# geekieo/collaborative-deep-metric-learning

Measured on NVIDIA B200. Metric: train_triplets_per_sec, higher is better.
Workload: dtype fp16 operands / fp32 accumulate (tcgen05 kind::f16), fp32 master weights

## Files before the change

collaborative-deep-metric-learning_b200/csrc/gemm_launch.cuh:

```cuda
#pragma once
#include "../../include/cdml.h"
#include "ctx.cuh"
#include "gemm_sm100.cuh"
#include "gemm2_sm100.cuh"

#include <stdlib.h>

namespace cdml {

inline bool trace_on() {
  static int on = -1;
  if (on < 0) on = getenv("CDML_TRACE") != nullptr ? 1 : 0;
  return on == 1;
}
inline int trace_sync(const char* what, long M, long N, long K, int grid, cudaStream_t st) {
  if (!trace_on()) return 0;
  fprintf(stderr, "[cdml] %s M=%ld N=%ld K=%ld grid=%d ... ", what, M, N, K, grid);
  fflush(stderr);
  cudaError_t e = cudaStreamSynchronize(st);
  fprintf(stderr, "%s\n", cudaGetErrorString(e));
  fflush(stderr);
  return e == cudaSuccess ? 0 : -2;
}

constexpr int kBN = 256;
constexpr int kStages = 4;

inline int pick_splits(int num_sms, int tiles, int num_kb) {
  if (tiles >= 2 * num_sms || num_kb < 16) return 1;
  const int smax = max(1, min(64, num_kb / 8));
  int best = 1;
  double best_eff = -1.0;
  for (int s = 1; s <= smax; ++s) {
    const int per = (num_kb + s - 1) / s;
    const int seff = (num_kb + per - 1) / per;
    if (seff != s) continue;
    const long units = static_cast<long>(tiles) * s;
    const long waves = (units + num_sms - 1) / num_sms;
    double eff = static_cast<double>(units) / static_cast<double>(waves * num_sms);
    if (units < num_sms) eff *= 0.5;
    eff -= 0.002 * s;
    if (eff > best_eff) best_eff = eff, best = s;
  }
  return best;
}

inline bool two_cta_enabled() {
  static int on = -1;
  if (on < 0) {
    const char* e = getenv("CDML_2CTA");
    on = (e != nullptr && e[0] == '0') ? 0 : 1;
  }
  return on == 1;
}

template <int AMN, int BMN, class Epi>
static int launch_gemm2(cdml_ctx* ctx, const void* A, int64_t lda, const void* B, int64_t ldb, int64_t M, int64_t N,
                        int64_t K, int dtype16, int num_splits, const Epi& epi, cudaStream_t stream) {
  using L = Gemm2Smem;
  CUtensorMap ta, tb;
  int rc;
  if (AMN == 0) rc = make_tmap_2d(ctx, &ta, A, dtype16, K, M, lda, kBK, kBM);
  else rc = make_tmap_2d(ctx, &ta, A, dtype16, M, K, lda, 64, kBK);
  if (rc) return rc;
  if (BMN == 0) rc = make_tmap_2d(ctx, &tb, B, dtype16, K, N, ldb, kBK, kBN2 / 2);
  else rc = make_tmap_2d(ctx, &tb, B, dtype16, N, K, ldb, 64, kBK);
  if (rc) return rc;
  GemmShape s;
  s.M = static_cast<int>(M), s.N = static_cast<int>(N), s.K = static_cast<int>(K);
  s.m_tiles = (s.M + 2 * kBM - 1) / (2 * kBM);
  s.n_tiles = (s.N + kBN2 - 1) / kBN2;
  s.num_kb = (s.K + kBK - 1) / kBK;
  num_splits = max(1, min(num_splits, s.num_kb));
  s.kb_per_split = (s.num_kb + num_splits - 1) / num_splits;
  s.num_splits = (s.num_kb + s.kb_per_split - 1) / s.kb_per_split;
  s.idesc = make_idesc_f16(dtype16 == CDML_BF16 ? 1 : 0, AMN, BMN, 2 * kBM, kBN2);
  s.m_fastest = (s.num_splits > 1 && N >= M) ? 1 : 0;
  auto kern = gemm2_tcgen05_kernel<AMN, BMN, Epi>;
  static bool attr_set = false;
  if (!attr_set) {
    CDML_CHECK_CUDA(cudaFuncSetAttribute(kern, cudaFuncAttributeMaxDynamicSharedMemorySize, L::kTotal));
    attr_set = true;
  }
  const long units = static_cast<long>(s.m_tiles) * s.n_tiles * s.num_splits;
  const int clusters = static_cast<int>(units < ctx->num_sms / 2 ? units : ctx->num_sms / 2);
  cudaLaunchConfig_t cfg = {};
  cfg.gridDim = dim3(2 * clusters);
  cfg.blockDim = dim3(kGemmThreads);
  cfg.dynamicSmemBytes = L::kTotal;
  cfg.stream = stream;
  cudaLaunchAttribute attr[1];
  attr[0].id = cudaLaunchAttributeClusterDimension;
  attr[0].val.clusterDim.x = 2, attr[0].val.clusterDim.y = 1, attr[0].val.clusterDim.z = 1;
  cfg.attrs = attr;
  cfg.numAttrs = 1;
  CDML_CHECK_CUDA(cudaLaunchKernelEx(&cfg, kern, ta, tb, s, epi));
  if (trace_sync("gemm2_tcgen05", M, N, K, 2 * clusters, stream)) return -2;
  return s.num_splits;
}

template <int AMN, int BMN, class Epi>
static int launch_gemm(cdml_ctx* ctx, const void* A, int64_t lda, const void* B, int64_t ldb, int64_t M, int64_t N,
                       int64_t K, int dtype16, int num_splits, const Epi& epi, cudaStream_t stream) {
  {
    const int64_t kb_per = ((K + kBK - 1) / kBK + max(num_splits, 1) - 1) / max(num_splits, 1);
    if (two_cta_enabled() && M >= 2 * kBM && kb_per >= 8)
      return launch_gemm2<AMN, BMN>(ctx, A, lda, B, ldb, M, N, K, dtype16, num_splits, epi, stream);
  }
  using L = GemmSmem<kBN, kStages>;
  CUtensorMap ta, tb;
  int rc;
  if (AMN == 0) rc = make_tmap_2d(ctx, &ta, A, dtype16, K, M, lda, kBK, kBM);
  else rc = make_tmap_2d(ctx, &ta, A, dtype16, M, K, lda, 64, kBK);
  if (rc) return rc;
  if (BMN == 0) rc = make_tmap_2d(ctx, &tb, B, dtype16, K, N, ldb, kBK, kBN);
  else rc = make_tmap_2d(ctx, &tb, B, dtype16, N, K, ldb, 64, kBK);
  if (rc) return rc;

  GemmShape s;
  s.M = static_cast<int>(M), s.N = static_cast<int>(N), s.K = static_cast<int>(K);
  s.m_tiles = (s.M + kBM - 1) / kBM;
  s.n_tiles = (s.N + kBN - 1) / kBN;
  s.num_kb = (s.K + kBK - 1) / kBK;
  num_splits = max(1, min(num_splits, s.num_kb));
  s.kb_per_split = (s.num_kb + num_splits - 1) / num_splits;
  s.num_splits = (s.num_kb + s.kb_per_split - 1) / s.kb_per_split;
  s.idesc = make_idesc_f16(dtype16 == CDML_BF16 ? 1 : 0, AMN, BMN, kBM, kBN);
  s.m_fastest = (s.num_splits > 1 && N >= M) ? 1 : 0;

  auto kern = gemm_tcgen05_kernel<AMN, BMN, kBN, kStages, Epi>;
  static bool attr_set = false;
  if (!attr_set) {
    CDML_CHECK_CUDA(cudaFuncSetAttribute(kern, cudaFuncAttributeMaxDynamicSharedMemorySize, L::kTotal));
    attr_set = true;
  }
  const long units = static_cast<long>(s.m_tiles) * s.n_tiles * s.num_splits;
  const int grid = static_cast<int>(units < ctx->num_sms ? units : ctx->num_sms);
  kern<<<grid, kGemmThreads, L::kTotal, stream>>>(ta, tb, s, epi);
  CDML_CHECK_CUDA(cudaGetLastError());
  if (trace_sync("gemm_tcgen05", M, N, K, grid, stream)) return -2;
  return s.num_splits;
}

constexpr int kResBStages = 4;
inline bool resb_applicable(int64_t K) {
  static int off = -1;
  if (off < 0) off = getenv("CDML_NO_RESB") != nullptr ? 1 : 0;
  return off == 0 && K <= 4 * kBK;
}

template <class Epi, int kEpiWarps = 8>
static int launch_gemm_resb(cdml_ctx* ctx, const void* A, int64_t lda, const void* B, int64_t ldb, int64_t M, int64_t N,
                            int64_t K, int dtype16, const Epi& epi, cudaStream_t stream, int n_fastest = 0) {
  using L = ResBSmem<kBN, kResBStages, kEpiWarps, Epi::kRowConsts, Epi::kTmaStore ? 2 : 1>;
  static_assert(L::kTotal <= 232448, "resident-B kernel: shared memory over the 227 KB limit");
  CUtensorMap ta, tb;
  int rc = make_tmap_2d(ctx, &ta, A, dtype16, K, M, lda, kBK, kBM);
  if (rc) return rc;
  rc = make_tmap_2d(ctx, &tb, B, dtype16, K, N, ldb, kBK, kBN);
  if (rc) return rc;
  ResBShape s;
  s.M = static_cast<int>(M), s.N = static_cast<int>(N), s.K = static_cast<int>(K);
  s.m_tiles = (s.M + kBM - 1) / kBM;
  s.n_tiles = (s.N + kBN - 1) / kBN;
  s.num_kb = (s.K + kBK - 1) / kBK;
  int best = 1;
  double best_eff = -1.0;
  const int cmax = max(1, min(s.m_tiles / 8, 4 * ctx->num_sms));
  for (int c = 1; c <= cmax; ++c) {
    const int tpc = (s.m_tiles + c - 1) / c;
    const int ceff = (s.m_tiles + tpc - 1) / tpc;
    if (ceff != c) continue;
    const long units = static_cast<long>(s.n_tiles) * c;
    const long waves = (units + ctx->num_sms - 1) / ctx->num_sms;
    double eff = static_cast<double>(units) / static_cast<double>(waves * ctx->num_sms);
    eff -= 0.15 / tpc;
    if (eff > best_eff) best_eff = eff, best = c;
  }
  s.m_chunks = best;
  s.tiles_per_chunk = (s.m_tiles + best - 1) / best;
  s.n_fastest = n_fastest;
  s.idesc = make_idesc_f16(dtype16 == CDML_BF16 ? 1 : 0, 0, 0, kBM, kBN);
  auto kern = gemm_resb_tcgen05_kernel<kBN, kResBStages, Epi, kEpiWarps>;
  static bool attr_set = false;
  if (!attr_set) {
    CDML_CHECK_CUDA(cudaFuncSetAttribute(kern, cudaFuncAttributeMaxDynamicSharedMemorySize, L::kTotal));
    attr_set = true;
  }
  const long units = static_cast<long>(s.n_tiles) * s.m_chunks;
  const int grid = static_cast<int>(units < ctx->num_sms ? units : ctx->num_sms);
  kern<<<grid, 128 + 32 * kEpiWarps, L::kTotal, stream>>>(ta, tb, s, epi);
  CDML_CHECK_CUDA(cudaGetLastError());
  if (trace_sync("gemm_resb", M, N, K, grid, stream)) return -2;
  return 1;
}

}
```

collaborative-deep-metric-learning_b200/csrc/gemm_sm100.cuh:

```cuda
#pragma once
#include "common.cuh"

namespace cdml {

constexpr int kBM = 128;
constexpr int kBK = 64;
constexpr int kUK = 16;
constexpr uint32_t kEpiStageBytes = 16384;
constexpr int kGemmThreads = 384;

struct GemmShape {
  int M, N, K;
  int m_tiles, n_tiles;
  int num_kb;
  int kb_per_split;
  int num_splits;
  int m_fastest;
  uint32_t idesc;
};

template <int BN, int kStages>
struct GemmSmem {
  static constexpr uint32_t kABytes = kBM * kBK * 2;
  static constexpr uint32_t kBBytes = BN * kBK * 2;
  static constexpr uint32_t kEpiOff = kStages * (kABytes + kBBytes);
  static constexpr uint32_t kBarOff = kEpiOff + kEpiStageBytes;
  static constexpr uint32_t kNumBars = 2 * kStages + 4;
  static constexpr uint32_t kTotal = kBarOff + kNumBars * 8 + 16 + 1024;
};

__device__ __forceinline__ float leaky(float v, float alpha) { return v > 0.f ? v : alpha * v; }
__device__ __forceinline__ float chunk_bias(const float* bias, int nb, int N) {
  const int col = nb + static_cast<int>(threadIdx.x & 31);
  return (bias != nullptr && col < N) ? __ldg(bias + col) : 0.f;
}

__device__ __forceinline__ void store_chunk16(uint16_t* out, int64_t ld, int row_base, int nb, int M, int N, uint32_t stg,
                                              const uint32_t (&pk)[16]) {
  const int lane = threadIdx.x & 31;
  __syncwarp();
#pragma unroll
  for (int j = 0; j < 4; ++j)
    sts128(stg + lane * 64 + ((j ^ ((lane >> 1) & 3)) << 4), pk[4 * j], pk[4 * j + 1], pk[4 * j + 2], pk[4 * j + 3]);
  __syncwarp();
  const int cch = lane & 3;
  const int col = nb + 8 * cch;
  const bool vec = (ld & 7) == 0;
#pragma unroll
  for (int i = 0; i < 4; ++i) {
    const int r = 8 * i + (lane >> 2);
    const uint4 v = lds128(stg + r * 64 + ((cch ^ ((r >> 1) & 3)) << 4));
    const int grow = row_base + r;
    if (grow < M) {
      uint16_t* p = out + static_cast<int64_t>(grow) * ld + col;
      if (vec && col + 8 <= N) {
        *reinterpret_cast<uint4*>(p) = v;
      } else {
        const uint32_t w[4] = {v.x, v.y, v.z, v.w};
#pragma unroll
        for (int e = 0; e < 8; ++e)
          if (col + e < N) p[e] = static_cast<uint16_t>(w[e >> 1] >> ((e & 1) * 16));
      }
    }
  }
}

__device__ __forceinline__ void store_chunk32(float* out, int64_t ld, int row_base, int nb, int M, int N, uint32_t stg,
                                              const float (&f)[32]) {
  const int lane = threadIdx.x & 31;
  __syncwarp();
#pragma unroll
  for (int j = 0; j < 8; ++j)
    sts128(stg + lane * 128 + ((j ^ (lane & 7)) << 4), __float_as_uint(f[4 * j]), __float_as_uint(f[4 * j + 1]),
           __float_as_uint(f[4 * j + 2]), __float_as_uint(f[4 * j + 3]));
  __syncwarp();
  const int cch = lane & 7;
  const int col = nb + 4 * cch;
  const bool vec = (ld & 3) == 0;
#pragma unroll
  for (int i = 0; i < 8; ++i) {
    const int r = 4 * i + (lane >> 3);
    const uint4 v = lds128(stg + r * 128 + ((cch ^ (r & 7)) << 4));
    const int grow = row_base + r;
    if (grow < M) {
      float* p = out + static_cast<int64_t>(grow) * ld + col;
      if (vec && col + 4 <= N) {
        *reinterpret_cast<uint4*>(p) = v;
      } else {
        const uint32_t w[4] = {v.x, v.y, v.z, v.w};
#pragma unroll
        for (int e = 0; e < 4; ++e)
          if (col + e < N) p[e] = __uint_as_float(w[e]);
      }
    }
  }
}

constexpr uint32_t kColCacheOff = 128, kColTagOff = 640, kWarpSliceBytes = 2048;
__device__ __forceinline__ void col_cache_reset(uint32_t epi_smem) {
  for (int w = 0; w < 8; ++w)
    asm volatile("st.shared.b32 [%0], %1;" ::"r"(epi_smem + w * kWarpSliceBytes + kColTagOff), "r"(0u) : "memory");
}
template <class Fetch>
__device__ __forceinline__ void col_cache_fill(uint32_t stg, int n0, int c0, Fetch&& fetch) {
  uint32_t tag;
  asm volatile("ld.shared.b32 %0, [%1];" : "=r"(tag) : "r"(stg + kColTagOff) : "memory");
  if (tag == static_cast<uint32_t>(n0 + 1)) return;
  const int lane = threadIdx.x & 31;
  __syncwarp();
#pragma unroll
  for (int i = 0; i < 4; ++i) {
    const uint32_t v = fetch(n0 + (c0 + i) * 32 + lane);
    asm volatile("st.shared.b32 [%0], %1;" ::"r"(stg + kColCacheOff + 4 * (32 * i + lane)), "r"(v) : "memory");
  }
  if (lane == 0) asm volatile("st.shared.b32 [%0], %1;" ::"r"(stg + kColTagOff), "r"(n0 + 1) : "memory");
  __syncwarp();
}

template <int BN>
struct EpiStoreF32 {
  static constexpr bool kSplitColumns = true;
  struct State {};
  __device__ __forceinline__ void pre(State&, int, int, const GemmShape&, int, int, uint32_t) const {}
  static constexpr bool kPrefetchNext = false;
  static constexpr bool kRowConsts = false;
  static constexpr bool kEarlyRelease = false;
  static constexpr bool kTmaStore = false;
  __device__ __forceinline__ void cols(int, const GemmShape&, int, int, uint32_t) const {}
  __device__ __forceinline__ void block_begin(uint32_t) const {}
  __device__ __forceinline__ void block_end(uint32_t) const {}
  float* out;
  int64_t ld;
  int64_t split_stride;
  const float* bias;
  float alpha;
  __device__ __forceinline__ void run(uint32_t taddr, int row, int n0, int split, const GemmShape& s, int c0, int c1, uint32_t stg, State& st) const {
    float* orow = out + static_cast<int64_t>(split) * split_stride + static_cast<int64_t>(row) * ld;
    const bool row_ok = row < s.M;
#pragma unroll 1
    for (int c = c0; c < c1; ++c) {
      const int nb = n0 + c * 32;
      if (nb >= s.N) break;
      uint32_t v[32];
      tmem_ld_32x32(taddr + c * 32, v);
      const float b_lane = chunk_bias(bias, nb, s.N);
      tmem_ld_wait();
      float f[32];
#pragma unroll
      for (int j = 0; j < 32; ++j)
        f[j] = leaky(__uint_as_float(v[j]) + __shfl_sync(0xffffffffu, b_lane, j), alpha);
      if (row_ok) {
        if (nb + 32 <= s.N && (ld & 3) == 0) {
          float4* p = reinterpret_cast<float4*>(orow + nb);
#pragma unroll
          for (int j = 0; j < 8; ++j) p[j] = make_float4(f[4 * j], f[4 * j + 1], f[4 * j + 2], f[4 * j + 3]);
        } else {
#pragma unroll
          for (int j = 0; j < 32; ++j)
            if (nb + j < s.N) orow[nb + j] = f[j];
        }
      }
    }
  }
};

template <int BN, int kBf16>
struct EpiStore16 {
  static constexpr bool kSplitColumns = true;
  struct State {};
  __device__ __forceinline__ void pre(State&, int, int, const GemmShape&, int, int, uint32_t) const {}
  static constexpr bool kPrefetchNext = false;
  static constexpr bool kRowConsts = false;
  static constexpr bool kEarlyRelease = false;
  static constexpr bool kTmaStore = false;
  __device__ __forceinline__ void cols(int, const GemmShape&, int, int, uint32_t) const {}
  __device__ __forceinline__ void block_begin(uint32_t) const {}
  __device__ __forceinline__ void block_end(uint32_t) const {}
  uint16_t* out;
  int64_t ld;
  const float* bias;
  float alpha;
  uint32_t* mask_out;
  int64_t ld_mask;
  __device__ __forceinline__ void run(uint32_t taddr, int row, int n0, int , const GemmShape& s, int c0, int c1, uint32_t stg, State& st) const {
#pragma unroll 1
    for (int c = c0; c < c1; ++c) {
      const int nb = n0 + c * 32;
      if (nb >= s.N) break;
      uint32_t v[32];
      tmem_ld_32x32(taddr + c * 32, v);
      const float b_lane = chunk_bias(bias, nb, s.N);
      tmem_ld_wait();
      uint32_t pk[16];
      uint32_t bits = 0u;
#pragma unroll
      for (int j = 0; j < 16; ++j) {
        const float x0 = __uint_as_float(v[2 * j]) + __shfl_sync(0xffffffffu, b_lane, 2 * j);
        const float x1 = __uint_as_float(v[2 * j + 1]) + __shfl_sync(0xffffffffu, b_lane, 2 * j + 1);
        bits |= (x0 > 0.f ? 1u : 0u) << (2 * j);
        bits |= (x1 > 0.f ? 1u : 0u) << (2 * j + 1);
        pk[j] = pack2<kBf16>(leaky(x0, alpha), leaky(x1, alpha));
      }
      if (mask_out != nullptr && row < s.M) mask_out[static_cast<int64_t>(nb >> 5) * ld_mask + row] = bits;
      store_chunk16(out, ld, row - static_cast<int>(threadIdx.x & 31), nb, s.M, s.N, stg, pk);
    }
  }
};

template <int BN, int kBf16>
struct EpiL2Norm {
  static constexpr bool kSplitColumns = false;
  struct State {};
  __device__ __forceinline__ void pre(State&, int, int, const GemmShape&, int, int, uint32_t) const {}
  static constexpr bool kPrefetchNext = false;
  static constexpr bool kRowConsts = false;
  static constexpr bool kEarlyRelease = false;
  static constexpr bool kTmaStore = false;
  __device__ __forceinline__ void cols(int, const GemmShape&, int, int, uint32_t) const {}
  __device__ __forceinline__ void block_begin(uint32_t) const {}
  __device__ __forceinline__ void block_end(uint32_t) const {}
  float* out;
  int64_t ld;
  const float* bias;
  float alpha;
  float* rinv;
  uint16_t* out16;
  int64_t ld16;
  __device__ __forceinline__ void run(uint32_t taddr, int row, int n0, int , const GemmShape& s, int c0, int c1, uint32_t stg, State& st) const {
    const bool row_ok = row < s.M;
    float ss = 0.f;
#pragma unroll 1
    for (int c = c0; c < c1; ++c) {
      const int nb = n0 + c * 32;
      if (nb >= s.N) break;
      uint32_t v[32];
      tmem_ld_32x32(taddr + c * 32, v);
      const float b_lane = chunk_bias(bias, nb, s.N);
      tmem_ld_wait();
#pragma unroll
      for (int j = 0; j < 32; ++j) {
        const float x = leaky(__uint_as_float(v[j]) + __shfl_sync(0xffffffffu, b_lane, j), alpha);
        ss = fmaf(x, x, ss);
      }
    }
    const float r = rsqrtf(fmaxf(ss, 1e-12f));
    if (row_ok && rinv != nullptr) rinv[row] = r;
#pragma unroll 1
    for (int c = c0; c < c1; ++c) {
      const int nb = n0 + c * 32;
      if (nb >= s.N) break;
      uint32_t v[32];
      tmem_ld_32x32(taddr + c * 32, v);
      const float b_lane = chunk_bias(bias, nb, s.N);
      tmem_ld_wait();
      float f[32];
#pragma unroll
      for (int j = 0; j < 32; ++j)
        f[j] = leaky(__uint_as_float(v[j]) + __shfl_sync(0xffffffffu, b_lane, j), alpha) * r;
      store_chunk32(out, ld, row - static_cast<int>(threadIdx.x & 31), nb, s.M, s.N, stg, f);
      if (out16 != nullptr) {
        uint32_t pk[16];
#pragma unroll
        for (int j = 0; j < 16; ++j) pk[j] = pack2<kBf16>(f[2 * j], f[2 * j + 1]);
        store_chunk16(out16, ld16, row - static_cast<int>(threadIdx.x & 31), nb, s.M, s.N, stg, pk);
      }
    }
  }
};

template <int BN, int kBf16>
struct EpiMaskLeaky {
  static constexpr bool kSplitColumns = true;
  struct State {
    uint4 raw[4][4];
  };
  static constexpr bool kPrefetchNext = false;
  static constexpr bool kRowConsts = false;
  static constexpr bool kEarlyRelease = false;
  static constexpr bool kTmaStore = false;
  __device__ __forceinline__ void cols(int, const GemmShape&, int, int, uint32_t) const {}
  __device__ __forceinline__ void block_begin(uint32_t) const {}
  __device__ __forceinline__ void block_end(uint32_t) const {}
  uint16_t* out;
  int64_t ld;
  const uint16_t* mask;
  int64_t ld_mask;
  float alpha;
  __device__ __forceinline__ void fetch_mask(int row_base, int nb, int M, int N, bool active, uint4 (&raw)[4]) const {
    const int lane = threadIdx.x & 31;
    const int col = nb + 8 * (lane & 3);
#pragma unroll
    for (int i = 0; i < 4; ++i) {
      const int grow = row_base + 8 * i + (lane >> 2);
      raw[i] = make_uint4(0u, 0u, 0u, 0u);
      if (active && grow < M) {
        const uint16_t* p = mask + static_cast<int64_t>(grow) * ld_mask + col;
        if ((ld_mask & 7) == 0 && col + 8 <= N) {
          raw[i] = __ldg(reinterpret_cast<const uint4*>(p));
        } else {
          uint32_t w[4] = {0u, 0u, 0u, 0u};
#pragma unroll
          for (int e = 0; e < 8; ++e)
            if (col + e < N) w[e >> 1] |= static_cast<uint32_t>(p[e]) << ((e & 1) * 16);
          raw[i] = make_uint4(w[0], w[1], w[2], w[3]);
        }
      }
    }
  }
  __device__ __forceinline__ void transpose_mask(uint32_t stg, const uint4 (&raw)[4], uint32_t (&mk)[16]) const {
    const int lane = threadIdx.x & 31;
    const int cch = lane & 3;
    __syncwarp();
#pragma unroll
    for (int i = 0; i < 4; ++i) {
      const int r = 8 * i + (lane >> 2);
      sts128(stg + r * 64 + ((cch ^ ((r >> 1) & 3)) << 4), raw[i].x, raw[i].y, raw[i].z, raw[i].w);
    }
    __syncwarp();
#pragma unroll
    for (int j = 0; j < 4; ++j) {
      const uint4 t = lds128(stg + lane * 64 + ((j ^ ((lane >> 1) & 3)) << 4));
      mk[4 * j] = t.x, mk[4 * j + 1] = t.y, mk[4 * j + 2] = t.z, mk[4 * j + 3] = t.w;
    }
  }
  __device__ __forceinline__ void pre(State& st, int row, int n0, const GemmShape& s, int c0, int c1, uint32_t ) const {
    static_assert(BN == 256, "a warp owns 4 chunks of the tile");
    const int row_base = row - static_cast<int>(threadIdx.x & 31);
#pragma unroll
    for (int cc = 0; cc < 4; ++cc)
      fetch_mask(row_base, n0 + (c0 + cc) * 32, s.M, s.N, c0 + cc < c1 && n0 + (c0 + cc) * 32 < s.N, st.raw[cc]);
  }
  __device__ __forceinline__ void run(uint32_t taddr, int row, int n0, int , const GemmShape& s, int c0, int c1,
                                      uint32_t stg, State& st) const {
    const int row_base = row - static_cast<int>(threadIdx.x & 31);
#pragma unroll
    for (int cc = 0; cc < 4; ++cc) {
      const int c = c0 + cc;
      const int nb = n0 + c * 32;
      if (c < c1 && nb < s.N) {
        uint32_t v[32];
        tmem_ld_32x32(taddr + c * 32, v);
        uint32_t mk[16];
        transpose_mask(stg, st.raw[cc], mk);
        tmem_ld_wait();
        uint32_t pk[16];
#pragma unroll
        for (int j = 0; j < 16; ++j) {
          const float2 m = unpack2<kBf16>(mk[j]);
          const float x0 = __uint_as_float(v[2 * j]) * (m.x > 0.f ? 1.f : alpha);
          const float x1 = __uint_as_float(v[2 * j + 1]) * (m.y > 0.f ? 1.f : alpha);
          pk[j] = pack2<kBf16>(x0, x1);
        }
        store_chunk16(out, ld, row_base, nb, s.M, s.N, stg, pk);
      }
    }
  }
};

template <int BN, int kBf16>
struct EpiMaskBits {
  static constexpr bool kSplitColumns = true;
  struct State {
    uint32_t bits[4];
  };
  static constexpr bool kPrefetchNext = true;
  static constexpr bool kRowConsts = false;
  static constexpr bool kEarlyRelease = false;
  static constexpr bool kTmaStore = false;
  __device__ __forceinline__ void cols(int, const GemmShape&, int, int, uint32_t) const {}
  __device__ __forceinline__ void block_begin(uint32_t) const {}
  __device__ __forceinline__ void block_end(uint32_t) const {}
  uint16_t* out;
  int64_t ld;
  const uint32_t* mask;
  int64_t ld_mask;
  float alpha;
  __device__ __forceinline__ void pre(State& st, int row, int n0, const GemmShape& s, int c0, int c1, uint32_t ) const {
    static_assert(BN == 256, "a warp owns 4 chunks of the tile");
#pragma unroll
    for (int cc = 0; cc < 4; ++cc) {
      const int nb = n0 + (c0 + cc) * 32;
      st.bits[cc] = (c0 + cc < c1 && nb < s.N && row < s.M) ? __ldg(mask + static_cast<int64_t>(nb >> 5) * ld_mask + row) : 0u;
    }
  }
  __device__ __forceinline__ void run(uint32_t taddr, int row, int n0, int , const GemmShape& s, int c0, int c1,
                                      uint32_t stg, State& st) const {
    const int row_base = row - static_cast<int>(threadIdx.x & 31);
    auto ok = [&](int cc) { return c0 + cc < c1 && n0 + (c0 + cc) * 32 < s.N; };
    auto chunk = [&](const uint32_t (&v)[32], int cc) {
      const uint32_t b = st.bits[cc];
      uint32_t pk[16];
#pragma unroll
      for (int j = 0; j < 16; ++j) {
        const float x0 = __uint_as_float(v[2 * j]) * ((b >> (2 * j)) & 1u ? 1.f : alpha);
        const float x1 = __uint_as_float(v[2 * j + 1]) * ((b >> (2 * j + 1)) & 1u ? 1.f : alpha);
        pk[j] = pack2<kBf16>(x0, x1);
      }
      store_chunk16(out, ld, row_base, n0 + (c0 + cc) * 32, s.M, s.N, stg, pk);
    };
    uint32_t va[32], vb[32];
    if (ok(0)) tmem_ld_32x32(taddr + c0 * 32, va);
#pragma unroll
    for (int cc = 0; cc < 4; cc += 2) {
      tmem_ld_wait();
      if (ok(cc + 1)) tmem_ld_32x32(taddr + (c0 + cc + 1) * 32, vb);
      if (ok(cc)) chunk(va, cc);
      tmem_ld_wait();
      if (cc + 2 < 4 && ok(cc + 2)) tmem_ld_32x32(taddr + (c0 + cc + 2) * 32, va);
      if (ok(cc + 1)) chunk(vb, cc + 1);
    }
  }
};

template <int BN, int kBf16>
struct EpiMaskBitsTma {
  static constexpr bool kSplitColumns = true;
  struct State {
    uint32_t bits[4];
    uint32_t release_bar;
  };
  static constexpr bool kPrefetchNext = true;
  static constexpr bool kRowConsts = false;
  static constexpr bool kEarlyRelease = true;
  static constexpr bool kTmaStore = true;
  __device__ __forceinline__ void cols(int, const GemmShape&, int, int, uint32_t) const {}
  __device__ __forceinline__ void block_begin(uint32_t) const {}
  __device__ __forceinline__ void block_end(uint32_t) const {}
  CUtensorMap out_map;
  const uint32_t* mask;
  int64_t ld_mask;
  float alpha;
  __device__ __forceinline__ void pre(State& st, int row, int n0, const GemmShape& s, int c0, int c1, uint32_t ) const {
    static_assert(BN == 256, "a warp owns 4 chunks of the tile");
#pragma unroll
    for (int cc = 0; cc < 4; ++cc) {
      const int nb = n0 + (c0 + cc) * 32;
      st.bits[cc] = (c0 + cc < c1 && nb < s.N && row < s.M) ? __ldg(mask + static_cast<int64_t>(nb >> 5) * ld_mask + row) : 0u;
    }
    st.release_bar = 0u;
  }
  __device__ __forceinline__ void run(uint32_t taddr, int row, int n0, int , const GemmShape& s, int c0, int c1,
                                      uint32_t stg0, State& st) const {
    const int lane = threadIdx.x & 31;
    const int row_base = row - lane;
    auto ok = [&](int cc) { return c0 + cc < c1 && n0 + (c0 + cc) * 32 < s.N; };
    auto chunk = [&](const uint32_t (&v)[32], int cc) {
      const uint32_t b = st.bits[cc];
      uint32_t pk[16];
#pragma unroll
      for (int j = 0; j < 16; ++j) {
        const float x0 = __uint_as_float(v[2 * j]) * ((b >> (2 * j)) & 1u ? 1.f : alpha);
        const float x1 = __uint_as_float(v[2 * j + 1]) * ((b >> (2 * j + 1)) & 1u ? 1.f : alpha);
        pk[j] = pack2<kBf16>(x0, x1);
      }
      const uint32_t stg = stg0 + (cc & 1) * 2048u;
      if (lane == 0) bulk_wait_read1();
      __syncwarp();
#pragma unroll
      for (int j = 0; j < 4; ++j)
        sts128(stg + lane * 64 + ((j ^ ((lane >> 1) & 3)) << 4), pk[4 * j], pk[4 * j + 1], pk[4 * j + 2], pk[4 * j + 3]);
      fence_proxy_async();
      __syncwarp();
      if (lane == 0) {
        tma_store_2d(&out_map, stg, n0 + (c0 + cc) * 32, row_base);
        bulk_commit();
      }
    };
    uint32_t va[32], vb[32];
    if (ok(0)) tmem_ld_32x32(taddr + c0 * 32, va);
#pragma unroll
    for (int cc = 0; cc < 4; cc += 2) {
      tmem_ld_wait();
      if (ok(cc + 1)) tmem_ld_32x32(taddr + (c0 + cc + 1) * 32, vb);
      if (ok(cc)) chunk(va, cc);
      tmem_ld_wait();
      if (cc + 2 < 4 && ok(cc + 2)) tmem_ld_32x32(taddr + (c0 + cc + 2) * 32, va);
      if (cc + 2 >= 4 && st.release_bar != 0u) {
        tc_fence_before();
        __syncwarp();
        if (lane == 0) mbar_arrive(st.release_bar);
      }
      if (ok(cc + 1)) chunk(vb, cc + 1);
    }
  }
};

template <int BN, int kReadTmem>
struct EpiNull {
  static constexpr bool kSplitColumns = true;
  struct State {};
  __device__ __forceinline__ void pre(State&, int, int, const GemmShape&, int, int, uint32_t) const {}
  static constexpr bool kPrefetchNext = false;
  static constexpr bool kRowConsts = false;
  static constexpr bool kEarlyRelease = false;
  static constexpr bool kTmaStore = false;
  __device__ __forceinline__ void cols(int, const GemmShape&, int, int, uint32_t) const {}
  __device__ __forceinline__ void block_begin(uint32_t) const {}
  __device__ __forceinline__ void block_end(uint32_t) const {}
  float* out;
  __device__ __forceinline__ void run(uint32_t taddr, int row, int n0, int , const GemmShape& s, int c0, int c1, uint32_t stg, State& st) const {
    if (kReadTmem) {
      uint32_t acc = 0u;
#pragma unroll 1
      for (int c = c0; c < c1; ++c) {
        uint32_t v[32];
        tmem_ld_32x32(taddr + c * 32, v);
        tmem_ld_wait();
#pragma unroll
        for (int j = 0; j < 32; ++j) acc ^= v[j];
      }
      if (acc == 0x7fc12345u && row == s.M + 7) out[0] = 1.f;
    }
  }
};

template <int kAMajorMN, int kBMajorMN, int BN, int kStages, class Epi>
__global__ void __launch_bounds__(kGemmThreads, 1)
gemm_tcgen05_kernel(const __grid_constant__ CUtensorMap tma_a, const __grid_constant__ CUtensorMap tma_b,
                    const GemmShape s, const Epi epi) {
  using L = GemmSmem<BN, kStages>;
  extern __shared__ uint8_t smem_raw[];
  const uint32_t raw_u32 = smem_u32(smem_raw);
  const uint32_t base = (raw_u32 + 1023u) & ~1023u;
  const uint32_t bar0 = base + L::kBarOff;
  auto a_smem = [&](int st) { return base + st * L::kABytes; };
  auto b_smem = [&](int st) { return base + kStages * L::kABytes + st * L::kBBytes; };
  auto full_bar = [&](int st) { return bar0 + 8u * st; };
  auto empty_bar = [&](int st) { return bar0 + 8u * (kStages + st); };
  auto tfull_bar = [&](int i) { return bar0 + 8u * (2 * kStages + i); };
  auto tempty_bar = [&](int i) { return bar0 + 8u * (2 * kStages + 2 + i); };
  const uint32_t tmem_slot = bar0 + 8u * L::kNumBars;
  volatile uint32_t* tmem_slot_ptr = reinterpret_cast<volatile uint32_t*>(smem_raw + (tmem_slot - raw_u32));

  const int warp = threadIdx.x >> 5;
  const int lane = threadIdx.x & 31;
  constexpr uint32_t kTmemCols = (2 * BN <= 32) ? 32 : (2 * BN <= 64) ? 64 : (2 * BN <= 128) ? 128 : (2 * BN <= 256) ? 256 : 512;
  static_assert(2 * BN <= 512, "two accumulator stages must fit TMEM");

  if (warp == 0 && lane == 0) {
    tma_prefetch_desc(&tma_a);
    tma_prefetch_desc(&tma_b);
  }
  if (warp == 1 && lane == 0) {
    for (int i = 0; i < kStages; ++i) {
      mbar_init(full_bar(i), 1);
      mbar_init(empty_bar(i), 1);
    }
    for (int i = 0; i < 2; ++i) {
      mbar_init(tfull_bar(i), 1);
      mbar_init(tempty_bar(i), 8);
    }
    fence_mbar_init();
  }
  if (warp == 2) {
    tmem_alloc(tmem_slot, kTmemCols);
    tmem_relinquish();
  }
  if (threadIdx.x == 96) epi.block_begin(base + L::kEpiOff);
  tc_fence_before();
  __syncthreads();
  tc_fence_after();
  const uint32_t tmem_base = *tmem_slot_ptr;

  const int tiles = s.m_tiles * s.n_tiles;
  const int units = tiles * s.num_splits;

  if (warp == 0 && lane == 0) {
    int stage = 0;
    uint32_t phase = 0;
    for (int u = blockIdx.x; u < units; u += gridDim.x) {
      const int split = u / tiles, t = u - split * tiles;
      const int m0 = (s.m_fastest ? t % s.m_tiles : t / s.n_tiles) * kBM;
      const int n0 = (s.m_fastest ? t / s.m_tiles : t % s.n_tiles) * BN;
      const int kb0 = split * s.kb_per_split;
      const int kb1 = min(s.num_kb, kb0 + s.kb_per_split);
      for (int kb = kb0; kb < kb1; ++kb) {
        mbar_wait(empty_bar(stage), phase ^ 1, 100 + stage);
        mbar_arrive_expect_tx(full_bar(stage), L::kABytes + L::kBBytes);
        const int k0 = kb * kBK;
        if constexpr (kAMajorMN == 0) {
          tma_load_2d(a_smem(stage), &tma_a, full_bar(stage), k0, m0);
        } else {
#pragma unroll
          for (int i = 0; i < kBM / 64; ++i)
            tma_load_2d(a_smem(stage) + i * (kBK * 128), &tma_a, full_bar(stage), m0 + i * 64, k0);
        }
        if constexpr (kBMajorMN == 0) {
          tma_load_2d(b_smem(stage), &tma_b, full_bar(stage), k0, n0);
        } else {
#pragma unroll
          for (int i = 0; i < BN / 64; ++i)
            tma_load_2d(b_smem(stage) + i * (kBK * 128), &tma_b, full_bar(stage), n0 + i * 64, k0);
        }
        if (++stage == kStages) stage = 0, phase ^= 1;
      }
    }
  } else if (warp == 1 && lane == 0) {
    int stage = 0;
    uint32_t phase = 0;
    int it = 0;
    constexpr uint32_t kAStep = kAMajorMN ? (kUK * 128) : (kUK * 2);
    constexpr uint32_t kBStep = kBMajorMN ? (kUK * 128) : (kUK * 2);
    constexpr uint32_t kALbo = kAMajorMN ? (kBK * 128) : 16;
    constexpr uint32_t kBLbo = kBMajorMN ? (kBK * 128) : 16;
    for (int u = blockIdx.x; u < units; u += gridDim.x, ++it) {
      const int split = u / tiles;
      const int kb0 = split * s.kb_per_split;
      const int kb1 = min(s.num_kb, kb0 + s.kb_per_split);
      const int as = it & 1;
      const uint32_t ap = (it >> 1) & 1;
      mbar_wait(tempty_bar(as), ap ^ 1, 200 + as);
      tc_fence_after();
      const uint32_t tmem_d = tmem_base + as * BN;
      for (int kb = kb0; kb < kb1; ++kb) {
        mbar_wait(full_bar(stage), phase, 300 + stage);
        tc_fence_after();
#pragma unroll
        for (int k = 0; k < kBK / kUK; ++k) {
          const uint64_t ad = make_smem_desc(a_smem(stage) + k * kAStep, kALbo, 1024);
          const uint64_t bd = make_smem_desc(b_smem(stage) + k * kBStep, kBLbo, 1024);
          umma_f16(tmem_d, ad, bd, s.idesc, (kb > kb0 || k > 0) ? 1u : 0u);
        }
        tc_commit(empty_bar(stage));
        if (kb == kb1 - 1) tc_commit(tfull_bar(as));
        if (++stage == kStages) stage = 0, phase ^= 1;
      }
    }
  } else if (warp >= 4) {
    const int q = warp & 3;
    const int half = (warp - 4) >> 2;
    const uint32_t stg = base + L::kEpiOff + (warp - 4) * (Epi::kSplitColumns ? 2048u : 4096u);
    int it = 0;
    for (int u = blockIdx.x; u < units; u += gridDim.x, ++it) {
      const int split = u / tiles, t = u - split * tiles;
      const int m0 = (s.m_fastest ? t % s.m_tiles : t / s.n_tiles) * kBM;
      const int n0 = (s.m_fastest ? t / s.m_tiles : t % s.n_tiles) * BN;
      const int as = it & 1;
      const uint32_t ap = (it >> 1) & 1;
      const int ec0 = Epi::kSplitColumns ? half * (BN / 64) : 0, ec1 = Epi::kSplitColumns ? (half + 1) * (BN / 64) : BN / 32;
      typename Epi::State est;
      if (Epi::kSplitColumns || half == 0) {
        epi.cols(n0, s, ec0, ec1, stg);
        epi.pre(est, m0 + q * 32 + lane, n0, s, ec0, ec1, stg);
      }
      mbar_wait(tfull_bar(as), ap, 400 + as);
      tc_fence_after();
      const uint32_t taddr = tmem_base + (static_cast<uint32_t>(q * 32) << 16) + as * BN;
      if (Epi::kSplitColumns || half == 0) epi.run(taddr, m0 + q * 32 + lane, n0, split, s, ec0, ec1, stg, est);
      tc_fence_before();
      __syncwarp();
      if (lane == 0) mbar_arrive(tempty_bar(as));
    }
  }

  tc_fence_before();
  __syncthreads();
  if (threadIdx.x == 96) epi.block_end(base + L::kEpiOff);
  if (warp == 2) {
    tc_fence_after();
    tmem_dealloc(tmem_base, kTmemCols);
  }
}

struct ResBShape {
  int M, N, K;
  int m_tiles, n_tiles, num_kb;
  int m_chunks;
  int tiles_per_chunk;
  int n_fastest;
  uint32_t idesc;
};

template <int BN, int kAStages, int kEpiWarps = 8, bool kRowSlots = false, int kStageSlices = 1>
struct ResBSmem {
  static constexpr uint32_t kABytes = kBM * kBK * 2;
  static constexpr uint32_t kBPanel = BN * kBK * 2;
  static constexpr uint32_t kMaxKb = 4;
  static constexpr uint32_t kEpiOff = kMaxKb * kBPanel + kAStages * kABytes;
  static constexpr uint32_t kEpiBytes = kEpiWarps * 2048 * kStageSlices;
  static constexpr uint32_t kRowConstOff = kEpiOff + kEpiBytes;
  static constexpr uint32_t kRowConstSlot = kRowSlots ? kBM * 32 : 0;
  static constexpr uint32_t kBarOff = kRowConstOff + 2 * kRowConstSlot;
  static constexpr uint32_t kNumBars = 2 * kAStages + 2 + 4 + 2;
  static constexpr uint32_t kTotal = kBarOff + kNumBars * 8 + 16 + 1024;
};

template <int BN, int kAStages, class Epi, int kEpiWarps = 8>
__global__ void __launch_bounds__(128 + 32 * kEpiWarps, 1)
gemm_resb_tcgen05_kernel(const __grid_constant__ CUtensorMap tma_a, const __grid_constant__ CUtensorMap tma_b,
                         const ResBShape s, const __grid_constant__ Epi epi) {
  using L = ResBSmem<BN, kAStages, kEpiWarps, Epi::kRowConsts, Epi::kTmaStore ? 2 : 1>;
  static_assert(kEpiWarps == 8 || kEpiWarps == 16, "two or four epilogue warps per TMEM lane quarter");
  static_assert(kEpiWarps == 8 || Epi::kSplitColumns, "four warps per quarter split the tile's columns");
  extern __shared__ uint8_t smem_raw[];
  const uint32_t raw_u32 = smem_u32(smem_raw);
  const uint32_t base = (raw_u32 + 1023u) & ~1023u;
  const uint32_t bar0 = base + L::kBarOff;
  auto b_panel = [&](int kb) { return base + kb * L::kBPanel; };
  auto a_smem = [&](int st) { return base + L::kMaxKb * L::kBPanel + st * L::kABytes; };
  auto a_full = [&](int st) { return bar0 + 8u * st; };
  auto a_empty = [&](int st) { return bar0 + 8u * (kAStages + st); };
  const uint32_t b_full = bar0 + 8u * (2 * kAStages);
  const uint32_t b_empty = bar0 + 8u * (2 * kAStages + 1);
  auto tfull_bar = [&](int i) { return bar0 + 8u * (2 * kAStages + 2 + i); };
  auto tempty_bar = [&](int i) { return bar0 + 8u * (2 * kAStages + 4 + i); };
  auto cfull_bar = [&](int i) { return bar0 + 8u * (2 * kAStages + 6 + i); };
  auto cslot = [&](int i) { return base + L::kRowConstOff + i * L::kRowConstSlot; };
  const uint32_t tmem_slot = bar0 + 8u * L::kNumBars;
  volatile uint32_t* tmem_slot_ptr = reinterpret_cast<volatile uint32_t*>(smem_raw + (tmem_slot - raw_u32));
  const int warp = threadIdx.x >> 5;
  const int lane = threadIdx.x & 31;
  constexpr uint32_t kTmemCols = 512;
  static_assert(2 * BN <= 512, "two accumulator stages must fit TMEM");

  if (warp == 0 && lane == 0) {
    tma_prefetch_desc(&tma_a);
    tma_prefetch_desc(&tma_b);
  }
  if (warp == 1 && lane == 0) {
    for (int i = 0; i < kAStages; ++i) {
      mbar_init(a_full(i), 1);
      mbar_init(a_empty(i), 1);
    }
    mbar_init(b_full, 1);
    mbar_init(b_empty, 1);
    for (int i = 0; i < 2; ++i) {
      mbar_init(tfull_bar(i), 1);
      mbar_init(tempty_bar(i), kEpiWarps);
      mbar_init(cfull_bar(i), 1);
    }
    fence_mbar_init();
  }
  if (warp == 2) {
    tmem_alloc(tmem_slot, kTmemCols);
    tmem_relinquish();
  }
  if (threadIdx.x == 96) epi.block_begin(base + L::kEpiOff);
  tc_fence_before();
  __syncthreads();
  tc_fence_after();
  const uint32_t tmem_base = *tmem_slot_ptr;

  const int units = s.n_tiles * s.m_chunks;
  if (warp == 0 && lane == 0) {
    int stage = 0;
    uint32_t phase = 0, bphase = 0;
    for (int u = blockIdx.x; u < units; u += gridDim.x) {
      const int chunk = s.n_fastest ? u / s.n_tiles : u % s.m_chunks, nblk = s.n_fastest ? u % s.n_tiles : u / s.m_chunks;
      const int t0 = chunk * s.tiles_per_chunk, t1 = min(s.m_tiles, t0 + s.tiles_per_chunk);
      if (t0 >= t1) continue;
      mbar_wait(b_empty, bphase ^ 1, 500);
      mbar_arrive_expect_tx(b_full, s.num_kb * L::kBPanel);
      for (int kb = 0; kb < s.num_kb; ++kb) tma_load_2d(b_panel(kb), &tma_b, b_full, kb * kBK, nblk * BN);
      bphase ^= 1;
      for (int t = t0; t < t1; ++t) {
        for (int kb = 0; kb < s.num_kb; ++kb) {
          mbar_wait(a_empty(stage), phase ^ 1, 100 + stage);
          mbar_arrive_expect_tx(a_full(stage), L::kABytes);
          tma_load_2d(a_smem(stage), &tma_a, a_full(stage), kb * kBK, t * kBM);
          if (++stage == kAStages) stage = 0, phase ^= 1;
        }
      }
    }
  } else if (warp == 1 && lane == 0) {
    int stage = 0, it = 0;
    uint32_t phase = 0, bphase = 0;
    for (int u = blockIdx.x; u < units; u += gridDim.x) {
      const int chunk = s.n_fastest ? u / s.n_tiles : u % s.m_chunks, nblk = s.n_fastest ? u % s.n_tiles : u / s.m_chunks;
      const int t0 = chunk * s.tiles_per_chunk, t1 = min(s.m_tiles, t0 + s.tiles_per_chunk);
      if (t0 >= t1) continue;
      mbar_wait(b_full, bphase, 600);
      bphase ^= 1;
      tc_fence_after();
      for (int t = t0; t < t1; ++t, ++it) {
        const int as = it & 1;
        const uint32_t ap = (it >> 1) & 1;
        mbar_wait(tempty_bar(as), ap ^ 1, 200 + as);
        tc_fence_after();
        const uint32_t tmem_d = tmem_base + as * BN;
        for (int kb = 0; kb < s.num_kb; ++kb) {
          mbar_wait(a_full(stage), phase, 300 + stage);
          tc_fence_after();
#pragma unroll
          for (int k = 0; k < kBK / kUK; ++k) {
            const uint64_t ad = make_smem_desc(a_smem(stage) + k * (kUK * 2), 16, 1024);
            const uint64_t bd = make_smem_desc(b_panel(kb) + k * (kUK * 2), 16, 1024);
            umma_f16(tmem_d, ad, bd, s.idesc, (kb > 0 || k > 0) ? 1u : 0u);
          }
          tc_commit(a_empty(stage));
          if (kb == s.num_kb - 1) tc_commit(tfull_bar(as));
          if (++stage == kAStages) stage = 0, phase ^= 1;
        }
      }
      tc_commit(b_empty);
    }
  } else if (warp == 3) {
   if constexpr (Epi::kRowConsts) {
    int it = 0;
    GemmShape gs;
    gs.M = s.M, gs.N = s.N, gs.K = s.K;
    for (int u = blockIdx.x; u < units; u += gridDim.x) {
      const int chunk = s.n_fastest ? u / s.n_tiles : u % s.m_chunks;
      const int t0 = chunk * s.tiles_per_chunk, t1 = min(s.m_tiles, t0 + s.tiles_per_chunk);
      for (int t = t0; t < t1; ++t, ++it) {
        const int as = it & 1;
        const uint32_t ap = (it >> 1) & 1;
        mbar_wait(tempty_bar(as), ap ^ 1, 700 + as);
#pragma unroll
        for (int r = lane; r < kBM; r += 32) epi.row_consts(t * kBM + r, gs, cslot(as) + r * 32);
        __syncwarp();
        if (lane == 0) mbar_arrive(cfull_bar(as));
      }
    }
   }
  } else if (warp >= 4) {
    const int q = warp & 3;
    const int half = (warp - 4) >> 2;
    const uint32_t stg = base + L::kEpiOff + (warp - 4) * (Epi::kTmaStore ? 4096u : (Epi::kSplitColumns || kEpiWarps == 16) ? 2048u : 4096u);
    int it = 0;
    GemmShape gs;
    gs.M = s.M, gs.N = s.N, gs.K = s.K, gs.m_tiles = s.m_tiles, gs.n_tiles = s.n_tiles, gs.num_kb = s.num_kb;
    gs.kb_per_split = s.num_kb, gs.num_splits = 1, gs.m_fastest = 0, gs.idesc = s.idesc;
    struct TileIter {
      int u, t, t1, nblk;
      bool valid;
    };
    auto seek = [&](TileIter& ti) {
      ti.valid = false;
      for (; ti.u < units; ti.u += gridDim.x) {
        const int chunk = s.n_fastest ? ti.u / s.n_tiles : ti.u % s.m_chunks;
        const int t0 = chunk * s.tiles_per_chunk, t1 = min(s.m_tiles, t0 + s.tiles_per_chunk);
        if (t0 < t1) {
          ti.t = t0, ti.t1 = t1, ti.nblk = s.n_fastest ? ti.u % s.n_tiles : ti.u / s.m_chunks, ti.valid = true;
          return;
        }
      }
    };
    const bool active = Epi::kSplitColumns || half == 0;
    constexpr int kChunksPerWarp = (BN / 32) / (kEpiWarps / 4);
    const int ec0 = Epi::kSplitColumns ? half * kChunksPerWarp : 0, ec1 = Epi::kSplitColumns ? (half + 1) * kChunksPerWarp : BN / 32;
    TileIter cur;
    cur.u = blockIdx.x;
    seek(cur);
    typename Epi::State est;
    if (cur.valid && active) {
      epi.cols(cur.nblk * BN, gs, ec0, ec1, stg);
      if constexpr (!Epi::kRowConsts) epi.pre(est, cur.t * kBM + q * 32 + lane, cur.nblk * BN, gs, ec0, ec1, stg);
    }
    while (cur.valid) {
      TileIter nxt = cur;
      if (++nxt.t >= nxt.t1) {
        nxt.u += gridDim.x;
        seek(nxt);
      }
      const int as = it & 1;
      const uint32_t ap = (it >> 1) & 1;
      typename Epi::State est_next;
      if constexpr (Epi::kRowConsts) {
        mbar_wait(cfull_bar(as), ap, 800 + as);
        if (active) epi.load_state(est, cslot(as) + (q * 32 + lane) * 32);
        est_next = est;
      }
      mbar_wait(tfull_bar(as), ap, 400 + as);
      tc_fence_after();
      const uint32_t taddr = tmem_base + (static_cast<uint32_t>(q * 32) << 16) + as * BN;
      if (active) {
        if constexpr (!Epi::kRowConsts)
          if (Epi::kPrefetchNext && nxt.valid) epi.pre(est_next, nxt.t * kBM + q * 32 + lane, nxt.nblk * BN, gs, ec0, ec1, stg);
        if constexpr (Epi::kEarlyRelease) est.release_bar = tempty_bar(as);
        epi.run(taddr, cur.t * kBM + q * 32 + lane, cur.nblk * BN, 0, gs, ec0, ec1, stg, est);
      }
      if (!(Epi::kEarlyRelease && active)) {
        tc_fence_before();
        __syncwarp();
        if (lane == 0) mbar_arrive(tempty_bar(as));
      }
      if (active && nxt.valid) {
        epi.cols(nxt.nblk * BN, gs, ec0, ec1, stg);
        if constexpr (!Epi::kRowConsts)
          if (!Epi::kPrefetchNext) epi.pre(est_next, nxt.t * kBM + q * 32 + lane, nxt.nblk * BN, gs, ec0, ec1, stg);
      }
      est = est_next;
      cur = nxt;
      ++it;
    }
    if constexpr (Epi::kTmaStore) {
      if (lane == 0) bulk_wait_all();
    }
  }

  tc_fence_before();
  __syncthreads();
  if (threadIdx.x == 96) epi.block_end(base + L::kEpiOff);
  if (warp == 2) {
    tc_fence_after();
    tmem_dealloc(tmem_base, kTmemCols);
  }
}

}
```

collaborative-deep-metric-learning_b200/csrc/knn.cu:

```cuda
#include <math.h>
#include <string.h>

#include <algorithm>

#include <vector>

#include "gemm_launch.cuh"

namespace cdml {

constexpr int kCandCap = 2048;
constexpr int kKeepCap = 2048;
constexpr int kMaxGroups = 4096;
constexpr int kRefineThreads = 256;

__device__ __forceinline__ uint32_t f2key(float f) {
  const uint32_t u = __float_as_uint(f);
  return (u & 0x80000000u) ? ~u : (u | 0x80000000u);
}
__device__ __forceinline__ float key2f(uint32_t k) {
  return __uint_as_float((k & 0x80000000u) ? (k & 0x7FFFFFFFu) : ~k);
}
__device__ __forceinline__ float neg_inf() { return __int_as_float(0xff800000); }
__device__ __forceinline__ float pos_inf() { return __int_as_float(0x7f800000); }

__device__ __forceinline__ float4 ld4_or(const float* p, int col, int N, float fill) {
  if (col + 4 <= N) return __ldg(reinterpret_cast<const float4*>(p + col));
  float4 r;
  r.x = col < N ? __ldg(p + col) : fill;
  r.y = col + 1 < N ? __ldg(p + col + 1) : fill;
  r.z = col + 2 < N ? __ldg(p + col + 2) : fill;
  r.w = col + 3 < N ? __ldg(p + col + 3) : fill;
  return r;
}

template <int BN>
struct EpiKnnGroupMax {
  static constexpr bool kSplitColumns = true;
  static constexpr bool kPrefetchNext = false;
  static constexpr bool kRowConsts = false;
  static constexpr bool kEarlyRelease = false;
  static constexpr bool kTmaStore = false;
  struct State {};
  __device__ __forceinline__ void pre(State&, int, int, const GemmShape&, int, int, uint32_t) const {}
  __device__ __forceinline__ void block_begin(uint32_t epi_smem) const { col_cache_reset(epi_smem); }
  __device__ __forceinline__ void block_end(uint32_t) const {}
  const float* h;
  float* gmax;
  int64_t ldg;
  int wide;
  __device__ __forceinline__ void cols(int n0, const GemmShape& s, int c0, int , uint32_t stg) const {
    static_assert(BN == 256, "a warp owns 4 chunks (128 columns) of the tile");
    col_cache_fill(stg, n0, c0, [&](int col) { return __float_as_uint(col < s.N ? __ldg(h + col) : pos_inf()); });
  }
  __device__ __forceinline__ void run(uint32_t taddr, int row, int n0, int , const GemmShape& s, int c0,
                                      int , uint32_t stg, State& ) const {
    float g[4];
    uint32_t va[32], vb[32];
    auto group = [&](const uint32_t (&v)[32], int cc) {
      const uint32_t hbase = stg + kColCacheOff + 128 * cc;
      float b0 = neg_inf(), b1 = neg_inf();
#pragma unroll
      for (int j = 0; j < 8; ++j) {
        const uint4 t = lds128(hbase + 16 * j);
        const float2 lo = sub2(__uint_as_float(v[4 * j]), __uint_as_float(v[4 * j + 1]), __uint_as_float(t.x), __uint_as_float(t.y));
        const float2 hi = sub2(__uint_as_float(v[4 * j + 2]), __uint_as_float(v[4 * j + 3]), __uint_as_float(t.z), __uint_as_float(t.w));
        b0 = fmax3(b0, lo.x, lo.y);
        b1 = fmax3(b1, hi.x, hi.y);
      }
      return fmaxf(b0, b1);
    };
    auto ok = [&](int cc) { return n0 + (c0 + cc) * 32 < s.N; };
    tmem_ld_32x32(taddr + c0 * 32, va);
#pragma unroll
    for (int cc = 0; cc < 4; cc += 2) {
      tmem_ld_wait();
      if (ok(cc + 1)) tmem_ld_32x32(taddr + (c0 + cc + 1) * 32, vb);
      g[cc] = ok(cc) ? group(va, cc) : neg_inf();
      tmem_ld_wait();
      if (cc + 2 < 4 && ok(cc + 2)) tmem_ld_32x32(taddr + (c0 + cc + 2) * 32, va);
      g[cc + 1] = ok(cc + 1) ? group(vb, cc + 1) : neg_inf();
    }
    if (row < s.M) {
      if (wide) gmax[static_cast<int64_t>(row) * ldg + n0 / 128 + c0 / 4] = fmaxf(fmaxf(g[0], g[1]), fmaxf(g[2], g[3]));
      else *reinterpret_cast<float4*>(gmax + static_cast<int64_t>(row) * ldg + n0 / 32 + c0) = make_float4(g[0], g[1], g[2], g[3]);
    }
  }
};

constexpr uint32_t kKnnWarpStage = kWarpSliceBytes;
constexpr uint32_t kKnnThrOff = kColCacheOff, kKnnCurOff = 644;
constexpr int kKnnLogsPerCta = 8;

template <int BN>
struct EpiKnnCollect {
  static constexpr bool kSplitColumns = true;
  const float* h;
  const float* thr;
  uint4* log;
  int32_t* log_count;
  int32_t* log_overflow;
  unsigned int warp_cap;
  struct State {
    float hr;
    uint32_t release_bar;
  };
  static constexpr bool kPrefetchNext = true;
  static constexpr bool kRowConsts = false;
  static constexpr bool kEarlyRelease = true;
  static constexpr bool kTmaStore = false;
  __device__ __forceinline__ void block_begin(uint32_t epi_smem) const {
    col_cache_reset(epi_smem);
    for (int w = 0; w < kKnnLogsPerCta; ++w)
      asm volatile("st.shared.b32 [%0], %1;" ::"r"(epi_smem + w * kKnnWarpStage + kKnnCurOff), "r"(0u) : "memory");
  }
  __device__ __forceinline__ void block_end(uint32_t epi_smem) const {
    for (int w = 0; w < kKnnLogsPerCta; ++w) {
      unsigned int n;
      asm volatile("ld.shared.b32 %0, [%1];" : "=r"(n) : "r"(epi_smem + w * kKnnWarpStage + kKnnCurOff) : "memory");
      log_count[blockIdx.x * kKnnLogsPerCta + w] = static_cast<int32_t>(n < warp_cap ? n : warp_cap);
      if (n > warp_cap) atomicOr(log_overflow, 1);
    }
  }
  __device__ __forceinline__ void pre(State& st, int row, int, const GemmShape& s, int, int, uint32_t) const {
    st.hr = row < s.M ? __ldg(h + row) : pos_inf();
    st.release_bar = 0u;
  }
  __device__ __forceinline__ void cols(int n0, const GemmShape& s, int c0, int , uint32_t stg) const {
    static_assert(BN == 256, "a warp owns 4 chunks (128 columns) of the tile");
    col_cache_fill(stg, n0, c0, [&](int col) { return __float_as_uint(col < s.N ? __ldg(thr + col) : pos_inf()); });
  }
  __device__ __forceinline__ void run(uint32_t taddr, int row, int n0, int , const GemmShape& s, int c0,
                                      int c1, uint32_t stg, State& st) const {
    const float hr = st.hr;
    const int lane = threadIdx.x & 31;
    const int warp_slot = (threadIdx.x >> 5) - 4;
    uint4* my_log = log + (static_cast<size_t>(blockIdx.x) * kKnnLogsPerCta + warp_slot) * warp_cap;
    unsigned int cursor;
    asm volatile("ld.shared.b32 %0, [%1];" : "=r"(cursor) : "r"(stg + kKnnCurOff) : "memory");
    uint32_t va[32], vb[32];
    tmem_ld_32x32(taddr + c0 * 32, va);
    auto chunk = [&](const uint32_t (&v)[32], int cc) {
      const int nb = n0 + (c0 + cc) * 32;
      const uint32_t tbase = stg + kKnnThrOff + 128 * cc;
      float m0 = neg_inf(), m1 = neg_inf();
#pragma unroll
      for (int j = 0; j < 8; ++j) {
        const uint4 t = lds128(tbase + 16 * j);
        const float2 lo = sub2(__uint_as_float(v[4 * j]), __uint_as_float(v[4 * j + 1]), __uint_as_float(t.x), __uint_as_float(t.y));
        const float2 hi = sub2(__uint_as_float(v[4 * j + 2]), __uint_as_float(v[4 * j + 3]), __uint_as_float(t.z), __uint_as_float(t.w));
        m0 = fmax3(m0, lo.x, lo.y);
        m1 = fmax3(m1, hi.x, hi.y);
      }
      unsigned int hits = __ballot_sync(0xffffffffu, fmaxf(m0, m1) > hr);
      if (hits != 0u) {
        float thr_lane;
        asm volatile("ld.shared.f32 %0, [%1];" : "=f"(thr_lane) : "r"(tbase + 4 * lane) : "memory");
        do {
          const int src = __ffs(hits) - 1;
          hits &= hits - 1u;
          __syncwarp();
          if (lane == src) {
#pragma unroll
            for (int j = 0; j < 8; ++j) sts128(stg + 16 * j, v[4 * j], v[4 * j + 1], v[4 * j + 2], v[4 * j + 3]);
          }
          __syncwarp();
          float val;
          asm volatile("ld.shared.f32 %0, [%1];" : "=f"(val) : "r"(stg + 4 * lane) : "memory");
          const float hr_src = __shfl_sync(0xffffffffu, hr, src);
          const bool pass = val - thr_lane > hr_src;
          const unsigned int pm = __ballot_sync(0xffffffffu, pass);
          const unsigned int pos = cursor + static_cast<unsigned int>(__popc(pm & ((1u << lane) - 1u)));
          if (pass && pos < warp_cap)
            my_log[pos] = make_uint4(static_cast<uint32_t>(nb + lane), static_cast<uint32_t>(row - lane + src),
                                     __float_as_uint(val - hr_src), 0u);
          cursor += static_cast<unsigned int>(__popc(pm));
        } while (hits != 0u);
      }
    };
#pragma unroll
    for (int cc = 0; cc < 4; cc += 2) {
      const bool ok0 = c0 + cc < c1 && n0 + (c0 + cc) * 32 < s.N;
      const bool ok1 = c0 + cc + 1 < c1 && n0 + (c0 + cc + 1) * 32 < s.N;
      const bool ok2 = cc + 2 < 4 && c0 + cc + 2 < c1 && n0 + (c0 + cc + 2) * 32 < s.N;
      tmem_ld_wait();
      if (ok1) tmem_ld_32x32(taddr + (c0 + cc + 1) * 32, vb);
      if (ok0) chunk(va, cc);
      tmem_ld_wait();
      if (ok2) tmem_ld_32x32(taddr + (c0 + cc + 2) * 32, va);
      if (cc + 2 >= 4 && st.release_bar != 0u) {
        tc_fence_before();
        __syncwarp();
        if (lane == 0) mbar_arrive(st.release_bar);
      }
      if (ok1) chunk(vb, cc + 1);
    }
    __syncwarp();
    if (lane == 0) asm volatile("st.shared.b32 [%0], %1;" ::"r"(stg + kKnnCurOff), "r"(cursor) : "memory");
  }
};

__global__ void __launch_bounds__(256)
knn_bin_kernel(const uint4* __restrict__ log, const int32_t* __restrict__ log_count, unsigned int log_cap,
               int32_t* __restrict__ cand_idx, float* __restrict__ cand_val, int32_t* __restrict__ cnt, int cap) {
  const int n = log_count[blockIdx.y];
  const uint4* my = log + static_cast<size_t>(blockIdx.y) * log_cap;
  for (int i = blockIdx.x * blockDim.x + threadIdx.x; i < n; i += gridDim.x * blockDim.x) {
    const uint4 e = my[i];
    const int pos = atomicAdd(cnt + e.x, 1);
    if (pos < cap) {
      cand_idx[static_cast<int64_t>(e.x) * cap + pos] = static_cast<int32_t>(e.y);
      cand_val[static_cast<int64_t>(e.x) * cap + pos] = __uint_as_float(e.z);
    }
  }
}

__global__ void __launch_bounds__(256)
row_sumsq32_kernel(const float* __restrict__ X, int64_t n, int d, int64_t ld, float* __restrict__ ss, float half_scale,
                   float* __restrict__ half_out) {
  const int warp = threadIdx.x >> 5, lane = threadIdx.x & 31;
  for (int64_t r = static_cast<int64_t>(blockIdx.x) * 8 + warp; r < n; r += static_cast<int64_t>(gridDim.x) * 8) {
    const float* x = X + r * ld;
    float a = 0.f;
    for (int j = lane; j < d; j += 32) a = fmaf(x[j], x[j], a);
#pragma unroll
    for (int o = 16; o > 0; o >>= 1) a += __shfl_xor_sync(0xffffffffu, a, o);
    if (lane == 0) {
      ss[r] = a;
      if (half_out != nullptr) half_out[r] = a * half_scale;
    }
  }
}

__global__ void max_reduce_kernel(const float* __restrict__ x, int64_t n, float* __restrict__ out) {
  __shared__ float sh[32];
  float m = 0.f;
  for (int64_t i = threadIdx.x; i < n; i += blockDim.x) m = fmaxf(m, x[i]);
#pragma unroll
  for (int o = 16; o > 0; o >>= 1) m = fmaxf(m, __shfl_xor_sync(0xffffffffu, m, o));
  if ((threadIdx.x & 31) == 0) sh[threadIdx.x >> 5] = m;
  __syncthreads();
  if (threadIdx.x < 32) {
    m = threadIdx.x < (blockDim.x >> 5) ? sh[threadIdx.x] : 0.f;
#pragma unroll
    for (int o = 16; o > 0; o >>= 1) m = fmaxf(m, __shfl_xor_sync(0xffffffffu, m, o));
    if (threadIdx.x == 0) *out = m;
  }
}

__global__ void fill_f32_kernel(float* p, int64_t n, float v) {
  for (int64_t i = static_cast<int64_t>(blockIdx.x) * blockDim.x + threadIdx.x; i < n;
       i += static_cast<int64_t>(gridDim.x) * blockDim.x)
    p[i] = v;
}

__device__ __forceinline__ int block_sum(int v, int* sh) {
  v = __reduce_add_sync(0xffffffffu, v);
  __syncthreads();
  if ((threadIdx.x & 31) == 0) sh[threadIdx.x >> 5] = v;
  __syncthreads();
  int t = 0;
  for (int w = 0; w < (blockDim.x >> 5); ++w) t += sh[w];
  return t;
}

constexpr int kSelectBits = 20;
template <int kPer, bool kDual>
__global__ void __launch_bounds__(kRefineThreads)
knn_kth_kernel(const float* __restrict__ gmax, int64_t ldg, int G, int k, int k2, const float* __restrict__ qss,
               float slack_scale, float slack_abs, float* __restrict__ thr, float* __restrict__ thr2, float sign2) {
  __shared__ int sh[kRefineThreads / 32];
  const int q = blockIdx.x;
  const float* g = gmax + static_cast<int64_t>(q) * ldg;
  uint32_t keys[kPer];
#pragma unroll
  for (int i = 0; i < kPer; ++i) {
    const int j = threadIdx.x + i * kRefineThreads;
    keys[i] = j < G ? f2key(g[j]) : 0u;
  }
  uint32_t T = 0, T2 = 0;
  for (int bit = 31; bit >= 32 - kSelectBits; --bit) {
    const uint32_t cand = T | (1u << bit), cand2 = T2 | (1u << bit);
    int c = 0;
#pragma unroll
    for (int i = 0; i < kPer; ++i) c += (keys[i] >= cand ? 1 : 0) + (kDual && keys[i] >= cand2 ? 65536 : 0);
    c = block_sum(c, sh);
    if ((c & 0xffff) >= k) T = cand;
    if (kDual && (c >> 16) >= k2) T2 = cand2;
  }
  if (threadIdx.x == 0) {
    const float slack = slack_scale * sqrtf(qss[q]) + slack_abs;
    thr[q] = T > f2key(neg_inf()) ? key2f(T) - slack : neg_inf();
    if (kDual) thr2[q] = sign2 * (T2 > f2key(neg_inf()) ? key2f(T2) - slack : neg_inf());
  }
}

template <bool kDual>
__global__ void __launch_bounds__(256)
knn_kth_warp_kernel(const float* __restrict__ gmax, int64_t ldg, int G, int k, int k2, const float* __restrict__ qss,
                    int64_t nq, float slack_scale, float slack_abs, float* __restrict__ thr, float* __restrict__ thr2,
                    float sign2) {
  const int lane = threadIdx.x & 31;
  const int64_t q = static_cast<int64_t>(blockIdx.x) * 8 + (threadIdx.x >> 5);
  if (q >= nq) return;
  const float* g = gmax + q * ldg;
  uint32_t keys[32];
#pragma unroll
  for (int i = 0; i < 32; ++i) {
    const int j = lane + 32 * i;
    keys[i] = j < G ? f2key(g[j]) : 0u;
  }
  uint32_t T = 0, T2 = 0;
  for (int bit = 31; bit >= 32 - kSelectBits; --bit) {
    const uint32_t cand = T | (1u << bit), cand2 = T2 | (1u << bit);
    int c = 0;
#pragma unroll
    for (int i = 0; i < 32; ++i) c += (keys[i] >= cand ? 1 : 0) + (kDual && keys[i] >= cand2 ? 65536 : 0);
    c = __reduce_add_sync(0xffffffffu, c);
    if ((c & 0xffff) >= k) T = cand;
    if (kDual && (c >> 16) >= k2) T2 = cand2;
  }
  if (lane == 0) {
    const float slack = slack_scale * sqrtf(qss[q]) + slack_abs;
    thr[q] = T > f2key(neg_inf()) ? key2f(T) - slack : neg_inf();
    if (kDual) thr2[q] = sign2 * (T2 > f2key(neg_inf()) ? key2f(T2) - slack : neg_inf());
  }
}

__global__ void __launch_bounds__(256)
knn_nominee_kth_kernel(const float* __restrict__ cand_val, const int32_t* __restrict__ cnt, int cap, int k, int k2,
                       int64_t nq, float* __restrict__ pair) {
  const int lane = threadIdx.x & 31;
  const int64_t q = static_cast<int64_t>(blockIdx.x) * 8 + (threadIdx.x >> 5);
  if (q >= nq) return;
  const int n = cnt[q];
  float a = neg_inf(), b = neg_inf();
  if (n <= cap && n >= min(k, k2)) {
    const float* v = cand_val + q * cap;
    uint32_t keys[8];
    const bool in_regs = n <= 256;
#pragma unroll
    for (int i = 0; i < 8; ++i) keys[i] = (in_regs && lane + 32 * i < n) ? f2key(v[lane + 32 * i]) : 0u;
    uint32_t T = 0, T2 = 0;
    for (int bit = 31; bit >= 32 - kSelectBits; --bit) {
      const uint32_t cand = T | (1u << bit), cand2 = T2 | (1u << bit);
      int c = 0;
      if (in_regs) {
#pragma unroll
        for (int i = 0; i < 8; ++i) c += (keys[i] >= cand ? 1 : 0) + (keys[i] >= cand2 ? 65536 : 0);
      } else {
        for (int i = lane; i < n; i += 32) {
          const uint32_t key = f2key(v[i]);
          c += (key >= cand ? 1 : 0) + (key >= cand2 ? 65536 : 0);
        }
      }
      c = __reduce_add_sync(0xffffffffu, c);
      if ((c & 0xffff) >= k) T = cand;
      if ((c >> 16) >= k2) T2 = cand2;
    }
    if (n >= k && T > f2key(neg_inf())) a = key2f(T);
    if (n >= k2 && T2 > f2key(neg_inf())) b = key2f(T2);
  }
  if (lane == 0) pair[q] = a, pair[nq + q] = -b;
}

__global__ void knn_thr_combine_kernel(const float* __restrict__ full, const float* __restrict__ part,
                                       const float* __restrict__ qss, int64_t n, float slack_scale, float slack_abs,
                                       float* __restrict__ thr, float part_sign) {
  const int64_t i = static_cast<int64_t>(blockIdx.x) * blockDim.x + threadIdx.x;
  if (i >= n) return;
  const float b = fmaxf(full[i], part_sign * part[i]);
  thr[i] = b > neg_inf() ? b - (slack_scale * sqrtf(qss[i]) + slack_abs) : neg_inf();
}

__global__ void __launch_bounds__(kRefineThreads)
knn_refine_kernel(const float* __restrict__ Q, int64_t ldq, int d, const float* __restrict__ qss,
                  const float* __restrict__ X, int64_t ldx, const float* __restrict__ xss,
                  const int32_t* __restrict__ cand_idx, const float* __restrict__ cand_val,
                  const int32_t* __restrict__ cnt, int cap, int k, int metric, float slack_scale, float slack_abs,
                  int64_t id_offset, float* __restrict__ D, int64_t* __restrict__ I, int64_t out_ld,
                  int32_t* __restrict__ overflow, int n_all, const float* __restrict__ prune_pair, int64_t prune_ld,
                  const int32_t* __restrict__ handled) {
  __shared__ unsigned long long kept[kKeepCap];
  __shared__ int sh[kRefineThreads / 32];
  __shared__ uint32_t shu[2 * (kRefineThreads / 32)];
  __shared__ int n_keep;
  const int q = blockIdx.x;
  const int tid = threadIdx.x;
  if (handled != nullptr && handled[q] != 0) return;
  const int n = n_all > 0 ? 0 : cnt[q];
  if (n > cap) {
    if (tid == 0) overflow[q] = 1;
    return;
  }
  constexpr int kPer = kCandCap / kRefineThreads;
  uint32_t keys[kPer];
  int32_t idxs[kPer];
  uint32_t kmax = 0u, kmin = 0xffffffffu;
#pragma unroll
  for (int t = 0; t < kPer; ++t) {
    const int i = tid + t * kRefineThreads;
    keys[t] = 0u, idxs[t] = 0;
    if (i < n) {
      keys[t] = f2key(cand_val[static_cast<int64_t>(q) * cap + i]);
      idxs[t] = cand_idx[static_cast<int64_t>(q) * cap + i];
      kmax = max(kmax, keys[t]), kmin = min(kmin, keys[t]);
    }
  }
  if (tid == 0) n_keep = 0;
  uint32_t T = 0;
  if (n > k) {
    kmax = __reduce_max_sync(0xffffffffu, kmax), kmin = __reduce_min_sync(0xffffffffu, kmin);
    if ((tid & 31) == 0) shu[tid >> 5] = kmax, shu[kRefineThreads / 32 + (tid >> 5)] = kmin;
    __syncthreads();
#pragma unroll
    for (int w = 0; w < kRefineThreads / 32; ++w) kmax = max(kmax, shu[w]), kmin = min(kmin, shu[kRefineThreads / 32 + w]);
    const uint32_t diff = kmax ^ kmin;
    const int top = diff == 0u ? -1 : 31 - __clz(diff);
    T = top >= 31 ? 0u : (kmax >> (top + 1)) << (top + 1);
    for (int bit = top; bit >= 32 - kSelectBits; --bit) {
      const uint32_t cand = T | (1u << bit);
      int c = 0;
#pragma unroll
      for (int t = 0; t < kPer; ++t) c += keys[t] >= cand ? 1 : 0;
      if (block_sum(c, sh) >= k) T = cand;
    }
  } else {
    __syncthreads();
  }
  const float slack = slack_scale * sqrtf(qss[q]) + slack_abs;
  uint32_t keep_key = n > k ? f2key(key2f(T) - slack) : 0u;
  if (prune_pair != nullptr) {
    const float tg = fmaxf(prune_pair[q], -prune_pair[prune_ld + q]);
    if (tg > neg_inf()) keep_key = max(keep_key, f2key(tg - slack));
  }
#pragma unroll
  for (int t = 0; t < kPer; ++t) {
    if (tid + t * kRefineThreads < n && keys[t] >= keep_key) {
      const int pos = atomicAdd(&n_keep, 1);
      if (pos < kKeepCap) kept[pos] = static_cast<unsigned long long>(static_cast<uint32_t>(idxs[t]));
    }
  }
  if (n_all > 0) {
    for (int i = tid; i < n_all; i += kRefineThreads) kept[i] = static_cast<unsigned long long>(i);
    if (tid == 0) n_keep = n_all;
  }
  __syncthreads();
  const int nk = n_keep;
  if (nk > kKeepCap) {
    if (tid == 0) overflow[q] = 1;
    return;
  }
  const int warp = tid >> 5, lane = tid & 31;
  const float* qv = Q + static_cast<int64_t>(q) * ldq;
  const float qn = qss[q];
  const bool vec = (d & 3) == 0 && (ldx & 3) == 0 && (ldq & 3) == 0 &&
                   ((reinterpret_cast<uintptr_t>(X) | reinterpret_cast<uintptr_t>(Q)) & 15) == 0;
  for (int i0 = warp * 4; i0 < nk; i0 += (kRefineThreads / 32) * 4) {
    uint32_t id[4];
    float dot[4] = {0.f, 0.f, 0.f, 0.f};
#pragma unroll
    for (int c = 0; c < 4; ++c) id[c] = static_cast<uint32_t>(kept[min(i0 + c, nk - 1)]);
    if (vec) {
      for (int j = lane * 4; j < d; j += 128) {
        const float4 qq = __ldg(reinterpret_cast<const float4*>(qv + j));
        float4 xx[4];
#pragma unroll
        for (int c = 0; c < 4; ++c) xx[c] = __ldg(reinterpret_cast<const float4*>(X + static_cast<int64_t>(id[c]) * ldx + j));
#pragma unroll
        for (int c = 0; c < 4; ++c)
          dot[c] = fmaf(qq.x, xx[c].x, fmaf(qq.y, xx[c].y, fmaf(qq.z, xx[c].z, fmaf(qq.w, xx[c].w, dot[c]))));
      }
    } else {
      for (int j = lane; j < d; j += 32) {
        const float qj = qv[j];
#pragma unroll
        for (int c = 0; c < 4; ++c) dot[c] = fmaf(qj, X[static_cast<int64_t>(id[c]) * ldx + j], dot[c]);
      }
    }
#pragma unroll
    for (int c = 0; c < 4; ++c) {
#pragma unroll
      for (int o = 16; o > 0; o >>= 1) dot[c] += __shfl_xor_sync(0xffffffffu, dot[c], o);
    }
    __syncwarp();
    if (lane < 4 && i0 + lane < nk) {
      const float dsel = lane == 0 ? dot[0] : lane == 1 ? dot[1] : lane == 2 ? dot[2] : dot[3];
      const uint32_t isel = lane == 0 ? id[0] : lane == 1 ? id[1] : lane == 2 ? id[2] : id[3];
      const float key = metric == 0 ? fmaxf(qn + xss[isel] - 2.f * dsel, 0.f) : -dsel;
      kept[i0 + lane] = (static_cast<unsigned long long>(f2key(key)) << 32) | isel;
    }
  }
  __syncthreads();
  const auto emit = [&](int i, unsigned long long e) {
    const float key = key2f(static_cast<uint32_t>(e >> 32));
    D[static_cast<int64_t>(q) * out_ld + i] = metric == 0 ? key : -key;
    I[static_cast<int64_t>(q) * out_ld + i] = static_cast<int64_t>(static_cast<uint32_t>(e)) + id_offset;
  };
  if (nk <= 2 * kRefineThreads) {
    for (int i = tid; i < nk; i += kRefineThreads) {
      const unsigned long long e = kept[i];
      int rank = 0;
      for (int j = 0; j < nk; ++j) rank += kept[j] < e ? 1 : 0;
      if (rank < k) emit(rank, e);
    }
  } else {
    int P = 2;
    while (P < nk) P <<= 1;
    for (int i = nk + tid; i < P; i += kRefineThreads) kept[i] = ~0ull;
    __syncthreads();
    for (int size = 2; size <= P; size <<= 1) {
      for (int stride = size >> 1; stride > 0; stride >>= 1) {
        for (int t = tid; t < (P >> 1); t += kRefineThreads) {
          const int lo = ((t / stride) * (stride << 1)) + (t % stride);
          const int hi = lo + stride;
          const bool up = (lo & size) == 0;
          const unsigned long long a = kept[lo], b = kept[hi];
          if ((a > b) == up) kept[lo] = b, kept[hi] = a;
        }
        __syncthreads();
      }
    }
    for (int i = tid; i < k && i < nk; i += kRefineThreads) emit(i, kept[i]);
  }
  for (int i = nk + tid; i < k; i += kRefineThreads) {
    D[static_cast<int64_t>(q) * out_ld + i] = metric == 0 ? pos_inf() : neg_inf();
    I[static_cast<int64_t>(q) * out_ld + i] = -1;
  }
}

constexpr int kWarpNom = 256;
constexpr int kWarpKeep = 96;
__global__ void __launch_bounds__(256)
knn_refine_warp_kernel(const float* __restrict__ Q, int64_t ldq, int d, const float* __restrict__ qss,
                       const float* __restrict__ X, int64_t ldx, const float* __restrict__ xss,
                       const int32_t* __restrict__ cand_idx, const float* __restrict__ cand_val,
                       const int32_t* __restrict__ cnt, int cap, int k, int metric, float slack_scale, float slack_abs,
                       int64_t id_offset, float* __restrict__ D, int64_t* __restrict__ I, int64_t out_ld,
                       const float* __restrict__ prune_pair, int64_t prune_ld, int64_t nq, int32_t* __restrict__ handled) {
  __shared__ unsigned long long kept_all[8][kWarpKeep];
  const int warp = threadIdx.x >> 5, lane = threadIdx.x & 31;
  const int64_t q = static_cast<int64_t>(blockIdx.x) * 8 + warp;
  if (q >= nq) return;
  unsigned long long* kept = kept_all[warp];
  const int n = cnt[q];
  const float tg = fmaxf(prune_pair[q], -prune_pair[prune_ld + q]);
  if (n > kWarpNom || n > cap || !(tg > neg_inf())) {
    if (lane == 0) handled[q] = 0;
    return;
  }
  const float slack = slack_scale * sqrtf(qss[q]) + slack_abs;
  const uint32_t keep_key = f2key(tg - slack);
  int nk = 0;
#pragma unroll
  for (int t = 0; t < kWarpNom / 32; ++t) {
    const int i = lane + 32 * t;
    const bool pass = i < n && f2key(cand_val[q * cap + i]) >= keep_key;
    const unsigned int m = __ballot_sync(0xffffffffu, pass);
    const int pos = nk + __popc(m & ((1u << lane) - 1u));
    if (pass && pos < kWarpKeep) kept[pos] = static_cast<unsigned long long>(static_cast<uint32_t>(cand_idx[q * cap + i]));
    nk += __popc(m);
  }
  if (nk > kWarpKeep) {
    if (lane == 0) handled[q] = 0;
    return;
  }
  __syncwarp();
  const float* qv = Q + q * ldq;
  const float qn = qss[q];
  const bool vec = (d & 3) == 0 && (ldx & 3) == 0 && (ldq & 3) == 0 &&
                   ((reinterpret_cast<uintptr_t>(X) | reinterpret_cast<uintptr_t>(Q)) & 15) == 0;
  for (int i0 = 0; i0 < nk; i0 += 4) {
    uint32_t id[4];
    float dot[4] = {0.f, 0.f, 0.f, 0.f};
#pragma unroll
    for (int c = 0; c < 4; ++c) id[c] = static_cast<uint32_t>(kept[min(i0 + c, nk - 1)]);
    if (vec) {
      for (int j = lane * 4; j < d; j += 128) {
        const float4 qq = __ldg(reinterpret_cast<const float4*>(qv + j));
        float4 xx[4];
#pragma unroll
        for (int c = 0; c < 4; ++c) xx[c] = __ldg(reinterpret_cast<const float4*>(X + static_cast<int64_t>(id[c]) * ldx + j));
#pragma unroll
        for (int c = 0; c < 4; ++c)
          dot[c] = fmaf(qq.x, xx[c].x, fmaf(qq.y, xx[c].y, fmaf(qq.z, xx[c].z, fmaf(qq.w, xx[c].w, dot[c]))));
      }
    } else {
      for (int j = lane; j < d; j += 32) {
        const float qj = qv[j];
#pragma unroll
        for (int c = 0; c < 4; ++c) dot[c] = fmaf(qj, X[static_cast<int64_t>(id[c]) * ldx + j], dot[c]);
      }
    }
#pragma unroll
    for (int c = 0; c < 4; ++c) {
#pragma unroll
      for (int o = 16; o > 0; o >>= 1) dot[c] += __shfl_xor_sync(0xffffffffu, dot[c], o);
    }
    __syncwarp();
    if (lane < 4 && i0 + lane < nk) {
      const float dsel = lane == 0 ? dot[0] : lane == 1 ? dot[1] : lane == 2 ? dot[2] : dot[3];
      const uint32_t isel = lane == 0 ? id[0] : lane == 1 ? id[1] : lane == 2 ? id[2] : id[3];
      const float key = metric == 0 ? fmaxf(qn + xss[isel] - 2.f * dsel, 0.f) : -dsel;
      kept[i0 + lane] = (static_cast<unsigned long long>(f2key(key)) << 32) | isel;
    }
    __syncwarp();
  }
  for (int i = lane; i < nk; i += 32) {
    const unsigned long long e = kept[i];
    int rank = 0;
    for (int j = 0; j < nk; ++j) rank += kept[j] < e ? 1 : 0;
    if (rank < k) {
      const float key = key2f(static_cast<uint32_t>(e >> 32));
      D[q * out_ld + rank] = metric == 0 ? key : -key;
      I[q * out_ld + rank] = static_cast<int64_t>(static_cast<uint32_t>(e)) + id_offset;
    }
  }
  for (int i = nk + lane; i < k; i += 32) {
    D[q * out_ld + i] = metric == 0 ? pos_inf() : neg_inf();
    I[q * out_ld + i] = -1;
  }
  if (lane == 0) handled[q] = 1;
}

constexpr int kFbQueries = 8;
constexpr int kFbThreads = 256;
constexpr int kFbRound = (kFbThreads / 32) * 32;

__global__ void __launch_bounds__(kFbThreads)
knn_exact_batch_kernel(const int32_t* __restrict__ qlist, int nlist, const float* __restrict__ Q, int64_t ldq, int d,
                       const float* __restrict__ X, int64_t N, int64_t ldx, const float* __restrict__ xss, int metric,
                       int k, int kcap, int64_t id_offset, float* __restrict__ D, int64_t* __restrict__ I, int compact_out) {
  extern __shared__ unsigned long long fb_smem[];
  unsigned long long* buf = fb_smem;
  float* qs = reinterpret_cast<float*>(buf + kFbQueries * 2 * kcap);
  __shared__ uint32_t thr_key[kFbQueries];
  __shared__ int cnt[kFbQueries];
  __shared__ float qnorm[kFbQueries];
  const int tid = threadIdx.x, warp = tid >> 5, lane = tid & 31;
  const int q0 = blockIdx.x * kFbQueries;
  const int nqs = min(kFbQueries, nlist - q0);
  const int cap = 2 * kcap;
  for (int i = tid; i < kFbQueries * d; i += kFbThreads) {
    const int j = i / d;
    qs[i] = j < nqs ? Q[static_cast<int64_t>(qlist[q0 + j]) * ldq + (i - j * d)] : 0.f;
  }
  if (tid < kFbQueries) thr_key[tid] = 0xffffffffu, cnt[tid] = 0;
  __syncthreads();
  if (warp < kFbQueries) {
    float a = 0.f;
    for (int c = lane; c < d; c += 32) a = fmaf(qs[warp * d + c], qs[warp * d + c], a);
#pragma unroll
    for (int o = 16; o > 0; o >>= 1) a += __shfl_xor_sync(0xffffffffu, a, o);
    if (lane == 0) qnorm[warp] = a;
  }
  __syncthreads();
  auto compact = [&](int j) {
    const int n = min(cnt[j], cap);
    unsigned long long* b = buf + static_cast<size_t>(j) * cap;
    int P = 2;
    while (P < n) P <<= 1;
    for (int i = n + tid; i < P; i += kFbThreads) b[i] = ~0ull;
    __syncthreads();
    for (int size = 2; size <= P; size <<= 1)
      for (int stride = size >> 1; stride > 0; stride >>= 1) {
        for (int t = tid; t < (P >> 1); t += kFbThreads) {
          const int lo = ((t / stride) * (stride << 1)) + (t % stride), hi = lo + stride;
          const bool up = (lo & size) == 0;
          const unsigned long long x = b[lo], y = b[hi];
          if ((x > y) == up) b[lo] = y, b[hi] = x;
        }
        __syncthreads();
      }
    if (tid == 0) {
      const int keep = min(n, k);
      cnt[j] = keep;
      if (keep == k) thr_key[j] = static_cast<uint32_t>(b[k - 1] >> 32);
    }
    __syncthreads();
  };
  const int64_t row_lo = N * blockIdx.y / gridDim.y, row_hi = N * (blockIdx.y + 1) / gridDim.y;
  float qreg[kFbQueries][8];
#pragma unroll
  for (int j = 0; j < kFbQueries; ++j)
#pragma unroll
    for (int p = 0; p < 8; ++p) qreg[j][p] = (d <= 256 && lane + 32 * p < d) ? qs[j * d + lane + 32 * p] : 0.f;
  for (int64_t r0 = row_lo; r0 < row_hi; r0 += kFbRound) {
    auto offer = [&](int64_t r, const float (&dot)[kFbQueries]) {
      if (lane < nqs) {
        float dsel = dot[0];
#pragma unroll
        for (int j = 1; j < kFbQueries; ++j) dsel = lane == j ? dot[j] : dsel;
        const float key = metric == 0 ? fmaxf(qnorm[lane] + xss[r] - 2.f * dsel, 0.f) : -dsel;
        const uint32_t kk = f2key(key);
        if (kk <= thr_key[lane]) {
          const int pos = atomicAdd(&cnt[lane], 1);
          if (pos < cap) buf[static_cast<size_t>(lane) * cap + pos] = (static_cast<unsigned long long>(kk) << 32) | static_cast<uint32_t>(r);
        }
      }
    };
    if (d <= 256) {
      for (int rr = 0; rr < 32; rr += 4) {
        const int64_t rb = r0 + warp * 32 + rr;
        if (rb >= row_hi) break;
        float x[4][8];
#pragma unroll
        for (int a = 0; a < 4; ++a) {
          const float* xv = X + min(rb + a, row_hi - 1) * ldx;
#pragma unroll
          for (int p = 0; p < 8; ++p) x[a][p] = lane + 32 * p < d ? __ldg(xv + lane + 32 * p) : 0.f;
        }
#pragma unroll
        for (int a = 0; a < 4; ++a) {
          float dot[kFbQueries];
#pragma unroll
          for (int j = 0; j < kFbQueries; ++j) {
            float t = 0.f;
#pragma unroll
            for (int p = 0; p < 8; ++p) t = fmaf(x[a][p], qreg[j][p], t);
#pragma unroll
            for (int o = 16; o > 0; o >>= 1) t += __shfl_xor_sync(0xffffffffu, t, o);
            dot[j] = t;
          }
          if (rb + a < row_hi) offer(rb + a, dot);
        }
      }
    } else {
      for (int rr = 0; rr < 32; ++rr) {
        const int64_t r = r0 + warp * 32 + rr;
        if (r >= row_hi) break;
        const float* xv = X + r * ldx;
        float dot[kFbQueries];
#pragma unroll
        for (int j = 0; j < kFbQueries; ++j) dot[j] = 0.f;
        for (int c = lane; c < d; c += 32) {
          const float x = __ldg(xv + c);
#pragma unroll
          for (int j = 0; j < kFbQueries; ++j) dot[j] = fmaf(x, qs[j * d + c], dot[j]);
        }
#pragma unroll
        for (int j = 0; j < kFbQueries; ++j) {
#pragma unroll
          for (int o = 16; o > 0; o >>= 1) dot[j] += __shfl_xor_sync(0xffffffffu, dot[j], o);
        }
        offer(r, dot);
      }
    }
    __syncthreads();
    unsigned int need = 0u;
    for (int j = 0; j < nqs; ++j) need |= (cnt[j] + kFbRound > cap ? 1u : 0u) << j;
    __syncthreads();
    for (int j = 0; j < nqs; ++j)
      if ((need >> j) & 1u) compact(j);
  }
  for (int j = 0; j < nqs; ++j) {
    compact(j);
    const int64_t q = compact_out ? static_cast<int64_t>(blockIdx.y) * nlist + q0 + j : qlist[q0 + j];
    const int have = cnt[j];
    for (int i = tid; i < k; i += kFbThreads) {
      if (i < have) {
        const unsigned long long e = buf[static_cast<size_t>(j) * cap + i];
        const float key = key2f(static_cast<uint32_t>(e >> 32));
        D[q * k + i] = metric == 0 ? key : -key;
        I[q * k + i] = static_cast<int64_t>(static_cast<uint32_t>(e)) + id_offset;
      } else {
        D[q * k + i] = metric == 0 ? pos_inf() : neg_inf();
        I[q * k + i] = -1;
      }
    }
    __syncthreads();
  }
}

__global__ void knn_scatter_rows_kernel(const int32_t* __restrict__ qlist, int nlist, int k, const float* __restrict__ Dm,
                                        const int64_t* __restrict__ Im, float* __restrict__ D, int64_t* __restrict__ I) {
  const int64_t i = static_cast<int64_t>(blockIdx.x) * blockDim.x + threadIdx.x;
  if (i >= static_cast<int64_t>(nlist) * k) return;
  const int64_t q = qlist[i / k];
  D[q * k + i % k] = Dm[i], I[q * k + i % k] = Im[i];
}

__global__ void __launch_bounds__(256)
knn_merge_kernel(const float* __restrict__ Dg, const int64_t* __restrict__ Ig, int G, int64_t nq, int k, int metric,
                 float* __restrict__ D, int64_t* __restrict__ I) {
  extern __shared__ unsigned long long mk[];
  const int64_t q = blockIdx.x;
  const int tid = threadIdx.x;
  const int n = G * k;
  int P = 2;
  while (P < n) P <<= 1;
  unsigned long long* key = mk;
  int* src = reinterpret_cast<int*>(mk + P);
  for (int i = tid; i < P; i += 256) {
    if (i < n) {
      const int g = i / k, j = i % k;
      const int64_t off = (static_cast<int64_t>(g) * nq + q) * k + j;
      const int64_t id = Ig[off];
      const float dv = Dg[off];
      key[i] = id < 0 ? ~0ull : ((static_cast<unsigned long long>(f2key(metric == 0 ? dv : -dv)) << 32) |
                                 static_cast<uint32_t>(id));
    } else {
      key[i] = ~0ull;
    }
    src[i] = i;
  }
  __syncthreads();
  for (int size = 2; size <= P; size <<= 1) {
    for (int stride = size >> 1; stride > 0; stride >>= 1) {
      for (int t = tid; t < (P >> 1); t += 256) {
        const int lo = ((t / stride) * (stride << 1)) + (t % stride);
        const int hi = lo + stride;
        const bool up = (lo & size) == 0;
        const unsigned long long a = key[lo], b = key[hi];
        if ((a > b) == up) {
          key[lo] = b, key[hi] = a;
          const int s = src[lo];
          src[lo] = src[hi], src[hi] = s;
        }
      }
      __syncthreads();
    }
  }
  for (int i = tid; i < k; i += 256) {
    const int s = src[i];
    if (key[i] != ~0ull && s < n) {
      const int g = s / k, j = s % k;
      const int64_t off = (static_cast<int64_t>(g) * nq + q) * k + j;
      D[q * k + i] = Dg[off];
      I[q * k + i] = Ig[off];
    } else {
      D[q * k + i] = metric == 0 ? pos_inf() : neg_inf();
      I[q * k + i] = -1;
    }
  }
}

__global__ void knn_any_overflow_kernel(const int32_t* __restrict__ overflow, int64_t n, const int32_t* __restrict__ log_overflow,
                                        int32_t* __restrict__ flag) {
  int any = (threadIdx.x == 0 && *log_overflow != 0) ? 1 : 0;
  for (int64_t i = threadIdx.x; i < n; i += blockDim.x) any |= overflow[i] != 0 ? 1 : 0;
  if (__syncthreads_or(any) && threadIdx.x == 0) *flag = 1;
}

__global__ void knn_pack_kernel(const float* __restrict__ D, const int64_t* __restrict__ I, int64_t n, int metric,
                                unsigned long long* __restrict__ rec) {
  const int64_t i = static_cast<int64_t>(blockIdx.x) * blockDim.x + threadIdx.x;
  if (i >= n) return;
  const int64_t id = I[i];
  const float dv = D[i];
  rec[i] = id < 0 ? ~0ull : ((static_cast<unsigned long long>(f2key(metric == 0 ? dv : -dv)) << 32) | static_cast<uint32_t>(id));
}

__global__ void knn_unpack_kernel(const unsigned long long* __restrict__ rec, int64_t n, int metric, float* __restrict__ D,
                                  int64_t* __restrict__ I) {
  const int64_t i = static_cast<int64_t>(blockIdx.x) * blockDim.x + threadIdx.x;
  if (i >= n) return;
  const unsigned long long e = rec[i];
  if (e == ~0ull) {
    D[i] = metric == 0 ? pos_inf() : neg_inf();
    I[i] = -1;
  } else {
    const float key = key2f(static_cast<uint32_t>(e >> 32));
    D[i] = metric == 0 ? key : -key;
    I[i] = static_cast<int64_t>(static_cast<uint32_t>(e));
  }
}

__global__ void __launch_bounds__(256)
knn_merge_packed_kernel(const unsigned long long* __restrict__ rec, int G, int64_t nq, int k, int metric, int warps,
                        float* __restrict__ D, int64_t* __restrict__ I, unsigned long long* __restrict__ rec_out) {
  extern __shared__ unsigned long long ms[];
  const int warp = threadIdx.x >> 5, lane = threadIdx.x & 31;
  if (warp >= warps) return;
  const int64_t q = static_cast<int64_t>(blockIdx.x) * warps + warp;
  if (q >= nq) return;
  unsigned long long* mine = ms + static_cast<size_t>(warp) * G * k;
  for (int g = 0; g < G; ++g)
    for (int j = lane; j < k; j += 32) mine[g * k + j] = rec[(static_cast<int64_t>(g) * nq + q) * k + j];
  __syncwarp();
  int pos = 0;
  unsigned long long head = lane < G ? mine[lane * k] : ~0ull;
  for (int i = 0; i < k; ++i) {
    const uint32_t hi = static_cast<uint32_t>(head >> 32);
    const uint32_t mhi = __reduce_min_sync(0xffffffffu, hi);
    const uint32_t lo = hi == mhi ? static_cast<uint32_t>(head) : 0xffffffffu;
    const uint32_t mlo = __reduce_min_sync(0xffffffffu, lo);
    const bool win = hi == mhi && static_cast<uint32_t>(head) == mlo && head != ~0ull;
    const unsigned int who = __ballot_sync(0xffffffffu, win);
    if (who == 0u) {
      if (lane == 0) {
        if (rec_out != nullptr) {
          rec_out[q * k + i] = ~0ull;
        } else {
          D[q * k + i] = metric == 0 ? pos_inf() : neg_inf();
          I[q * k + i] = -1;
        }
      }
      continue;
    }
    if (lane == __ffs(who) - 1) {
      if (rec_out != nullptr) {
        rec_out[q * k + i] = head;
      } else {
        const float key = key2f(mhi);
        D[q * k + i] = metric == 0 ? key : -key;
        I[q * k + i] = static_cast<int64_t>(mlo);
      }
      ++pos;
      head = pos < k ? mine[lane * k + pos] : ~0ull;
    }
  }
}

template <typename T>
static int dev_alloc(T** p, size_t n) {
  CDML_CHECK_CUDA(cudaMalloc(reinterpret_cast<void**>(p), n * sizeof(T)));
  return 0;
}

}

using namespace cdml;

struct cdml_index {
  cdml_ctx* ctx;
  int64_t N;
  int d, dpad, metric;
  float* x32;
  float* xss;
  float* h;
  uint16_t* x16;
  int64_t Ns;
  uint16_t* xs16;
  float* hs;
  float xmaxnorm;
  int64_t qc;
  uint16_t* q16;
  float *qss, *gmax, *thr, *cand_val;
  int32_t *cand_idx, *cnt, *overflow, *handled;
  uint4* log;
  int32_t* log_count;
  unsigned int log_cap;
  int32_t *h_cnt, *h_ovf, *h_logovf;
  float* h_qss;
  int64_t h_cap;
  int64_t ldg;
  int64_t stats[2];
  float* Dtmp;
  int64_t* Itmp;
  int64_t tmp_cap;
};

static void index_free(cdml_index* ix) {
  if (ix == nullptr) return;
  cudaFree(ix->x32), cudaFree(ix->xss), cudaFree(ix->h), cudaFree(ix->x16), cudaFree(ix->xs16), cudaFree(ix->hs);
  cudaFree(ix->q16), cudaFree(ix->qss), cudaFree(ix->gmax), cudaFree(ix->thr), cudaFree(ix->cand_val);
  cudaFree(ix->cand_idx), cudaFree(ix->cnt), cudaFree(ix->overflow), cudaFree(ix->handled);
  cudaFree(ix->log), cudaFree(ix->log_count);
  cudaFree(ix->Dtmp), cudaFree(ix->Itmp);
  cudaFreeHost(ix->h_cnt), cudaFreeHost(ix->h_ovf), cudaFreeHost(ix->h_qss), cudaFreeHost(ix->h_logovf);
  delete ix;
}

extern "C" {

int cdml_knn_index_build(cdml_ctx* ctx, const float* X, int64_t N, int d, int64_t ldx, int metric, void* stream,
                         cdml_index** out) {
  CDML_REQUIRE(ctx && X && out, "cdml_knn_index_build: NULL argument");
  CDML_REQUIRE(N > 0 && N < (1ll << 31) && d > 0 && ldx >= d && (metric == 0 || metric == 1),
               "cdml_knn_index_build: bad geometry N=%lld d=%d", (long long)N, d);
  cudaStream_t st = static_cast<cudaStream_t>(stream);
  cdml_index* ix = new cdml_index();
  memset(ix, 0, sizeof(*ix));
  ix->ctx = ctx, ix->N = N, ix->d = d, ix->dpad = (d + 7) / 8 * 8, ix->metric = metric;
  *out = nullptr;
  int rc = 0;
  rc |= dev_alloc(&ix->x32, static_cast<size_t>(N) * d);
  rc |= dev_alloc(&ix->xss, N + 1);
  rc |= dev_alloc(&ix->h, N);
  rc |= dev_alloc(&ix->x16, static_cast<size_t>(N) * ix->dpad);
  if (rc) { index_free(ix); return -2; }
  cudaError_t e = cudaMemcpy2DAsync(ix->x32, sizeof(float) * d, X, sizeof(float) * ldx, sizeof(float) * d, N,
                                    cudaMemcpyDeviceToDevice, st);
  if (e != cudaSuccess) { index_free(ix); set_error("index build copy failed: %s", cudaGetErrorString(e)); return -2; }
  const int grid = static_cast<int>(std::min<int64_t>((N + 7) / 8, ctx->num_sms * 8));
  row_sumsq32_kernel<<<grid, 256, 0, st>>>(ix->x32, N, d, d, ix->xss, metric == 0 ? 0.5f : 0.f, ix->h);
  max_reduce_kernel<<<1, 1024, 0, st>>>(ix->xss, N, ix->xss + N);
  rc = cdml_rows_normalize_cast(ctx, ix->x32, N, d, d, 0, 0.f, ix->x16, ix->dpad, CDML_F16, nullptr, 0, nullptr, stream);
  if (rc) { index_free(ix); return rc; }
  float maxss = 0.f;
  e = cudaMemcpyAsync(&maxss, ix->xss + N, sizeof(float), cudaMemcpyDeviceToHost, st);
  if (e == cudaSuccess) e = cudaStreamSynchronize(st);
  if (e != cudaSuccess) { index_free(ix); set_error("index build failed: %s", cudaGetErrorString(e)); return -2; }
  ix->xmaxnorm = sqrtf(maxss);
  if (N > kCandCap) {
    int64_t ns = std::max<int64_t>(N / 8, 4096);
    ns = std::min<int64_t>(std::min<int64_t>(ns, N), static_cast<int64_t>(kMaxGroups) * 32);
    ns = ns / 32 * 32;
    ix->Ns = ns;
    std::vector<int32_t> rows(ns);
    for (int64_t i = 0; i < ns; ++i) rows[i] = static_cast<int32_t>(i * N / ns);
    int32_t* drows = nullptr;
    rc |= dev_alloc(&drows, ns);
    rc |= dev_alloc(&ix->xs16, static_cast<size_t>(ns) * ix->dpad);
    rc |= dev_alloc(&ix->hs, ns);
    if (rc) { cudaFree(drows); index_free(ix); return -2; }
    cudaMemcpyAsync(drows, rows.data(), sizeof(int32_t) * ns, cudaMemcpyHostToDevice, st);
    rc = cdml_gather_rows(ctx, ix->x16, N, ix->dpad * 2, ix->dpad * 2, drows, 0, ns, ix->xs16, ix->dpad * 2, stream);
    if (!rc) rc = cdml_gather_rows(ctx, ix->h, N, 4, 4, drows, 0, ns, ix->hs, 4, stream);
    cudaStreamSynchronize(st);
    cudaFree(drows);
    if (rc) { index_free(ix); return rc; }
  }
  *out = ix;
  return 0;
}

int cdml_knn_index_destroy(cdml_index* index) {
  index_free(index);
  return 0;
}

int cdml_knn_last_stats(cdml_index* index, int64_t* stats) {
  CDML_REQUIRE(index && stats, "cdml_knn_last_stats: NULL argument");
  stats[0] = index->stats[0], stats[1] = index->stats[1];
  return 0;
}

static int ensure_workspace(cdml_index* ix, int64_t qc) {
  if (ix->qc >= qc) return 0;
  cudaFree(ix->q16), cudaFree(ix->qss), cudaFree(ix->gmax), cudaFree(ix->thr), cudaFree(ix->cand_val);
  cudaFree(ix->cand_idx), cudaFree(ix->cnt), cudaFree(ix->overflow), cudaFree(ix->log), cudaFree(ix->log_count);
  cudaFree(ix->handled);
  ix->handled = nullptr;
  ix->log = nullptr, ix->log_count = nullptr;
  ix->q16 = nullptr, ix->qss = ix->gmax = ix->thr = ix->cand_val = nullptr, ix->cand_idx = ix->cnt = ix->overflow = nullptr;
  ix->qc = 0;
  ix->ldg = ix->Ns > 0 ? ((ix->Ns / 32 + 7) / 8 * 8) : 8;
  int rc = 0;
  rc |= dev_alloc(&ix->q16, static_cast<size_t>(qc) * ix->dpad);
  rc |= dev_alloc(&ix->qss, qc);
  rc |= dev_alloc(&ix->gmax, static_cast<size_t>(qc) * ix->ldg);
  rc |= dev_alloc(&ix->thr, qc);
  rc |= dev_alloc(&ix->cand_val, static_cast<size_t>(qc) * kCandCap);
  rc |= dev_alloc(&ix->cand_idx, static_cast<size_t>(qc) * kCandCap);
  rc |= dev_alloc(&ix->cnt, qc);
  rc |= dev_alloc(&ix->overflow, qc);
  rc |= dev_alloc(&ix->handled, qc);
  const int sms = ix->ctx->num_sms;
  ix->log_cap = static_cast<unsigned int>(std::max<int64_t>(qc * 2048 / (sms * kKnnLogsPerCta), 16384));
  rc |= dev_alloc(&ix->log, static_cast<size_t>(sms) * kKnnLogsPerCta * ix->log_cap);
  rc |= dev_alloc(&ix->log_count, sms * kKnnLogsPerCta + 1);
  if (rc) return -2;
  ix->qc = qc;
  return 0;
}

static int knn_run(cdml_ctx* ctx, cdml_index* ix, const float* Q, int64_t nq, int64_t ldq, int k, float* D, int64_t* I,
                   int64_t id_offset, void* stream, const float* ext_full, const float* ext_part, int k_part,
                   float* out_full, float* out_part, int phase = 0, float part_sign = 1.f, float* nom_pair = nullptr,
                   const float* prune_pair = nullptr, int32_t* defer_flag = nullptr) {
  const bool bounds_only = out_full != nullptr;
  CDML_REQUIRE((phase == 0 && !(bounds_only && part_sign < 0.f)) || nq <= 65536,
               "cdml_knn_shard_*: one chunk of at most 65536 queries per call (got %lld)", (long long)nq);
  CDML_REQUIRE(ctx && ix && Q && (bounds_only || phase == 1 || (D && I)), "cdml_knn_search: NULL argument");
  CDML_REQUIRE(nq >= 0 && ldq >= ix->d && k >= 1 && k <= 1024, "cdml_knn_search: bad arguments (k=%d, supported 1..1024)", k);
  CDML_REQUIRE(k <= kKeepCap / 2, "cdml_knn_search: k=%d exceeds the re-rank capacity %d", k, kKeepCap / 2);
  if (nq == 0) return 0;
  cudaStream_t st = static_cast<cudaStream_t>(stream);
  const int64_t chunk = std::min<int64_t>(nq, (phase != 0 || (bounds_only && part_sign < 0.f)) ? 65536 : 32768);
  int rc = ensure_workspace(ix, chunk);
  if (rc) { set_error("cdml_knn_search: workspace allocation failed"); return rc; }
  if (phase != 2) ix->stats[0] = ix->stats[1] = 0;
  const int d = ix->d;
  const float rel = 1.5f * 0.0009765625f + 1.2e-7f * d;
  const float slack_scale = 2.f * rel * ix->xmaxnorm;
  const float slack_abs = 2.f * 1e-6f * (1.f + ix->xmaxnorm);
  if (ix->h_cap < nq) {
    cudaFreeHost(ix->h_cnt), cudaFreeHost(ix->h_ovf), cudaFreeHost(ix->h_qss), cudaFreeHost(ix->h_logovf);
    ix->h_cnt = ix->h_ovf = ix->h_logovf = nullptr, ix->h_qss = nullptr, ix->h_cap = 0;
    CDML_CHECK_CUDA(cudaMallocHost(reinterpret_cast<void**>(&ix->h_cnt), sizeof(int32_t) * nq));
    CDML_CHECK_CUDA(cudaMallocHost(reinterpret_cast<void**>(&ix->h_ovf), sizeof(int32_t) * nq));
    CDML_CHECK_CUDA(cudaMallocHost(reinterpret_cast<void**>(&ix->h_qss), sizeof(float) * nq));
    CDML_CHECK_CUDA(cudaMallocHost(reinterpret_cast<void**>(&ix->h_logovf), sizeof(int32_t) * (nq / chunk + 2)));
    ix->h_cap = nq;
  }
  for (int64_t q0 = 0; q0 < nq; q0 += chunk) {
    const int64_t qc = std::min<int64_t>(chunk, nq - q0);
    const float* Qc = Q + q0 * ldq;
    const bool tiny = ix->N <= kKeepCap;
    if (phase != 2) {
    rc = cdml_rows_normalize_cast(ctx, Qc, qc, d, ldq, 0, 0.f, ix->q16, ix->dpad, CDML_F16, nullptr, 0, nullptr, stream);
    if (rc) return rc;
    const int grid = static_cast<int>(std::min<int64_t>((qc + 7) / 8, ctx->num_sms * 8));
    row_sumsq32_kernel<<<grid, 256, 0, st>>>(Qc, qc, d, ldq, ix->qss, 0.f, nullptr);
    CDML_CHECK_CUDA(cudaMemsetAsync(ix->cnt, 0, sizeof(int32_t) * qc, st));
    CDML_CHECK_CUDA(cudaMemsetAsync(ix->overflow, 0, sizeof(int32_t) * qc, st));
    CDML_CHECK_CUDA(cudaMemsetAsync(ix->log_count, 0, sizeof(int32_t) * (ctx->num_sms * kKnnLogsPerCta + 1), st));
    if (bounds_only && (tiny || !(ix->Ns > 0 && ix->Ns / 32 >= k))) {
      fill_f32_kernel<<<64, 256, 0, st>>>(out_full + q0, qc, -INFINITY);
      fill_f32_kernel<<<64, 256, 0, st>>>(out_part + q0, qc, -INFINITY * part_sign);
      continue;
    }
    }
    if (!tiny) {
     if (phase != 2) {
      if (ext_full != nullptr) {
        knn_thr_combine_kernel<<<static_cast<int>((qc + 255) / 256), 256, 0, st>>>(ext_full + q0, ext_part + q0, ix->qss, qc,
                                                                                slack_scale, slack_abs, ix->thr, part_sign);
      } else if (ix->Ns > 0 && ix->Ns / 32 >= k) {
        const int wide = (ix->Ns / 128 >= 2 * static_cast<int64_t>(k)) ? 1 : 0;
        const int groups = wide ? static_cast<int>((ix->Ns + 255) / 256 * 2) : static_cast<int>(ix->Ns / 32);
        EpiKnnGroupMax<kBN> ea{ix->hs, ix->gmax, ix->ldg, wide};
        if (resb_applicable(ix->dpad) && qc >= 8 * kBM)
          rc = launch_gemm_resb(ctx, ix->q16, ix->dpad, ix->xs16, ix->dpad, qc, ix->Ns, ix->dpad, CDML_F16, ea, st);
        else
          rc = launch_gemm<0, 0>(ctx, ix->q16, ix->dpad, ix->xs16, ix->dpad, qc, ix->Ns, ix->dpad, CDML_F16, 1, ea, st);
        if (rc < 0) return rc;
        auto kth = [&](int kk, int kk2, float sc, float ab, float* out, float* out2) {
          const int grid = static_cast<int>(qc);
          if (groups <= 1024) {
            const int wgrid = static_cast<int>((qc + 7) / 8);
            if (out2) knn_kth_warp_kernel<true><<<wgrid, 256, 0, st>>>(ix->gmax, ix->ldg, groups, kk, kk2, ix->qss, qc, sc, ab, out, out2, part_sign);
            else knn_kth_warp_kernel<false><<<wgrid, 256, 0, st>>>(ix->gmax, ix->ldg, groups, kk, kk2, ix->qss, qc, sc, ab, out, out2, part_sign);
          } else if (groups <= 4 * kRefineThreads) {
            if (out2) knn_kth_kernel<4, true><<<grid, kRefineThreads, 0, st>>>(ix->gmax, ix->ldg, groups, kk, kk2, ix->qss, sc, ab, out, out2, part_sign);
            else knn_kth_kernel<4, false><<<grid, kRefineThreads, 0, st>>>(ix->gmax, ix->ldg, groups, kk, kk2, ix->qss, sc, ab, out, out2, part_sign);
          } else {
            constexpr int kP = kMaxGroups / kRefineThreads;
            if (out2) knn_kth_kernel<kP, true><<<grid, kRefineThreads, 0, st>>>(ix->gmax, ix->ldg, groups, kk, kk2, ix->qss, sc, ab, out, out2, part_sign);
            else knn_kth_kernel<kP, false><<<grid, kRefineThreads, 0, st>>>(ix->gmax, ix->ldg, groups, kk, kk2, ix->qss, sc, ab, out, out2, part_sign);
          }
        };
        if (bounds_only) {
          kth(k, std::max(1, std::min(k_part, k)), 0.f, 0.f, out_full + q0, out_part + q0);
          CDML_CHECK_CUDA(cudaGetLastError());
          continue;
        }
        kth(k, k, slack_scale, slack_abs, ix->thr, nullptr);
      } else {
        fill_f32_kernel<<<64, 256, 0, st>>>(ix->thr, qc, -INFINITY);
      }
      EpiKnnCollect<kBN> eb{ix->h, ix->thr, ix->log, ix->log_count, ix->log_count + ctx->num_sms * kKnnLogsPerCta, ix->log_cap};
      if (resb_applicable(ix->dpad) && ix->N >= 8 * kBM)
        rc = launch_gemm_resb(ctx, ix->x16, ix->dpad, ix->q16, ix->dpad, ix->N, qc, ix->dpad, CDML_F16, eb, st, 1);
      else
        rc = launch_gemm<0, 0>(ctx, ix->x16, ix->dpad, ix->q16, ix->dpad, ix->N, qc, ix->dpad, CDML_F16, 1, eb, st);
      if (rc < 0) return rc;
      knn_bin_kernel<<<dim3(4, ctx->num_sms * kKnnLogsPerCta), 256, 0, st>>>(ix->log, ix->log_count, ix->log_cap, ix->cand_idx, ix->cand_val,
                                                            ix->cnt, kCandCap);
     }
      if (phase == 1) {
        knn_nominee_kth_kernel<<<static_cast<int>((qc + 7) / 8), 256, 0, st>>>(ix->cand_val, ix->cnt, kCandCap, k,
                                                                              std::max(1, std::min(k_part, k)), qc, nom_pair);
        CDML_CHECK_CUDA(cudaGetLastError());
        continue;
      }
      if (prune_pair != nullptr)
        knn_refine_warp_kernel<<<static_cast<int>((qc + 7) / 8), 256, 0, st>>>(
            Qc, ldq, d, ix->qss, ix->x32, d, ix->xss, ix->cand_idx, ix->cand_val, ix->cnt, kCandCap, k, ix->metric,
            slack_scale, slack_abs, id_offset, D + q0 * k, I + q0 * k, k, prune_pair, qc, qc, ix->handled);
      knn_refine_kernel<<<static_cast<int>(qc), kRefineThreads, 0, st>>>(
          Qc, ldq, d, ix->qss, ix->x32, d, ix->xss, ix->cand_idx, ix->cand_val, ix->cnt, kCandCap, k, ix->metric,
          slack_scale, slack_abs, id_offset, D + q0 * k, I + q0 * k, k, ix->overflow, 0, prune_pair, qc,
          prune_pair != nullptr ? ix->handled : nullptr);
    } else {
      if (phase == 1) {
        fill_f32_kernel<<<64, 256, 0, st>>>(nom_pair, qc, -INFINITY);
        fill_f32_kernel<<<64, 256, 0, st>>>(nom_pair + qc, qc, INFINITY);
        CDML_CHECK_CUDA(cudaGetLastError());
        continue;
      }
      knn_refine_kernel<<<static_cast<int>(qc), kRefineThreads, 0, st>>>(
          Qc, ldq, d, ix->qss, ix->x32, d, ix->xss, ix->cand_idx, ix->cand_val, ix->cnt, kCandCap, k, ix->metric,
          slack_scale, slack_abs, id_offset, D + q0 * k, I + q0 * k, k, ix->overflow, static_cast<int>(ix->N), nullptr, 0, nullptr);
      ix->stats[0] += ix->N * qc;
    }
    CDML_CHECK_CUDA(cudaGetLastError());
    CDML_CHECK_CUDA(cudaMemcpyAsync(ix->h_cnt + q0, ix->cnt, sizeof(int32_t) * qc, cudaMemcpyDeviceToHost, st));
    CDML_CHECK_CUDA(cudaMemcpyAsync(ix->h_ovf + q0, ix->overflow, sizeof(int32_t) * qc, cudaMemcpyDeviceToHost, st));
    CDML_CHECK_CUDA(cudaMemcpyAsync(ix->h_qss + q0, ix->qss, sizeof(float) * qc, cudaMemcpyDeviceToHost, st));
    CDML_CHECK_CUDA(cudaMemcpyAsync(ix->h_logovf + q0 / chunk, ix->log_count + ctx->num_sms * kKnnLogsPerCta, sizeof(int32_t),
                                    cudaMemcpyDeviceToHost, st));
  }
  if (bounds_only || phase == 1) return 0;
  if (defer_flag != nullptr) {
    knn_any_overflow_kernel<<<1, 1024, 0, st>>>(ix->overflow, nq, ix->log_count + ctx->num_sms * kKnnLogsPerCta, defer_flag);
    CDML_CHECK_CUDA(cudaGetLastError());
    return 0;
  }
  CDML_CHECK_CUDA(cudaStreamSynchronize(st));
  std::vector<int32_t> redo;
  for (int64_t i = 0; i < nq; ++i) {
    ix->stats[0] += ix->N <= kKeepCap ? 0 : ix->h_cnt[i];
    if (ix->h_ovf[i] || ix->h_logovf[i / chunk]) redo.push_back(static_cast<int32_t>(i));
  }
  ix->stats[1] = static_cast<int64_t>(redo.size());
  if (!redo.empty()) {
    int kcap = 64;
    while (kcap < k) kcap <<= 1;
    kcap = std::max(kcap, kFbRound);
    const size_t smem = static_cast<size_t>(kFbQueries) * 2 * kcap * sizeof(unsigned long long) + static_cast<size_t>(kFbQueries) * d * sizeof(float);
    CDML_REQUIRE(smem <= 200 * 1024, "cdml_knn_search: exact fallback needs %zu bytes of shared memory (k=%d, d=%d)", smem, k, d);
    CDML_CHECK_CUDA(cudaFuncSetAttribute(knn_exact_batch_kernel, cudaFuncAttributeMaxDynamicSharedMemorySize, static_cast<int>(smem)));
    int32_t* dlist = nullptr;
    if (dev_alloc(&dlist, redo.size())) return -2;
    CDML_CHECK_CUDA(cudaMemcpyAsync(dlist, redo.data(), sizeof(int32_t) * redo.size(), cudaMemcpyHostToDevice, st));
    const int nlist = static_cast<int>(redo.size());
    const int blocks = (nlist + kFbQueries - 1) / kFbQueries;
    int splits = std::max(1, std::min(16, (2 * ctx->num_sms + blocks - 1) / blocks));
    if (ix->N < 64 * 1024) splits = 1;
    float* Dp = nullptr;
    int64_t* Ip = nullptr;
    if (splits > 1 && (dev_alloc(&Dp, static_cast<size_t>(splits + 1) * nlist * k) || dev_alloc(&Ip, static_cast<size_t>(splits + 1) * nlist * k))) {
      cudaFree(dlist), cudaFree(Dp);
      return -2;
    }
    knn_exact_batch_kernel<<<dim3(blocks, splits), kFbThreads, smem, st>>>(dlist, nlist, Q, ldq, d, ix->x32, ix->N, d, ix->xss,
                                                                          ix->metric, k, kcap, id_offset, splits > 1 ? Dp : D,
                                                                          splits > 1 ? Ip : I, splits > 1 ? 1 : 0);
    CDML_CHECK_CUDA(cudaGetLastError());
    if (splits > 1) {
      float* Dm = Dp + static_cast<size_t>(splits) * nlist * k;
      int64_t* Im = Ip + static_cast<size_t>(splits) * nlist * k;
      int rcm = cdml_knn_merge(ctx, Dp, Ip, splits, nlist, k, ix->metric, Dm, Im, stream);
      if (rcm) { cudaFree(dlist), cudaFree(Dp), cudaFree(Ip); return rcm; }
      const int64_t tot = static_cast<int64_t>(nlist) * k;
      knn_scatter_rows_kernel<<<static_cast<int>((tot + 255) / 256), 256, 0, st>>>(dlist, nlist, k, Dm, Im, D, I);
      CDML_CHECK_CUDA(cudaGetLastError());
    }
    CDML_CHECK_CUDA(cudaStreamSynchronize(st));
    cudaFree(dlist), cudaFree(Dp), cudaFree(Ip);
  }
  return 0;
}

int cdml_knn_search(cdml_ctx* ctx, cdml_index* ix, const float* Q, int64_t nq, int64_t ldq, int k, float* D,
                    int64_t* I, int64_t id_offset, void* stream) {
  return knn_run(ctx, ix, Q, nq, ldq, k, D, I, id_offset, stream, nullptr, nullptr, k, nullptr, nullptr);
}

int cdml_knn_bounds(cdml_ctx* ctx, cdml_index* ix, const float* Q, int64_t nq, int64_t ldq, int k_full, int k_part,
                    float* bound_full, float* bound_part, void* stream) {
  CDML_REQUIRE(bound_full && bound_part && k_part >= 1, "cdml_knn_bounds: NULL / bad argument");
  return knn_run(ctx, ix, Q, nq, ldq, k_full, nullptr, nullptr, 0, stream, nullptr, nullptr, k_part, bound_full, bound_part);
}

int cdml_knn_search_bounded(cdml_ctx* ctx, cdml_index* ix, const float* Q, int64_t nq, int64_t ldq, int k,
                            const float* bound_full, const float* bound_part, float* D, int64_t* I, int64_t id_offset,
                            void* stream) {
  CDML_REQUIRE(bound_full && bound_part, "cdml_knn_search_bounded: NULL bounds");
  return knn_run(ctx, ix, Q, nq, ldq, k, D, I, id_offset, stream, bound_full, bound_part, k, nullptr, nullptr);
}

int cdml_knn_shard_bounds(cdml_ctx* ctx, cdml_index* ix, const float* Q, int64_t nq, int64_t ldq, int k, int k_part,
                          float* pair, void* stream) {
  CDML_REQUIRE(pair && k_part >= 1, "cdml_knn_shard_bounds: NULL / bad argument");
  return knn_run(ctx, ix, Q, nq, ldq, k, nullptr, nullptr, 0, stream, nullptr, nullptr, k_part, pair, pair + nq, 0, -1.f);
}

int cdml_knn_shard_collect(cdml_ctx* ctx, cdml_index* ix, const float* Q, int64_t nq, int64_t ldq, int k, int k_part,
                           const float* pair, float* nom_pair, void* stream) {
  CDML_REQUIRE(pair && nom_pair && k_part >= 1, "cdml_knn_shard_collect: NULL / bad argument");
  return knn_run(ctx, ix, Q, nq, ldq, k, nullptr, nullptr, 0, stream, pair, pair + nq, k_part, nullptr, nullptr, 1, -1.f,
                 nom_pair);
}

int cdml_knn_shard_refine(cdml_ctx* ctx, cdml_index* ix, const float* Q, int64_t nq, int64_t ldq, int k,
                          const float* nom_pair, unsigned long long* rec, int64_t id_offset, int32_t* overflow_flag,
                          void* stream) {
  CDML_REQUIRE(ix && rec, "cdml_knn_shard_refine: NULL argument");
  CDML_REQUIRE(id_offset >= 0 && id_offset + ix->N <= (1ll << 32) - 1, "cdml_knn_shard_refine: global ids must fit 32 bits");
  if (ix->tmp_cap < nq * k) {
    cudaFree(ix->Dtmp), cudaFree(ix->Itmp);
    ix->Dtmp = nullptr, ix->Itmp = nullptr, ix->tmp_cap = 0;
    if (dev_alloc(&ix->Dtmp, static_cast<size_t>(nq) * k) || dev_alloc(&ix->Itmp, static_cast<size_t>(nq) * k)) return -2;
    ix->tmp_cap = nq * k;
  }
  int rc = knn_run(ctx, ix, Q, nq, ldq, k, ix->Dtmp, ix->Itmp, id_offset, stream, nullptr, nullptr, k, nullptr, nullptr, 2, -1.f,
                   nullptr, nom_pair, overflow_flag);
  if (rc) return rc;
  const int64_t n = nq * k;
  knn_pack_kernel<<<static_cast<unsigned>((n + 255) / 256), 256, 0, static_cast<cudaStream_t>(stream)>>>(ix->Dtmp, ix->Itmp, n, ix->metric, rec);
  CDML_CHECK_CUDA(cudaGetLastError());
  return 0;
}

int cdml_knn_unpack_records(cdml_ctx* ctx, const unsigned long long* rec, int64_t n, int metric, float* D, int64_t* I,
                            void* stream) {
  CDML_REQUIRE(ctx && rec && D && I && n >= 0, "cdml_knn_unpack_records: bad argument");
  if (n == 0) return 0;
  knn_unpack_kernel<<<static_cast<unsigned>((n + 255) / 256), 256, 0, static_cast<cudaStream_t>(stream)>>>(rec, n, metric, D, I);
  CDML_CHECK_CUDA(cudaGetLastError());
  return 0;
}

int cdml_knn_merge_packed(cdml_ctx* ctx, const unsigned long long* rec, int G, int64_t nq, int k, int metric, float* D,
                          int64_t* I, unsigned long long* rec_out, void* stream) {
  CDML_REQUIRE(ctx && rec && ((D && I) || rec_out) && G >= 1 && G <= 32 && k >= 1 && nq >= 0,
               "cdml_knn_merge_packed: bad argument (1 <= G <= 32)");
  if (nq == 0) return 0;
  const size_t per = static_cast<size_t>(G) * k * sizeof(unsigned long long);
  CDML_REQUIRE(per <= 200 * 1024, "cdml_knn_merge_packed: G*k=%d too large for one warp's staging", G * k);
  const int warps = static_cast<int>(std::max<size_t>(1, std::min<size_t>(8, (96 * 1024) / per)));
  const size_t smem = per * warps;
  if (smem > 48 * 1024)
    CDML_CHECK_CUDA(cudaFuncSetAttribute(knn_merge_packed_kernel, cudaFuncAttributeMaxDynamicSharedMemorySize, static_cast<int>(smem)));
  knn_merge_packed_kernel<<<static_cast<unsigned>((nq + warps - 1) / warps), 256, smem, static_cast<cudaStream_t>(stream)>>>(
      rec, G, nq, k, metric, warps, D, I, rec_out);
  CDML_CHECK_CUDA(cudaGetLastError());
  return 0;
}

int cdml_knn_merge(cdml_ctx* ctx, const float* Dg, const int64_t* Ig, int G, int64_t nq, int k, int metric, float* D,
                   int64_t* I, void* stream) {
  CDML_REQUIRE(ctx && Dg && Ig && D && I && G >= 1 && k >= 1 && nq >= 0, "cdml_knn_merge: bad argument");
  if (nq == 0) return 0;
  int P = 2;
  while (P < G * k) P <<= 1;
  const size_t smem = static_cast<size_t>(P) * (sizeof(unsigned long long) + sizeof(int));
  CDML_REQUIRE(smem <= 200 * 1024, "cdml_knn_merge: G*k=%d too large for one block", G * k);
  if (smem > 48 * 1024)
    CDML_CHECK_CUDA(cudaFuncSetAttribute(knn_merge_kernel, cudaFuncAttributeMaxDynamicSharedMemorySize, static_cast<int>(smem)));
  knn_merge_kernel<<<static_cast<unsigned>(nq), 256, smem, static_cast<cudaStream_t>(stream)>>>(Dg, Ig, G, nq, k, metric, D, I);
  CDML_CHECK_CUDA(cudaGetLastError());
  return 0;
}

}
```

collaborative-deep-metric-learning_b200/csrc/mine.cu:

```cuda
#include <algorithm>

#include "gemm_launch.cuh"

namespace cdml {

constexpr unsigned long long kNoCand = ~0ull;
constexpr int kMassHits = 4;

static int epi_warps() {
  static int w = -1;
  if (w < 0) {
    const char* e = getenv("CDML_MINE_EPI_WARPS");
    w = (e != nullptr && e[0] == '1') ? 16 : 8;
  }
  return w;
}

template <int BN, int kVariant = 0>
struct EpiMine {
  static constexpr bool kSplitColumns = true;
  static constexpr bool kPrefetchNext = (kVariant & 1) == 0;
  static constexpr bool kRowConsts = (kVariant & 4) != 0;
  struct State {
    float dpi, bound_d;
    int ga, gp;
    uint32_t bound_row;
    uint32_t release_bar;
  };
  static constexpr bool kEarlyRelease = true;
  static constexpr bool kTmaStore = false;
  const float* dp;
  const int32_t* guid;
  unsigned long long* best;
  int cand;
  unsigned long long* stats;
  __device__ __forceinline__ void row_consts(int row, const GemmShape& s, uint32_t dst) const {
    const bool row_ok = row < s.M;
    const uint32_t inf = 0x7f800000u;
    const uint32_t dpi = row_ok ? __float_as_uint(__ldg(dp + row)) : inf;
    const uint32_t ga = row_ok ? static_cast<uint32_t>(__ldg(guid + 3 * row)) : 0u;
    const uint32_t gp = row_ok ? static_cast<uint32_t>(__ldg(guid + 3 * row + 1)) : 0u;
    const unsigned long long key = row_ok ? *(reinterpret_cast<volatile unsigned long long*>(best) + row) : ~0ull;
    sts128(dst, dpi, ga, gp, static_cast<uint32_t>(key >> 32));
    asm volatile("st.shared.b32 [%0], %1;" ::"r"(dst + 16), "r"(static_cast<uint32_t>(key)) : "memory");
  }
  __device__ __forceinline__ void load_state(State& st, uint32_t src) const {
    const uint4 v = lds128(src);
    st.dpi = __uint_as_float(v.x), st.ga = static_cast<int>(v.y), st.gp = static_cast<int>(v.z), st.bound_d = __uint_as_float(v.w);
    asm volatile("ld.shared.b32 %0, [%1];" : "=r"(st.bound_row) : "r"(src + 16) : "memory");
    st.release_bar = 0u;
  }
  __device__ __forceinline__ void pre(State& st, int row, int , const GemmShape& s, int, int, uint32_t) const {
    const bool row_ok = row < s.M;
    const float inf = __int_as_float(0x7f800000);
    st.dpi = row_ok ? __ldg(dp + row) : inf;
    st.ga = row_ok ? __ldg(guid + 3 * row) : 0;
    st.gp = row_ok ? __ldg(guid + 3 * row + 1) : 0;
    const unsigned long long key = row_ok ? best[row] : ~0ull;
    st.bound_d = __uint_as_float(static_cast<uint32_t>(key >> 32));
    st.bound_row = static_cast<uint32_t>(key);
    st.release_bar = 0u;
  }
  __device__ __forceinline__ void cols(int n0, const GemmShape& s, int c0, int , uint32_t stg) const {
    static_assert(BN == 256, "a warp owns 4 chunks (128 columns) of the tile");
    col_cache_fill(stg, n0, c0, [&](int col) { return static_cast<uint32_t>(col < s.N ? __ldg(guid + 3 * col + cand) : -1); });
  }
  __device__ __forceinline__ void block_begin(uint32_t epi_smem) const { col_cache_reset(epi_smem); }
  __device__ __forceinline__ void block_end(uint32_t) const {}
  __device__ __forceinline__ void run(uint32_t taddr, int row, int n0, int , const GemmShape& s, int c0,
                                      int c1, uint32_t stg, State& st) const {
    const int lane = threadIdx.x & 31;
    const bool row_ok = row < s.M;
    const float inf = __int_as_float(0x7f800000);
    const float dpi = st.dpi;
    const float s_hi = row_ok ? 1.f - 0.5f * dpi : -inf;
    const int ga = st.ga, gp = st.gp;
    float bound_d = st.bound_d;
    if (!(bound_d == bound_d)) bound_d = inf;
    float s_lo = 1.f - 0.5f * bound_d;
    uint32_t brow = st.bound_row;
    float bd = inf;
    int br = -1;
    uint32_t va[32], vb[32];
    auto chunk = [&](const uint32_t (&v)[32], int cc) {
      const int nb = n0 + (c0 + cc) * 32;
      uint32_t u0 = 0xffffffffu, u1 = 0xffffffffu;
#pragma unroll
      for (int j = 0; j < 8; ++j) {
        const float2 lo = sub2(s_hi, s_hi, __uint_as_float(v[4 * j]), __uint_as_float(v[4 * j + 1]));
        const float2 hi = sub2(s_hi, s_hi, __uint_as_float(v[4 * j + 2]), __uint_as_float(v[4 * j + 3]));
        u0 = umin3(u0, __float_as_uint(lo.x), __float_as_uint(lo.y));
        u1 = umin3(u1, __float_as_uint(hi.x), __float_as_uint(hi.y));
      }
      const uint32_t mu = min(u0, u1), thr = __float_as_uint(s_hi - s_lo);
      unsigned int hits = __ballot_sync(0xffffffffu, mu < thr || (mu == thr && static_cast<uint32_t>(3 * nb + cand) < brow));
      if (hits != 0u && __popc(hits) >= kMassHits) {
        if (lane == 0) atomicAdd(stats, static_cast<unsigned long long>(__popc(hits)));
        if ((hits >> lane) & 1u) {
          uint32_t kbest = 0xffffffffu;
          int cbest = -1;
#pragma unroll
          for (int j = 0; j < 32; ++j) {
            int g;
            asm volatile("ld.shared.b32 %0, [%1];" : "=r"(g) : "r"(stg + kColCacheOff + 128 * cc + 4 * j) : "memory");
            const float sc = __uint_as_float(v[j]);
            const float d = fmaxf(fmaf(-2.f, sc, 2.f), 0.f);
            const bool pass = sc < s_hi && sc >= s_lo && d > dpi && d < bd && g != ga && g != gp && g >= 0;
            if (pass && __float_as_uint(d) < kbest) kbest = __float_as_uint(d), cbest = j;
          }
          if (cbest >= 0) {
            bd = __uint_as_float(kbest), br = 3 * (nb + cbest) + cand;
            const float s_new = 1.f - 0.5f * bd;
            if (s_new > s_lo || (s_new == s_lo && static_cast<uint32_t>(br) < brow)) brow = static_cast<uint32_t>(br);
            s_lo = fmaxf(s_lo, s_new);
          }
        }
        __syncwarp();
      } else if (hits != 0u) {
        if (lane == 0) atomicAdd(stats, static_cast<unsigned long long>(__popc(hits)));
        int g_lane;
        asm volatile("ld.shared.b32 %0, [%1];" : "=r"(g_lane) : "r"(stg + kColCacheOff + 128 * cc + 4 * lane) : "memory");
        do {
          const int src = __ffs(hits) - 1;
          hits &= hits - 1u;
          __syncwarp();
          if (lane == src) {
#pragma unroll
            for (int j = 0; j < 8; ++j) sts128(stg + 16 * j, v[4 * j], v[4 * j + 1], v[4 * j + 2], v[4 * j + 3]);
          }
          __syncwarp();
          float sc;
          asm volatile("ld.shared.f32 %0, [%1];" : "=f"(sc) : "r"(stg + 4 * lane) : "memory");
          const float hi_s = __shfl_sync(0xffffffffu, s_hi, src), lo_s = __shfl_sync(0xffffffffu, s_lo, src);
          const float dp_s = __shfl_sync(0xffffffffu, dpi, src), bd_s = __shfl_sync(0xffffffffu, bd, src);
          const int ga_s = __shfl_sync(0xffffffffu, ga, src), gp_s = __shfl_sync(0xffffffffu, gp, src);
          const float d = fmaxf(fmaf(-2.f, sc, 2.f), 0.f);
          const bool pass = sc < hi_s && sc >= lo_s && d > dp_s && d < bd_s && g_lane != ga_s && g_lane != gp_s && g_lane >= 0;
          const uint32_t kmin = __reduce_min_sync(0xffffffffu, pass ? __float_as_uint(d) : 0xffffffffu);
          if (kmin != 0xffffffffu) {
            const int col = __ffs(__ballot_sync(0xffffffffu, pass && __float_as_uint(d) == kmin)) - 1;
            if (lane == src) {
              bd = __uint_as_float(kmin), br = 3 * (nb + col) + cand;
              const float s_new = 1.f - 0.5f * bd;
              if (s_new > s_lo || (s_new == s_lo && static_cast<uint32_t>(br) < brow)) brow = static_cast<uint32_t>(br);
              s_lo = fmaxf(s_lo, s_new);
            }
          }
        } while (hits != 0u);
      }
    };
    auto ok = [&](int cc) { return c0 + cc < c1 && n0 + (c0 + cc) * 32 < s.N; };
    if constexpr ((kVariant & 2) == 0) {
      tmem_ld_32x32(taddr + c0 * 32, va);
#pragma unroll
      for (int cc = 0; cc < 4; cc += 2) {
        tmem_ld_wait();
        if (ok(cc + 1)) tmem_ld_32x32(taddr + (c0 + cc + 1) * 32, vb);
        if (ok(cc)) chunk(va, cc);
        tmem_ld_wait();
        if (cc + 2 < 4 && ok(cc + 2)) tmem_ld_32x32(taddr + (c0 + cc + 2) * 32, va);
        if (cc + 2 >= 4 && st.release_bar != 0u) {
          tc_fence_before();
          __syncwarp();
          if (lane == 0) mbar_arrive(st.release_bar);
        }
        if (ok(cc + 1)) chunk(vb, cc + 1);
      }
    } else {
#pragma unroll
      for (int cc = 0; cc < 4; ++cc) {
        if (ok(cc)) {
          tmem_ld_32x32(taddr + (c0 + cc) * 32, va);
          tmem_ld_wait();
          chunk(va, cc);
        }
      }
      if (st.release_bar != 0u) {
        tc_fence_before();
        __syncwarp();
        if (lane == 0) mbar_arrive(st.release_bar);
      }
    }
    if (br >= 0)
      atomicMin(best + row, (static_cast<unsigned long long>(__float_as_uint(bd)) << 32) | static_cast<uint32_t>(br));
  }
};

__global__ void mine_prepare_kernel(const float* __restrict__ E, int64_t ld, int D, const int64_t* __restrict__ guid64,
                                    int64_t B, float* __restrict__ dp, int32_t* __restrict__ guid32,
                                    unsigned long long* __restrict__ best, unsigned long long* __restrict__ stats) {
  const int warp = threadIdx.x >> 5, lane = threadIdx.x & 31;
  if (blockIdx.x == 0 && threadIdx.x < 2) stats[threadIdx.x] = 0ull;
  for (int64_t i = static_cast<int64_t>(blockIdx.x) * 8 + warp; i < B; i += static_cast<int64_t>(gridDim.x) * 8) {
    const float* a = E + 3 * i * ld;
    const float* p = a + ld;
    float s = 0.f;
    for (int j = lane; j < D; j += 32) {
      const float t = a[j] - p[j];
      s = fmaf(t, t, s);
    }
#pragma unroll
    for (int o = 16; o > 0; o >>= 1) s += __shfl_xor_sync(0xffffffffu, s, o);
    if (lane == 0) dp[i] = s, best[i] = kNoCand;
    if (lane < 3) guid32[3 * i + lane] = static_cast<int32_t>(guid64[3 * i + lane]);
  }
}

__global__ void mine_finalize_kernel(const float* __restrict__ E, int64_t ld, int D,
                                     const unsigned long long* __restrict__ best, int64_t B,
                                     int32_t* __restrict__ neg_row, float* __restrict__ d_an,
                                     unsigned long long* __restrict__ stats) {
  const int warp = threadIdx.x >> 5, lane = threadIdx.x & 31;
  unsigned int mined = 0;
  for (int64_t i = static_cast<int64_t>(blockIdx.x) * 8 + warp; i < B; i += static_cast<int64_t>(gridDim.x) * 8) {
    const unsigned long long kb = best[i];
    const int r = kb != kNoCand ? static_cast<int>(static_cast<uint32_t>(kb)) : static_cast<int>(3 * i + 2);
    mined += kb != kNoCand ? 1u : 0u;
    if (lane == 0) neg_row[i] = r;
    if (d_an != nullptr) {
      const float* a = E + 3 * i * ld;
      const float* n = E + static_cast<int64_t>(r) * ld;
      float s = 0.f;
      for (int j = lane; j < D; j += 32) {
        const float t = a[j] - n[j];
        s = fmaf(t, t, s);
      }
#pragma unroll
      for (int o = 16; o > 0; o >>= 1) s += __shfl_xor_sync(0xffffffffu, s, o);
      if (lane == 0) d_an[i] = s;
    }
  }
  if (lane == 0 && mined != 0u) atomicAdd(stats + 1, static_cast<unsigned long long>(mined));
}

}

using namespace cdml;

extern "C" int cdml_mine_semihard(cdml_ctx* ctx, const void* E16, int64_t ld16, int dtype16, const float* E32,
                                  int64_t ld32, const int64_t* guid, int64_t B, int D, float margin, int32_t* neg_row,
                                  float* d_an, void* stream) {
  CDML_REQUIRE(ctx && E16 && E32 && guid && neg_row, "cdml_mine_semihard: NULL argument");
  CDML_REQUIRE(B > 0 && 3 * B < (1ll << 31) && D > 0 && D % 8 == 0 && ld16 >= D && ld32 >= D,
               "cdml_mine_semihard: bad geometry B=%lld D=%d", (long long)B, D);
  cudaStream_t st = static_cast<cudaStream_t>(stream);
  const size_t bytes = static_cast<size_t>(B) * (8 + 4 + 12) + 64;
  uint8_t* ws = static_cast<uint8_t*>(ctx_scratch(ctx, bytes));
  if (ws == nullptr) return -2;
  if (ctx->mine_stats == nullptr) CDML_CHECK_CUDA(cudaMalloc(&ctx->mine_stats, 2 * sizeof(unsigned long long)));
  unsigned long long* stats = ctx->mine_stats;
  unsigned long long* best = reinterpret_cast<unsigned long long*>(ws);
  float* dp = reinterpret_cast<float*>(best + B);
  int32_t* guid32 = reinterpret_cast<int32_t*>(dp + B);
  const int grid = static_cast<int>(std::min<int64_t>((B + 7) / 8, ctx->num_sms * 8));
  mine_prepare_kernel<<<grid, 256, 0, st>>>(E32, ld32, D, guid, B, dp, guid32, best, stats);
  int rc = 0;
  const uint16_t* e16 = static_cast<const uint16_t*>(E16);
  for (int cand = 1; cand <= 2 && rc >= 0; ++cand) {
    EpiMine<kBN, 1> epi{dp, guid32, best, cand, stats};
    static int rowc = -1;
    if (rowc < 0) rowc = getenv("CDML_MINE_ROWCONSTS") != nullptr ? 1 : 0;
    if (resb_applicable(D) && B >= 8 * kBM && rowc) {
      EpiMine<kBN, 5> epi5{dp, guid32, best, cand, stats};
      rc = launch_gemm_resb(ctx, e16, 3 * ld16, e16 + cand * ld16, 3 * ld16, B, B, D, dtype16, epi5, st);
    } else if (resb_applicable(D) && B >= 8 * kBM && epi_warps() == 16)
      rc = launch_gemm_resb<EpiMine<kBN, 1>, 16>(ctx, e16, 3 * ld16, e16 + cand * ld16, 3 * ld16, B, B, D, dtype16, epi, st);
    else if (resb_applicable(D) && B >= 8 * kBM)
      rc = launch_gemm_resb(ctx, e16, 3 * ld16, e16 + cand * ld16, 3 * ld16, B, B, D, dtype16, epi, st);
    else
      rc = launch_gemm<0, 0>(ctx, e16, 3 * ld16, e16 + cand * ld16, 3 * ld16, B, B, D, dtype16, 1, epi, st);
  }
  if (rc >= 0) {
    mine_finalize_kernel<<<grid, 256, 0, st>>>(E32, ld32, D, best, B, neg_row, d_an, stats);
    rc = cudaGetLastError() == cudaSuccess ? 0 : -2;
  }
  return rc < 0 ? rc : 0;
}

extern "C" int cdml_mine_last_stats(cdml_ctx* ctx, int64_t* out2, void* stream) {
  CDML_REQUIRE(ctx && out2, "cdml_mine_last_stats: NULL argument");
  out2[0] = out2[1] = 0;
  if (ctx->mine_stats == nullptr) return 0;
  cudaStream_t st = static_cast<cudaStream_t>(stream);
  unsigned long long h[2];
  CDML_CHECK_CUDA(cudaMemcpyAsync(h, ctx->mine_stats, sizeof(h), cudaMemcpyDeviceToHost, st));
  CDML_CHECK_CUDA(cudaStreamSynchronize(st));
  out2[0] = static_cast<int64_t>(h[0]), out2[1] = static_cast<int64_t>(h[1]);
  return 0;
}
```

collaborative-deep-metric-learning_b200/ops.py:

```python
import ctypes

import torch

from . import _lib
from ._lib import BF16, EPI_L2NORM, EPI_MASK_BITS, EPI_MASK_LEAKY, EPI_STORE_16, EPI_STORE_F32, F16, check, ptr, stream_ptr

TORCH16 = {F16: torch.float16, BF16: torch.bfloat16}

_LAUNCHES = 0


def _count(n):
  global _LAUNCHES
  _LAUNCHES += n


def launch_count():
  return _LAUNCHES


def _ctx(t):
  return _lib.context(t.device.index if t.device.index is not None else torch.cuda.current_device())


def dtype16_of(t):
  if t.dtype == torch.float16:
    return F16
  if t.dtype == torch.bfloat16:
    return BF16
  raise TypeError("expected a float16/bfloat16 tensor, got %s" % t.dtype)


def _row_major_2d(t, name):
  if t.dim() != 2 or t.stride(1) != 1:
    raise ValueError("%s must be a 2-D tensor with unit inner stride" % name)
  return t.stride(0)


def poll_errors(device_tensor):
  flags = ctypes.c_int32(0)
  check(_lib.load().cdml_ctx_poll_errors(_ctx(device_tensor), stream_ptr(), ctypes.byref(flags)))
  return flags.value


def gather_rows(table, idx, out=None):
  pitch = _row_major_2d(table, "table") * table.element_size()
  flat = idx.reshape(-1)
  if flat.dtype not in (torch.int32, torch.int64):
    raise TypeError("idx must be int32 or int64")
  flat = flat.contiguous()
  row_bytes = table.shape[1] * table.element_size()
  if out is None:
    out = torch.empty((flat.numel(), table.shape[1]), dtype=table.dtype, device=table.device)
  if flat.numel() == 0:
    return out
  out_pitch = _row_major_2d(out, "out") * out.element_size()
  _count(1)
  check(_lib.load().cdml_gather_rows(_ctx(table), ptr(table), table.shape[0], row_bytes, pitch, ptr(flat),
                                     int(flat.dtype == torch.int64), flat.numel(), ptr(out), out_pitch, stream_ptr()))
  return out


def rows_normalize_cast(x, dtype16=F16, normalize=1, eps=1e-12, ld_out=None, want_fp32=False, want_sumsq=False,
                        out16=None):
  ld_in = _row_major_2d(x, "x")
  n, F = x.shape
  if ld_out is None:
    ld_out = (F + 7) // 8 * 8
  if out16 is None:
    out16 = torch.empty((n, ld_out), dtype=TORCH16[dtype16], device=x.device)
  out32 = torch.empty((n, F), dtype=torch.float32, device=x.device) if want_fp32 else None
  sumsq = torch.empty((n,), dtype=torch.float32, device=x.device) if want_sumsq else None
  _count(1)
  check(_lib.load().cdml_rows_normalize_cast(_ctx(x), ptr(x), n, F, ld_in, normalize, eps, ptr(out16), out16.stride(0),
                                             dtype16, ptr(out32), F, ptr(sumsq), stream_ptr()))
  return out16, out32, sumsq


def gemm16(A, B, M, N, K, a_mn_major, b_mn_major, epilogue, out, bias=None, alpha=1.0, aux0=None, aux1=None,
           num_splits=1, split_stride=0, ld_out=None):
  lda, ldb = _row_major_2d(A, "A"), _row_major_2d(B, "B")
  used = ctypes.c_int(0)
  if ld_out is None:
    ld_out = out.stride(-2) if out.dim() >= 2 else N
  ld_aux1 = aux1.stride(0) if aux1 is not None else (aux0.stride(0) if (epilogue == EPI_STORE_16 and aux0 is not None) else 0)
  _count(1)
  check(_lib.load().cdml_gemm16(_ctx(A), ptr(A), int(a_mn_major), lda, ptr(B), int(b_mn_major), ldb, M, N, K,
                                dtype16_of(A), epilogue, ptr(out), ld_out, ptr(bias), float(alpha), ptr(aux0),
                                ptr(aux1), ld_aux1, num_splits, split_stride,
                                ctypes.byref(used), stream_ptr()))
  return used.value


def sign_mask_buffer(rows, cols, device):
  return torch.empty(((cols + 31) // 32, rows), dtype=torch.int32, device=device)


def auto_splits(ref, M, N, K):
  return _lib.load().cdml_gemm16_auto_splits(_ctx(ref), M, N, K)


def sum_partials(parts, num_parts, stride, n, out, scale=1.0):
  _count(1)
  check(_lib.load().cdml_sum_partials(_ctx(parts), ptr(parts), num_parts, stride, n, float(scale), ptr(out), stream_ptr()))
  return out


def colsum16(X, R, N, out, workspace=None):
  need = _lib.load().cdml_colsum_workspace_floats(R, N)
  if workspace is None or workspace.numel() < need:
    workspace = torch.empty((need,), dtype=torch.float32, device=X.device)
  _count(2)
  check(_lib.load().cdml_colsum16(_ctx(X), ptr(X), R, N, X.stride(0), dtype16_of(X), ptr(workspace), ptr(out), stream_ptr()))
  return out


def colsum_workspace_floats(R, N):
  return _lib.load().cdml_colsum_workspace_floats(R, N)


def triplet_hinge(E, B, margin, neg_row=None, grad_scale=1.0, rinv=None, leaky_alpha=0.2, want_dE=False, dz16=None,
                  workspace=None, out=None):
  D = E.shape[1]
  dev = E.device
  out = out or {}
  pos = out.get("pos_dist") if "pos_dist" in out else torch.empty((B,), dtype=torch.float32, device=dev)
  neg = out.get("neg_dist") if "neg_dist" in out else torch.empty((B,), dtype=torch.float32, device=dev)
  hin = out.get("hinge_dist") if "hinge_dist" in out else torch.empty((B,), dtype=torch.float32, device=dev)
  stats = out.get("stats") if "stats" in out else torch.empty((4,), dtype=torch.float32, device=dev)
  dE = None
  if want_dE:
    dE = out.get("dE") if "dE" in out else torch.empty_like(E)
  if dz16 is not None and dE is None and workspace is None:
    workspace = torch.empty((3 * B * E.stride(0),), dtype=torch.float32, device=dev)
  mined_grad = neg_row is not None and (dE is not None or dz16 is not None)
  _count(2 + (2 if mined_grad else 0) + (1 if dz16 is not None else 0))
  check(_lib.load().cdml_triplet_hinge(_ctx(E), ptr(E), B, D, E.stride(0), ptr(neg_row), float(margin), float(grad_scale),
                                       ptr(rinv), float(leaky_alpha), ptr(pos), ptr(neg), ptr(hin), ptr(stats), ptr(dE),
                                       ptr(dz16), dz16.stride(0) if dz16 is not None else 0,
                                       dtype16_of(dz16) if dz16 is not None else F16, ptr(workspace), stream_ptr()))
  return {"pos_dist": pos, "neg_dist": neg, "hinge_dist": hin, "stats": stats, "dE": dE, "dz16": dz16}


def adam_prepare(step_counter, scalars, base_lr, decay_steps=1e6, decay_rate=0.96, staircase=True, beta1=0.9,
                 beta2=0.999):
  _count(1)
  check(_lib.load().cdml_adam_prepare(_ctx(scalars), ptr(step_counter), float(base_lr), float(decay_steps),
                                      float(decay_rate), int(staircase), float(beta1), float(beta2), ptr(scalars),
                                      stream_ptr()))


def adam_apply(w, m, v, g, scalars, beta1=0.9, beta2=0.999, eps=1e-8, grad_scale=1.0, w16=None):
  _count(1)
  check(_lib.load().cdml_adam_apply(_ctx(w), ptr(w), ptr(m), ptr(v), ptr(g), w.numel(), ptr(scalars), float(beta1),
                                    float(beta2), float(eps), float(grad_scale), ptr(w16),
                                    dtype16_of(w16) if w16 is not None else F16, stream_ptr()))


OPT_ADAM, OPT_MOMENTUM, OPT_LARS, OPT_SGD = 0, 1, 2, 3


def opt_workspace_floats():
  return int(_lib.load().cdml_opt_workspace_floats())


def opt_sumsq(g, w, out2, workspace, grad_scale=1.0, wd_reg=0.0):
  _count(2)
  check(_lib.load().cdml_opt_sumsq(_ctx(w), ptr(g), ptr(w), w.numel(), float(grad_scale), float(wd_reg), ptr(workspace),
                                   ptr(out2), stream_ptr()))
  return out2


def opt_apply(kind, w, m, v, g, scalars, norms=None, beta1=0.9, beta2=0.999, eps=1e-8, grad_scale=1.0, wd_reg=0.0,
              clip_norm=0.0, momentum=0.9, lars_weight_decay=1e-4, lars_eeta=1e-3, w16=None):
  _count(1)
  check(_lib.load().cdml_opt_apply(_ctx(w), int(kind), ptr(w), ptr(m), ptr(v), ptr(g), w.numel(), ptr(scalars), ptr(norms),
                                   float(beta1), float(beta2), float(eps), float(grad_scale), float(wd_reg), float(clip_norm),
                                   float(momentum), float(lars_weight_decay), float(lars_eeta), ptr(w16),
                                   dtype16_of(w16) if w16 is not None else F16, stream_ptr()))


EW_MUL, EW_ADD, EW_MUL_ADD_BOTH, EW_MASK, EW_MUL_ADD, EW_FMA, EW_MUL_ADD_MASK, EW_MUL_MASK = 0, 1, 2, 3, 4, 5, 6, 7


def ew16(op, a, b, out, c=None, alpha=0.2):
  rows, cols = out.shape
  _count(1)
  check(_lib.load().cdml_ew16(_ctx(out), int(op), ptr(a), a.stride(0), ptr(b), b.stride(0), ptr(c),
                              c.stride(0) if c is not None else 0, ptr(out), out.stride(0), rows, cols, float(alpha),
                              dtype16_of(out), stream_ptr()))
  return out


def rows_l2norm16(y16, e, rinv=None, e16=None, eps=1e-12):
  n, D = y16.shape
  _count(1)
  check(_lib.load().cdml_rows_l2norm16(_ctx(y16), ptr(y16), n, D, y16.stride(0), float(eps), dtype16_of(y16), ptr(e),
                                       e.stride(0), ptr(rinv), ptr(e16), e16.stride(0) if e16 is not None else 0,
                                       stream_ptr()))
  return e


def cast16(x, out16):
  _count(1)
  check(_lib.load().cdml_cast16(_ctx(x), ptr(x), x.numel(), ptr(out16), dtype16_of(out16), stream_ptr()))
  return out16


def fill_column16(X16, col, value):
  if X16.dim() != 2 or X16.stride(1) != 1 or not (0 <= col < X16.stride(0)):
    raise ValueError("fill_column16: column %d outside the row pitch" % col)
  _count(1)
  check(_lib.load().cdml_fill_column16(_ctx(X16), ptr(X16), X16.shape[0], X16.stride(0), int(col), float(value),
                                       dtype16_of(X16), stream_ptr()))


def sample_triplets(pairs, start, B, num_guid, seed, out=None):
  if pairs.dtype != torch.int64 or pairs.dim() != 2 or pairs.shape[1] != 2 or not pairs.is_contiguous():
    raise TypeError("pairs must be a contiguous int64 [n,2] tensor")
  if out is None:
    out = torch.empty((B, 3), dtype=torch.int64, device=pairs.device)
  if B == 0:
    return out
  _count(1)
  check(_lib.load().cdml_sample_triplets(_ctx(pairs), ptr(pairs), pairs.shape[0], int(start), int(B), int(num_guid),
                                         int(seed) & 0xFFFFFFFFFFFFFFFF, ptr(out), stream_ptr()))
  return out


def desim(eI, fI, fD=None, fD_threshold=1.4, f_end=31, out=None, row_offset=0):
  if eI.dtype != torch.int64 or fI.dtype != torch.int64 or (fD is not None and fD.dtype != torch.float32):
    raise TypeError("desim: eI / fI must be int64, fD float32")
  n, ke = eI.shape
  nf, kf = fI.shape
  lib = _lib.load()
  ws = torch.empty((max(int(lib.cdml_desim_workspace_bytes(nf, kf, int(f_end))), 4),), dtype=torch.uint8, device=eI.device)
  if out is None:
    out = torch.empty_like(eI)
  if n == 0:
    return out
  _count(2)
  check(lib.cdml_desim(_ctx(eI), ptr(eI), n, ke, _row_major_2d(eI, "eI"), ptr(fI), ptr(fD), nf, kf, _row_major_2d(fI, "fI"),
                       _row_major_2d(fD, "fD") if fD is not None else 0, float(fD_threshold), int(f_end), ptr(ws), ptr(out),
                       _row_major_2d(out, "out"), int(row_offset), stream_ptr()))
  return out


def filter_fI(fI, fD, fD_threshold=1.4):
  nf, kf = fI.shape
  probe = torch.full((1, 1), -1, dtype=torch.int64, device=fI.device)
  lib = _lib.load()
  ws = torch.empty((int(lib.cdml_desim_workspace_bytes(nf, kf, kf)),), dtype=torch.uint8, device=fI.device)
  _count(2)
  check(lib.cdml_desim(_ctx(fI), ptr(probe), 1, 1, 1, ptr(fI), ptr(fD), nf, kf, _row_major_2d(fI, "fI"),
                       _row_major_2d(fD, "fD"), float(fD_threshold), kf, ptr(ws), ptr(probe), 1, 0, stream_ptr()))
  return ws.view(torch.int32).view(nf, -1)[:, :kf]


def desim_simple(eI, fI, out=None):
  n, ke = eI.shape
  if out is None:
    out = torch.empty_like(eI)
  _count(1)
  check(_lib.load().cdml_desim_simple(_ctx(eI), ptr(eI), n, ke, _row_major_2d(eI, "eI"), ptr(fI), fI.shape[1],
                                      _row_major_2d(fI, "fI"), ptr(out), _row_major_2d(out, "out"), stream_ptr()))
  return out


def mean_pair_dist(V, pairs):
  out = torch.empty((1,), dtype=torch.float32, device=V.device)
  pairs = pairs.to(torch.int64).contiguous()
  _count(2)
  check(_lib.load().cdml_mean_pair_dist(_ctx(V), ptr(V), V.stride(0), V.shape[1], ptr(pairs), pairs.shape[0], ptr(out),
                                        stream_ptr()))
  return out


def mine_semihard(E16, E32, guid, B, margin, want_dist=True):
  D = E32.shape[1]
  neg_row = torch.empty((B,), dtype=torch.int32, device=E32.device)
  d_an = torch.empty((B,), dtype=torch.float32, device=E32.device) if want_dist else None
  guid = guid.to(torch.int64).contiguous()
  _count(4)
  check(_lib.load().cdml_mine_semihard(_ctx(E32), ptr(E16), E16.stride(0), dtype16_of(E16), ptr(E32), E32.stride(0),
                                       ptr(guid), B, D, float(margin), ptr(neg_row), ptr(d_an), stream_ptr()))
  return neg_row, d_an


def mine_stats(ref):
  out = (ctypes.c_int64 * 2)()
  check(_lib.load().cdml_mine_last_stats(_ctx(ref), out, stream_ptr()))
  return {"rescans": int(out[0]), "mined": int(out[1])}


class FlatIndex(object):

  def __init__(self, xb, metric="L2"):
    if xb.dtype != torch.float32 or xb.dim() != 2 or not xb.is_cuda:
      raise TypeError("FlatIndex needs a CUDA float32 [N,d] tensor")
    self.metric = {"L2": _lib.METRIC_L2, "IP": _lib.METRIC_IP}[metric]
    self.n, self.d = xb.shape
    self._ref = xb
    self._h = ctypes.c_void_p()
    _count(5)
    check(_lib.load().cdml_knn_index_build(_ctx(xb), ptr(xb), self.n, self.d, _row_major_2d(xb, "xb"), self.metric,
                                           stream_ptr(), ctypes.byref(self._h)))

  def search(self, xq, k, id_offset=0):
    if xq.dtype != torch.float32 or xq.dim() != 2 or xq.shape[1] != self.d:
      raise TypeError("queries must be float32 [nq,%d]" % self.d)
    nq = xq.shape[0]
    D = torch.empty((nq, k), dtype=torch.float32, device=xq.device)
    I = torch.empty((nq, k), dtype=torch.int64, device=xq.device)
    _count(6 * ((nq + 32767) // 32768))
    check(_lib.load().cdml_knn_search(_ctx(xq), self._h, ptr(xq), nq, _row_major_2d(xq, "xq"), k, ptr(D), ptr(I),
                                      int(id_offset), stream_ptr()))
    return D, I

  def bounds(self, xq, k_full, k_part):
    nq = xq.shape[0]
    bf = torch.empty((nq,), dtype=torch.float32, device=xq.device)
    bp = torch.empty((nq,), dtype=torch.float32, device=xq.device)
    _count(4 * ((nq + 32767) // 32768))
    check(_lib.load().cdml_knn_bounds(_ctx(xq), self._h, ptr(xq), nq, _row_major_2d(xq, "xq"), int(k_full), int(k_part),
                                      ptr(bf), ptr(bp), stream_ptr()))
    return bf, bp

  def search_bounded(self, xq, k, bound_full, bound_part, id_offset=0):
    nq = xq.shape[0]
    D = torch.empty((nq, k), dtype=torch.float32, device=xq.device)
    I = torch.empty((nq, k), dtype=torch.int64, device=xq.device)
    _count(5 * ((nq + 32767) // 32768))
    check(_lib.load().cdml_knn_search_bounded(_ctx(xq), self._h, ptr(xq), nq, _row_major_2d(xq, "xq"), k, ptr(bound_full),
                                              ptr(bound_part), ptr(D), ptr(I), int(id_offset), stream_ptr()))
    return D, I

  CHUNK = 65536

  def shard_bounds(self, xq, k, k_part, pair=None):
    nq = xq.shape[0]
    if pair is None:
      pair = torch.empty((2, nq), dtype=torch.float32, device=xq.device)
    _count(4)
    check(_lib.load().cdml_knn_shard_bounds(_ctx(xq), self._h, ptr(xq), nq, _row_major_2d(xq, "xq"), int(k), int(k_part),
                                            ptr(pair), stream_ptr()))
    return pair

  def shard_collect(self, xq, k, k_part, pair, nom_pair=None):
    nq = xq.shape[0]
    if nom_pair is None:
      nom_pair = torch.empty((2, nq), dtype=torch.float32, device=xq.device)
    _count(6)
    check(_lib.load().cdml_knn_shard_collect(_ctx(xq), self._h, ptr(xq), nq, _row_major_2d(xq, "xq"), int(k), int(k_part),
                                             ptr(pair), ptr(nom_pair), stream_ptr()))
    return nom_pair

  def shard_refine(self, xq, k, nom_pair, rec, id_offset=0, overflow_flag=None):
    nq = xq.shape[0]
    _count(3)
    check(_lib.load().cdml_knn_shard_refine(_ctx(xq), self._h, ptr(xq), nq, _row_major_2d(xq, "xq"), int(k), ptr(nom_pair),
                                            ptr(rec), int(id_offset), ptr(overflow_flag), stream_ptr()))
    return rec

  def last_stats(self):
    s = (ctypes.c_int64 * 2)()
    check(_lib.load().cdml_knn_last_stats(self._h, s))
    return {"candidates": int(s[0]), "fallback_queries": int(s[1])}

  def close(self):
    if self._h:
      _lib.load().cdml_knn_index_destroy(self._h)
      self._h = ctypes.c_void_p()

  def __del__(self):
    try:
      self.close()
    except Exception:
      pass


def knn_merge_packed(rec, metric="L2", as_records=False):
  G, nq, k = rec.shape
  rec = rec.contiguous()
  m = {"L2": 0, "IP": 1}[metric]
  _count(1)
  if as_records:
    out = torch.empty((nq, k), dtype=torch.int64, device=rec.device)
    check(_lib.load().cdml_knn_merge_packed(_ctx(rec), ptr(rec), G, nq, k, m, None, None, ptr(out), stream_ptr()))
    return out
  D = torch.empty((nq, k), dtype=torch.float32, device=rec.device)
  I = torch.empty((nq, k), dtype=torch.int64, device=rec.device)
  check(_lib.load().cdml_knn_merge_packed(_ctx(rec), ptr(rec), G, nq, k, m, ptr(D), ptr(I), None, stream_ptr()))
  return D, I


def knn_unpack_records(rec, metric="L2"):
  rec = rec.contiguous()
  D = torch.empty(rec.shape, dtype=torch.float32, device=rec.device)
  I = torch.empty(rec.shape, dtype=torch.int64, device=rec.device)
  _count(1)
  check(_lib.load().cdml_knn_unpack_records(_ctx(rec), ptr(rec), rec.numel(), {"L2": 0, "IP": 1}[metric], ptr(D), ptr(I),
                                            stream_ptr()))
  return D, I


def knn_merge(Dg, Ig, metric="L2"):
  G, nq, k = Dg.shape
  Dg, Ig = Dg.contiguous(), Ig.contiguous()
  D = torch.empty((nq, k), dtype=torch.float32, device=Dg.device)
  I = torch.empty((nq, k), dtype=torch.int64, device=Dg.device)
  _count(1)
  check(_lib.load().cdml_knn_merge(_ctx(Dg), ptr(Dg), ptr(Ig), G, nq, k, {"L2": 0, "IP": 1}[metric], ptr(D), ptr(I),
                                   stream_ptr()))
  return D, I
```

Before: 5.791 million.

## Fuse both mining candidate scans into one 2-CTA paired tcgen05 kernel

```diff
diff --git a/collaborative-deep-metric-learning_b200/csrc/gemm_launch.cuh b/collaborative-deep-metric-learning_b200/csrc/gemm_launch.cuh
--- a/collaborative-deep-metric-learning_b200/csrc/gemm_launch.cuh
+++ b/collaborative-deep-metric-learning_b200/csrc/gemm_launch.cuh
@@ -149,10 +149,10 @@
   return off == 0 && K <= 4 * kBK;
 }
 
-template <class Epi, int kEpiWarps = 8>
+template <class Epi>
 static int launch_gemm_resb(cdml_ctx* ctx, const void* A, int64_t lda, const void* B, int64_t ldb, int64_t M, int64_t N,
                             int64_t K, int dtype16, const Epi& epi, cudaStream_t stream, int n_fastest = 0) {
-  using L = ResBSmem<kBN, kResBStages, kEpiWarps, Epi::kRowConsts, Epi::kTmaStore ? 2 : 1>;
+  using L = ResBSmem<kBN, kResBStages, Epi::kTmaStore ? 2 : 1>;
   static_assert(L::kTotal <= 232448, "resident-B kernel: shared memory over the 227 KB limit");
   CUtensorMap ta, tb;
   int rc = make_tmap_2d(ctx, &ta, A, dtype16, K, M, lda, kBK, kBM);
@@ -181,7 +181,7 @@
   s.tiles_per_chunk = (s.m_tiles + best - 1) / best;
   s.n_fastest = n_fastest;
   s.idesc = make_idesc_f16(dtype16 == CDML_BF16 ? 1 : 0, 0, 0, kBM, kBN);
-  auto kern = gemm_resb_tcgen05_kernel<kBN, kResBStages, Epi, kEpiWarps>;
+  auto kern = gemm_resb_tcgen05_kernel<kBN, kResBStages, Epi>;
   static bool attr_set = false;
   if (!attr_set) {
     CDML_CHECK_CUDA(cudaFuncSetAttribute(kern, cudaFuncAttributeMaxDynamicSharedMemorySize, L::kTotal));
@@ -189,7 +189,7 @@
   }
   const long units = static_cast<long>(s.n_tiles) * s.m_chunks;
   const int grid = static_cast<int>(units < ctx->num_sms ? units : ctx->num_sms);
-  kern<<<grid, 128 + 32 * kEpiWarps, L::kTotal, stream>>>(ta, tb, s, epi);
+  kern<<<grid, kGemmThreads, L::kTotal, stream>>>(ta, tb, s, epi);
   CDML_CHECK_CUDA(cudaGetLastError());
   if (trace_sync("gemm_resb", M, N, K, grid, stream)) return -2;
   return 1;
diff --git a/collaborative-deep-metric-learning_b200/csrc/gemm_sm100.cuh b/collaborative-deep-metric-learning_b200/csrc/gemm_sm100.cuh
--- a/collaborative-deep-metric-learning_b200/csrc/gemm_sm100.cuh
+++ b/collaborative-deep-metric-learning_b200/csrc/gemm_sm100.cuh
@@ -123,7 +123,6 @@
   struct State {};
   __device__ __forceinline__ void pre(State&, int, int, const GemmShape&, int, int, uint32_t) const {}
   static constexpr bool kPrefetchNext = false;
-  static constexpr bool kRowConsts = false;
   static constexpr bool kEarlyRelease = false;
   static constexpr bool kTmaStore = false;
   __device__ __forceinline__ void cols(int, const GemmShape&, int, int, uint32_t) const {}
@@ -170,7 +169,6 @@
   struct State {};
   __device__ __forceinline__ void pre(State&, int, int, const GemmShape&, int, int, uint32_t) const {}
   static constexpr bool kPrefetchNext = false;
-  static constexpr bool kRowConsts = false;
   static constexpr bool kEarlyRelease = false;
   static constexpr bool kTmaStore = false;
   __device__ __forceinline__ void cols(int, const GemmShape&, int, int, uint32_t) const {}
@@ -213,7 +211,6 @@
   struct State {};
   __device__ __forceinline__ void pre(State&, int, int, const GemmShape&, int, int, uint32_t) const {}
   static constexpr bool kPrefetchNext = false;
-  static constexpr bool kRowConsts = false;
   static constexpr bool kEarlyRelease = false;
   static constexpr bool kTmaStore = false;
   __device__ __forceinline__ void cols(int, const GemmShape&, int, int, uint32_t) const {}
@@ -275,7 +272,6 @@
     uint4 raw[4][4];
   };
   static constexpr bool kPrefetchNext = false;
-  static constexpr bool kRowConsts = false;
   static constexpr bool kEarlyRelease = false;
   static constexpr bool kTmaStore = false;
   __device__ __forceinline__ void cols(int, const GemmShape&, int, int, uint32_t) const {}
@@ -364,7 +360,6 @@
     uint32_t bits[4];
   };
   static constexpr bool kPrefetchNext = true;
-  static constexpr bool kRowConsts = false;
   static constexpr bool kEarlyRelease = false;
   static constexpr bool kTmaStore = false;
   __device__ __forceinline__ void cols(int, const GemmShape&, int, int, uint32_t) const {}
@@ -420,7 +415,6 @@
     uint32_t release_bar;
   };
   static constexpr bool kPrefetchNext = true;
-  static constexpr bool kRowConsts = false;
   static constexpr bool kEarlyRelease = true;
   static constexpr bool kTmaStore = true;
   __device__ __forceinline__ void cols(int, const GemmShape&, int, int, uint32_t) const {}
@@ -491,7 +485,6 @@
   struct State {};
   __device__ __forceinline__ void pre(State&, int, int, const GemmShape&, int, int, uint32_t) const {}
   static constexpr bool kPrefetchNext = false;
-  static constexpr bool kRowConsts = false;
   static constexpr bool kEarlyRelease = false;
   static constexpr bool kTmaStore = false;
   __device__ __forceinline__ void cols(int, const GemmShape&, int, int, uint32_t) const {}
@@ -671,27 +664,23 @@
   uint32_t idesc;
 };
 
-template <int BN, int kAStages, int kEpiWarps = 8, bool kRowSlots = false, int kStageSlices = 1>
+template <int BN, int kAStages, int kStageSlices = 1>
 struct ResBSmem {
   static constexpr uint32_t kABytes = kBM * kBK * 2;
   static constexpr uint32_t kBPanel = BN * kBK * 2;
   static constexpr uint32_t kMaxKb = 4;
   static constexpr uint32_t kEpiOff = kMaxKb * kBPanel + kAStages * kABytes;
-  static constexpr uint32_t kEpiBytes = kEpiWarps * 2048 * kStageSlices;
-  static constexpr uint32_t kRowConstOff = kEpiOff + kEpiBytes;
-  static constexpr uint32_t kRowConstSlot = kRowSlots ? kBM * 32 : 0;
-  static constexpr uint32_t kBarOff = kRowConstOff + 2 * kRowConstSlot;
-  static constexpr uint32_t kNumBars = 2 * kAStages + 2 + 4 + 2;
+  static constexpr uint32_t kEpiBytes = 8 * 2048 * kStageSlices;
+  static constexpr uint32_t kBarOff = kEpiOff + kEpiBytes;
+  static constexpr uint32_t kNumBars = 2 * kAStages + 2 + 4;
   static constexpr uint32_t kTotal = kBarOff + kNumBars * 8 + 16 + 1024;
 };
 
-template <int BN, int kAStages, class Epi, int kEpiWarps = 8>
-__global__ void __launch_bounds__(128 + 32 * kEpiWarps, 1)
+template <int BN, int kAStages, class Epi>
+__global__ void __launch_bounds__(kGemmThreads, 1)
 gemm_resb_tcgen05_kernel(const __grid_constant__ CUtensorMap tma_a, const __grid_constant__ CUtensorMap tma_b,
                          const ResBShape s, const __grid_constant__ Epi epi) {
-  using L = ResBSmem<BN, kAStages, kEpiWarps, Epi::kRowConsts, Epi::kTmaStore ? 2 : 1>;
-  static_assert(kEpiWarps == 8 || kEpiWarps == 16, "two or four epilogue warps per TMEM lane quarter");
-  static_assert(kEpiWarps == 8 || Epi::kSplitColumns, "four warps per quarter split the tile's columns");
+  using L = ResBSmem<BN, kAStages, Epi::kTmaStore ? 2 : 1>;
   extern __shared__ uint8_t smem_raw[];
   const uint32_t raw_u32 = smem_u32(smem_raw);
   const uint32_t base = (raw_u32 + 1023u) & ~1023u;
@@ -704,8 +693,6 @@
   const uint32_t b_empty = bar0 + 8u * (2 * kAStages + 1);
   auto tfull_bar = [&](int i) { return bar0 + 8u * (2 * kAStages + 2 + i); };
   auto tempty_bar = [&](int i) { return bar0 + 8u * (2 * kAStages + 4 + i); };
-  auto cfull_bar = [&](int i) { return bar0 + 8u * (2 * kAStages + 6 + i); };
-  auto cslot = [&](int i) { return base + L::kRowConstOff + i * L::kRowConstSlot; };
   const uint32_t tmem_slot = bar0 + 8u * L::kNumBars;
   volatile uint32_t* tmem_slot_ptr = reinterpret_cast<volatile uint32_t*>(smem_raw + (tmem_slot - raw_u32));
   const int warp = threadIdx.x >> 5;
@@ -726,8 +713,7 @@
     mbar_init(b_empty, 1);
     for (int i = 0; i < 2; ++i) {
       mbar_init(tfull_bar(i), 1);
-      mbar_init(tempty_bar(i), kEpiWarps);
-      mbar_init(cfull_bar(i), 1);
+      mbar_init(tempty_bar(i), 8);
     }
     fence_mbar_init();
   }
@@ -794,29 +780,10 @@
       }
       tc_commit(b_empty);
     }
-  } else if (warp == 3) {
-   if constexpr (Epi::kRowConsts) {
-    int it = 0;
-    GemmShape gs;
-    gs.M = s.M, gs.N = s.N, gs.K = s.K;
-    for (int u = blockIdx.x; u < units; u += gridDim.x) {
-      const int chunk = s.n_fastest ? u / s.n_tiles : u % s.m_chunks;
-      const int t0 = chunk * s.tiles_per_chunk, t1 = min(s.m_tiles, t0 + s.tiles_per_chunk);
-      for (int t = t0; t < t1; ++t, ++it) {
-        const int as = it & 1;
-        const uint32_t ap = (it >> 1) & 1;
-        mbar_wait(tempty_bar(as), ap ^ 1, 700 + as);
-#pragma unroll
-        for (int r = lane; r < kBM; r += 32) epi.row_consts(t * kBM + r, gs, cslot(as) + r * 32);
-        __syncwarp();
-        if (lane == 0) mbar_arrive(cfull_bar(as));
-      }
-    }
-   }
   } else if (warp >= 4) {
     const int q = warp & 3;
     const int half = (warp - 4) >> 2;
-    const uint32_t stg = base + L::kEpiOff + (warp - 4) * (Epi::kTmaStore ? 4096u : (Epi::kSplitColumns || kEpiWarps == 16) ? 2048u : 4096u);
+    const uint32_t stg = base + L::kEpiOff + (warp - 4) * ((Epi::kTmaStore || !Epi::kSplitColumns) ? 4096u : 2048u);
     int it = 0;
     GemmShape gs;
     gs.M = s.M, gs.N = s.N, gs.K = s.K, gs.m_tiles = s.m_tiles, gs.n_tiles = s.n_tiles, gs.num_kb = s.num_kb;
@@ -837,15 +804,14 @@
       }
     };
     const bool active = Epi::kSplitColumns || half == 0;
-    constexpr int kChunksPerWarp = (BN / 32) / (kEpiWarps / 4);
-    const int ec0 = Epi::kSplitColumns ? half * kChunksPerWarp : 0, ec1 = Epi::kSplitColumns ? (half + 1) * kChunksPerWarp : BN / 32;
+    const int ec0 = Epi::kSplitColumns ? half * (BN / 64) : 0, ec1 = Epi::kSplitColumns ? (half + 1) * (BN / 64) : BN / 32;
     TileIter cur;
     cur.u = blockIdx.x;
     seek(cur);
     typename Epi::State est;
     if (cur.valid && active) {
       epi.cols(cur.nblk * BN, gs, ec0, ec1, stg);
-      if constexpr (!Epi::kRowConsts) epi.pre(est, cur.t * kBM + q * 32 + lane, cur.nblk * BN, gs, ec0, ec1, stg);
+      epi.pre(est, cur.t * kBM + q * 32 + lane, cur.nblk * BN, gs, ec0, ec1, stg);
     }
     while (cur.valid) {
       TileIter nxt = cur;
@@ -856,17 +822,11 @@
       const int as = it & 1;
       const uint32_t ap = (it >> 1) & 1;
       typename Epi::State est_next;
-      if constexpr (Epi::kRowConsts) {
-        mbar_wait(cfull_bar(as), ap, 800 + as);
-        if (active) epi.load_state(est, cslot(as) + (q * 32 + lane) * 32);
-        est_next = est;
-      }
       mbar_wait(tfull_bar(as), ap, 400 + as);
       tc_fence_after();
       const uint32_t taddr = tmem_base + (static_cast<uint32_t>(q * 32) << 16) + as * BN;
       if (active) {
-        if constexpr (!Epi::kRowConsts)
-          if (Epi::kPrefetchNext && nxt.valid) epi.pre(est_next, nxt.t * kBM + q * 32 + lane, nxt.nblk * BN, gs, ec0, ec1, stg);
+        if (Epi::kPrefetchNext && nxt.valid) epi.pre(est_next, nxt.t * kBM + q * 32 + lane, nxt.nblk * BN, gs, ec0, ec1, stg);
         if constexpr (Epi::kEarlyRelease) est.release_bar = tempty_bar(as);
         epi.run(taddr, cur.t * kBM + q * 32 + lane, cur.nblk * BN, 0, gs, ec0, ec1, stg, est);
       }
@@ -877,8 +837,7 @@
       }
       if (active && nxt.valid) {
         epi.cols(nxt.nblk * BN, gs, ec0, ec1, stg);
-        if constexpr (!Epi::kRowConsts)
-          if (!Epi::kPrefetchNext) epi.pre(est_next, nxt.t * kBM + q * 32 + lane, nxt.nblk * BN, gs, ec0, ec1, stg);
+        if (!Epi::kPrefetchNext) epi.pre(est_next, nxt.t * kBM + q * 32 + lane, nxt.nblk * BN, gs, ec0, ec1, stg);
       }
       est = est_next;
       cur = nxt;
diff --git a/collaborative-deep-metric-learning_b200/csrc/knn.cu b/collaborative-deep-metric-learning_b200/csrc/knn.cu
--- a/collaborative-deep-metric-learning_b200/csrc/knn.cu
+++ b/collaborative-deep-metric-learning_b200/csrc/knn.cu
@@ -38,7 +38,6 @@
 struct EpiKnnGroupMax {
   static constexpr bool kSplitColumns = true;
   static constexpr bool kPrefetchNext = false;
-  static constexpr bool kRowConsts = false;
   static constexpr bool kEarlyRelease = false;
   static constexpr bool kTmaStore = false;
   struct State {};
@@ -106,7 +105,6 @@
     uint32_t release_bar;
   };
   static constexpr bool kPrefetchNext = true;
-  static constexpr bool kRowConsts = false;
   static constexpr bool kEarlyRelease = true;
   static constexpr bool kTmaStore = false;
   __device__ __forceinline__ void block_begin(uint32_t epi_smem) const {
diff --git a/collaborative-deep-metric-learning_b200/csrc/mine.cu b/collaborative-deep-metric-learning_b200/csrc/mine.cu
--- a/collaborative-deep-metric-learning_b200/csrc/mine.cu
+++ b/collaborative-deep-metric-learning_b200/csrc/mine.cu
@@ -7,59 +7,118 @@
 constexpr unsigned long long kNoCand = ~0ull;
 constexpr int kMassHits = 4;
 
-static int epi_warps() {
-  static int w = -1;
-  if (w < 0) {
-    const char* e = getenv("CDML_MINE_EPI_WARPS");
-    w = (e != nullptr && e[0] == '1') ? 16 : 8;
-  }
-  return w;
-}
-
-template <int BN, int kVariant = 0>
+struct MineRow {
+  float dpi, s_hi;
+  int ga, gp;
+  float s_lo;
+  uint32_t brow;
+  unsigned long long key;
+  uint32_t rescans;
+};
+
+__device__ __forceinline__ void mine_row_seed(MineRow& r, int row, int B, const float* dp, const int32_t* guid,
+                                              const unsigned long long* best) {
+  const bool row_ok = row < B;
+  const float inf = __int_as_float(0x7f800000);
+  r.dpi = row_ok ? __ldg(dp + row) : inf;
+  r.s_hi = row_ok ? 1.f - 0.5f * r.dpi : -inf;
+  r.ga = row_ok ? __ldg(guid + 3 * row) : 0;
+  r.gp = row_ok ? __ldg(guid + 3 * row + 1) : 0;
+  const unsigned long long key = row_ok ? __ldcg(best + row) : kNoCand;
+  float bound_d = __uint_as_float(static_cast<uint32_t>(key >> 32));
+  if (!(bound_d == bound_d)) bound_d = inf;
+  r.s_lo = 1.f - 0.5f * bound_d;
+  r.brow = static_cast<uint32_t>(key);
+  r.key = kNoCand;
+}
+
+__device__ __forceinline__ void mine_flush_rescans(MineRow& r, unsigned long long* stats) {
+  const uint32_t n = __reduce_add_sync(0xffffffffu, r.rescans);
+  if ((threadIdx.x & 31) == 0 && n != 0u) atomicAdd(stats, static_cast<unsigned long long>(n));
+  r.rescans = 0;
+}
+
+__device__ __forceinline__ void mine_take(MineRow& r, uint32_t dbits, uint32_t row) {
+  const unsigned long long k = (static_cast<unsigned long long>(dbits) << 32) | row;
+  if (k < r.key) {
+    r.key = k;
+    const float s_new = 1.f - 0.5f * __uint_as_float(dbits);
+    if (s_new > r.s_lo || (s_new == r.s_lo && row < r.brow)) r.brow = row;
+    r.s_lo = fmaxf(r.s_lo, s_new);
+  }
+}
+
+__device__ __forceinline__ void mine_chunk(const uint32_t (&v)[32], int nb, int cand, uint32_t gcache, uint32_t stg,
+                                           MineRow& r) {
+  const int lane = threadIdx.x & 31;
+  const float s_hi = r.s_hi;
+  uint32_t u0 = 0xffffffffu, u1 = 0xffffffffu;
+#pragma unroll
+  for (int j = 0; j < 8; ++j) {
+    const float2 lo = sub2(s_hi, s_hi, __uint_as_float(v[4 * j]), __uint_as_float(v[4 * j + 1]));
+    const float2 hi = sub2(s_hi, s_hi, __uint_as_float(v[4 * j + 2]), __uint_as_float(v[4 * j + 3]));
+    u0 = umin3(u0, __float_as_uint(lo.x), __float_as_uint(lo.y));
+    u1 = umin3(u1, __float_as_uint(hi.x), __float_as_uint(hi.y));
+  }
+  const uint32_t mu = min(u0, u1), thr = __float_as_uint(s_hi - r.s_lo);
+  unsigned int hits = __ballot_sync(0xffffffffu, mu < thr || (mu == thr && static_cast<uint32_t>(3 * nb + cand) < r.brow));
+  r.rescans += (hits >> lane) & 1u;
+  if (hits != 0u && __popc(hits) >= kMassHits) {
+    if ((hits >> lane) & 1u) {
+      uint32_t kbest = 0xffffffffu;
+      int cbest = -1;
+#pragma unroll
+      for (int j = 0; j < 32; ++j) {
+        int g;
+        asm volatile("ld.shared.b32 %0, [%1];" : "=r"(g) : "r"(gcache + 4 * j) : "memory");
+        const float sc = __uint_as_float(v[j]);
+        const float d = fmaxf(fmaf(-2.f, sc, 2.f), 0.f);
+        const bool pass = sc < s_hi && sc >= r.s_lo && d > r.dpi && g != r.ga && g != r.gp && g >= 0;
+        if (pass && __float_as_uint(d) < kbest) kbest = __float_as_uint(d), cbest = j;
+      }
+      if (cbest >= 0) mine_take(r, kbest, static_cast<uint32_t>(3 * (nb + cbest) + cand));
+    }
+    __syncwarp();
+  } else if (hits != 0u) {
+    int g_lane;
+    asm volatile("ld.shared.b32 %0, [%1];" : "=r"(g_lane) : "r"(gcache + 4 * lane) : "memory");
+    do {
+      const int src = __ffs(hits) - 1;
+      hits &= hits - 1u;
+      __syncwarp();
+      if (lane == src) {
+#pragma unroll
+        for (int j = 0; j < 8; ++j) sts128(stg + 16 * j, v[4 * j], v[4 * j + 1], v[4 * j + 2], v[4 * j + 3]);
+      }
+      __syncwarp();
+      float sc;
+      asm volatile("ld.shared.f32 %0, [%1];" : "=f"(sc) : "r"(stg + 4 * lane) : "memory");
+      const float hi_s = __shfl_sync(0xffffffffu, s_hi, src), lo_s = __shfl_sync(0xffffffffu, r.s_lo, src);
+      const float dp_s = __shfl_sync(0xffffffffu, r.dpi, src);
+      const int ga_s = __shfl_sync(0xffffffffu, r.ga, src), gp_s = __shfl_sync(0xffffffffu, r.gp, src);
+      const float d = fmaxf(fmaf(-2.f, sc, 2.f), 0.f);
+      const bool pass = sc < hi_s && sc >= lo_s && d > dp_s && g_lane != ga_s && g_lane != gp_s && g_lane >= 0;
+      const uint32_t kmin = __reduce_min_sync(0xffffffffu, pass ? __float_as_uint(d) : 0xffffffffu);
+      if (kmin != 0xffffffffu) {
+        const int col = __ffs(__ballot_sync(0xffffffffu, pass && __float_as_uint(d) == kmin)) - 1;
+        if (lane == src) mine_take(r, kmin, static_cast<uint32_t>(3 * (nb + col) + cand));
+      }
+    } while (hits != 0u);
+  }
+}
+
+template <int BN>
 struct EpiMine {
   static constexpr bool kSplitColumns = true;
-  static constexpr bool kPrefetchNext = (kVariant & 1) == 0;
-  static constexpr bool kRowConsts = (kVariant & 4) != 0;
-  struct State {
-    float dpi, bound_d;
-    int ga, gp;
-    uint32_t bound_row;
-    uint32_t release_bar;
-  };
-  static constexpr bool kEarlyRelease = true;
-  static constexpr bool kTmaStore = false;
+  using State = MineRow;
   const float* dp;
   const int32_t* guid;
   unsigned long long* best;
   int cand;
   unsigned long long* stats;
-  __device__ __forceinline__ void row_consts(int row, const GemmShape& s, uint32_t dst) const {
-    const bool row_ok = row < s.M;
-    const uint32_t inf = 0x7f800000u;
-    const uint32_t dpi = row_ok ? __float_as_uint(__ldg(dp + row)) : inf;
-    const uint32_t ga = row_ok ? static_cast<uint32_t>(__ldg(guid + 3 * row)) : 0u;
-    const uint32_t gp = row_ok ? static_cast<uint32_t>(__ldg(guid + 3 * row + 1)) : 0u;
-    const unsigned long long key = row_ok ? *(reinterpret_cast<volatile unsigned long long*>(best) + row) : ~0ull;
-    sts128(dst, dpi, ga, gp, static_cast<uint32_t>(key >> 32));
-    asm volatile("st.shared.b32 [%0], %1;" ::"r"(dst + 16), "r"(static_cast<uint32_t>(key)) : "memory");
-  }
-  __device__ __forceinline__ void load_state(State& st, uint32_t src) const {
-    const uint4 v = lds128(src);
-    st.dpi = __uint_as_float(v.x), st.ga = static_cast<int>(v.y), st.gp = static_cast<int>(v.z), st.bound_d = __uint_as_float(v.w);
-    asm volatile("ld.shared.b32 %0, [%1];" : "=r"(st.bound_row) : "r"(src + 16) : "memory");
-    st.release_bar = 0u;
-  }
   __device__ __forceinline__ void pre(State& st, int row, int , const GemmShape& s, int, int, uint32_t) const {
-    const bool row_ok = row < s.M;
-    const float inf = __int_as_float(0x7f800000);
-    st.dpi = row_ok ? __ldg(dp + row) : inf;
-    st.ga = row_ok ? __ldg(guid + 3 * row) : 0;
-    st.gp = row_ok ? __ldg(guid + 3 * row + 1) : 0;
-    const unsigned long long key = row_ok ? best[row] : ~0ull;
-    st.bound_d = __uint_as_float(static_cast<uint32_t>(key >> 32));
-    st.bound_row = static_cast<uint32_t>(key);
-    st.release_bar = 0u;
+    mine_row_seed(st, row, s.M, dp, guid, best);
+    st.rescans = 0;
   }
   __device__ __forceinline__ void cols(int n0, const GemmShape& s, int c0, int , uint32_t stg) const {
     static_assert(BN == 256, "a warp owns 4 chunks (128 columns) of the tile");
@@ -69,129 +128,274 @@
   __device__ __forceinline__ void block_end(uint32_t) const {}
   __device__ __forceinline__ void run(uint32_t taddr, int row, int n0, int , const GemmShape& s, int c0,
                                       int c1, uint32_t stg, State& st) const {
-    const int lane = threadIdx.x & 31;
-    const bool row_ok = row < s.M;
-    const float inf = __int_as_float(0x7f800000);
-    const float dpi = st.dpi;
-    const float s_hi = row_ok ? 1.f - 0.5f * dpi : -inf;
-    const int ga = st.ga, gp = st.gp;
-    float bound_d = st.bound_d;
-    if (!(bound_d == bound_d)) bound_d = inf;
-    float s_lo = 1.f - 0.5f * bound_d;
-    uint32_t brow = st.bound_row;
-    float bd = inf;
-    int br = -1;
-    uint32_t va[32], vb[32];
-    auto chunk = [&](const uint32_t (&v)[32], int cc) {
+#pragma unroll 1
+    for (int cc = 0; cc < 4; ++cc) {
       const int nb = n0 + (c0 + cc) * 32;
-      uint32_t u0 = 0xffffffffu, u1 = 0xffffffffu;
-#pragma unroll
-      for (int j = 0; j < 8; ++j) {
-        const float2 lo = sub2(s_hi, s_hi, __uint_as_float(v[4 * j]), __uint_as_float(v[4 * j + 1]));
-        const float2 hi = sub2(s_hi, s_hi, __uint_as_float(v[4 * j + 2]), __uint_as_float(v[4 * j + 3]));
-        u0 = umin3(u0, __float_as_uint(lo.x), __float_as_uint(lo.y));
-        u1 = umin3(u1, __float_as_uint(hi.x), __float_as_uint(hi.y));
-      }
-      const uint32_t mu = min(u0, u1), thr = __float_as_uint(s_hi - s_lo);
-      unsigned int hits = __ballot_sync(0xffffffffu, mu < thr || (mu == thr && static_cast<uint32_t>(3 * nb + cand) < brow));
-      if (hits != 0u && __popc(hits) >= kMassHits) {
-        if (lane == 0) atomicAdd(stats, static_cast<unsigned long long>(__popc(hits)));
-        if ((hits >> lane) & 1u) {
-          uint32_t kbest = 0xffffffffu;
-          int cbest = -1;
-#pragma unroll
-          for (int j = 0; j < 32; ++j) {
-            int g;
-            asm volatile("ld.shared.b32 %0, [%1];" : "=r"(g) : "r"(stg + kColCacheOff + 128 * cc + 4 * j) : "memory");
-            const float sc = __uint_as_float(v[j]);
-            const float d = fmaxf(fmaf(-2.f, sc, 2.f), 0.f);
-            const bool pass = sc < s_hi && sc >= s_lo && d > dpi && d < bd && g != ga && g != gp && g >= 0;
-            if (pass && __float_as_uint(d) < kbest) kbest = __float_as_uint(d), cbest = j;
+      if (c0 + cc >= c1 || nb >= s.N) break;
+      uint32_t v[32];
+      tmem_ld_32x32(taddr + (c0 + cc) * 32, v);
+      tmem_ld_wait();
+      mine_chunk(v, nb, cand, stg + kColCacheOff + 128 * cc, stg, st);
+    }
+    if (row < s.M && st.key != kNoCand) atomicMin(best + row, st.key);
+    mine_flush_rescans(st, stats);
+  }
+};
+
+constexpr int kMineStages = 8;
+struct MineSmem {
+  static constexpr uint32_t kKbBytes = kBM * kBK * 2;
+  static constexpr uint32_t kMaxKb = 4;
+  static constexpr uint32_t kRingOff = kMaxKb * kKbBytes;
+  static constexpr uint32_t kEpiOff = kRingOff + kMineStages * kKbBytes;
+  static constexpr uint32_t kBarOff = kEpiOff + 8 * kWarpSliceBytes;
+  static constexpr uint32_t kNumBars = 2 * kMineStages + 4 + 2;
+  static constexpr uint32_t kTotal = kBarOff + kNumBars * 8 + 16 + 1024;
+};
+static_assert(MineSmem::kTotal <= 232448, "mining scan: shared memory over the 227 KB limit");
+
+struct MineScan {
+  int B;
+  int panels;
+  int num_kb;
+  long long tiles;
+  uint32_t idesc;
+  const float* dp;
+  const int32_t* guid;
+  const int32_t* cguid;
+  unsigned long long* best;
+  unsigned long long* stats;
+};
+
+__global__ void __launch_bounds__(kGemmThreads, 1)
+mine_pair_kernel(const __grid_constant__ CUtensorMap tma_a, const __grid_constant__ CUtensorMap tma_c1,
+                 const __grid_constant__ CUtensorMap tma_c2, const MineScan s) {
+  using L = MineSmem;
+  extern __shared__ uint8_t smem_raw[];
+  const uint32_t raw_u32 = smem_u32(smem_raw);
+  const uint32_t base = (raw_u32 + 1023u) & ~1023u;
+  const uint32_t bar0 = base + L::kBarOff;
+  auto a_res = [&](int kb) { return base + kb * L::kKbBytes; };
+  auto c_smem = [&](int st) { return base + L::kRingOff + st * L::kKbBytes; };
+  auto full_bar = [&](int st) { return bar0 + 8u * st; };
+  auto empty_bar = [&](int st) { return bar0 + 8u * (kMineStages + st); };
+  auto tfull_bar = [&](int i) { return bar0 + 8u * (2 * kMineStages + i); };
+  auto tempty_bar = [&](int i) { return bar0 + 8u * (2 * kMineStages + 2 + i); };
+  const uint32_t afull_bar = bar0 + 8u * (2 * kMineStages + 4);
+  const uint32_t aempty_bar = bar0 + 8u * (2 * kMineStages + 5);
+  const uint32_t tmem_slot = bar0 + 8u * L::kNumBars;
+  volatile uint32_t* tmem_slot_ptr = reinterpret_cast<volatile uint32_t*>(smem_raw + (tmem_slot - raw_u32));
+
+  const int warp = threadIdx.x >> 5;
+  const int lane = threadIdx.x & 31;
+  const uint32_t rank = cluster_ctarank();
+  const bool leader = rank == 0;
+  const long long pair = blockIdx.x >> 1, num_pairs = gridDim.x >> 1;
+  const long long t0 = s.tiles * pair / num_pairs, t1 = s.tiles * (pair + 1) / num_pairs;
+  const int per_group = 2 * s.panels;
+  constexpr uint32_t kTmemCols = 512;
+
+  cluster_sync_all();
+  if (warp == 0 && lane == 0) {
+    tma_prefetch_desc(&tma_a);
+    tma_prefetch_desc(&tma_c1);
+    tma_prefetch_desc(&tma_c2);
+  }
+  if (warp == 1 && lane == 0) {
+    for (int i = 0; i < kMineStages; ++i) {
+      mbar_init(full_bar(i), 2);
+      mbar_init(empty_bar(i), 1);
+    }
+    for (int i = 0; i < 2; ++i) {
+      mbar_init(tfull_bar(i), 1);
+      mbar_init(tempty_bar(i), 16);
+    }
+    mbar_init(afull_bar, 2);
+    mbar_init(aempty_bar, 1);
+    fence_mbar_init();
+  }
+  if (warp == 2) {
+    tmem_alloc2(tmem_slot, kTmemCols);
+    tmem_relinquish2();
+  }
+  tc_fence_before();
+  cluster_sync_all();
+  tc_fence_after();
+  const uint32_t tmem_base = *tmem_slot_ptr;
+
+  if (warp == 0 && lane == 0) {
+    int stage = 0;
+    uint32_t phase = 0, aphase = 0;
+    int g = static_cast<int>(t0 / per_group), p = static_cast<int>(t0 % per_group);
+    for (long long t = t0; t < t1; ++t, p = (p + 1 == per_group) ? (++g, 0) : p + 1) {
+      if (t == t0 || p == 0) {
+        mbar_wait(aempty_bar, aphase ^ 1, 500);
+        aphase ^= 1;
+        const int m0 = g * (2 * kBM) + static_cast<int>(rank) * kBM;
+        for (int kb = 0; kb < s.num_kb; ++kb) tma_load_2d_pair(a_res(kb), &tma_a, afull_bar, kb * kBK, m0);
+        if (leader) mbar_arrive_expect_tx(afull_bar, 2 * s.num_kb * L::kKbBytes);
+        else mbar_arrive_cluster(afull_bar & kPeerBitMask);
+      }
+      const CUtensorMap* tc = p < s.panels ? &tma_c1 : &tma_c2;
+      const int n0 = (p < s.panels ? p : p - s.panels) * kBN2 + static_cast<int>(rank) * (kBN2 / 2);
+      for (int kb = 0; kb < s.num_kb; ++kb) {
+        mbar_wait(empty_bar(stage), phase ^ 1, 100 + stage);
+        tma_load_2d_pair(c_smem(stage), tc, full_bar(stage), kb * kBK, n0);
+        if (leader) mbar_arrive_expect_tx(full_bar(stage), 2 * L::kKbBytes);
+        else mbar_arrive_cluster(full_bar(stage) & kPeerBitMask);
+        if (++stage == kMineStages) stage = 0, phase ^= 1;
+      }
+    }
+  } else if (warp == 1 && lane == 0) {
+    if (leader) {
+      int stage = 0, it = 0;
+      uint32_t phase = 0, aphase = 0;
+      int p = static_cast<int>(t0 % per_group);
+      for (long long t = t0; t < t1; ++t, ++it, p = (p + 1 == per_group) ? 0 : p + 1) {
+        if (t == t0 || p == 0) {
+          if (t != t0) tc_commit2(aempty_bar);
+          mbar_wait(afull_bar, aphase, 600);
+          aphase ^= 1;
+          tc_fence_after();
+        }
+        const int as = it & 1;
+        const uint32_t ap = (it >> 1) & 1;
+        mbar_wait(tempty_bar(as), ap ^ 1, 200 + as);
+        tc_fence_after();
+        const uint32_t tmem_d = tmem_base + as * kBN2;
+        for (int kb = 0; kb < s.num_kb; ++kb) {
+          mbar_wait(full_bar(stage), phase, 300 + stage);
+          tc_fence_after();
+#pragma unroll
+          for (int k = 0; k < kBK / kUK; ++k) {
+            const uint64_t ad = make_smem_desc(a_res(kb) + k * (kUK * 2), 16, 1024);
+            const uint64_t bd = make_smem_desc(c_smem(stage) + k * (kUK * 2), 16, 1024);
+            umma2_f16(tmem_d, ad, bd, s.idesc, (kb > 0 || k > 0) ? 1u : 0u);
           }
-          if (cbest >= 0) {
-            bd = __uint_as_float(kbest), br = 3 * (nb + cbest) + cand;
-            const float s_new = 1.f - 0.5f * bd;
-            if (s_new > s_lo || (s_new == s_lo && static_cast<uint32_t>(br) < brow)) brow = static_cast<uint32_t>(br);
-            s_lo = fmaxf(s_lo, s_new);
-          }
+          tc_commit2(empty_bar(stage));
+          if (kb == s.num_kb - 1) tc_commit2(tfull_bar(as));
+          if (++stage == kMineStages) stage = 0, phase ^= 1;
         }
-        __syncwarp();
-      } else if (hits != 0u) {
-        if (lane == 0) atomicAdd(stats, static_cast<unsigned long long>(__popc(hits)));
-        int g_lane;
-        asm volatile("ld.shared.b32 %0, [%1];" : "=r"(g_lane) : "r"(stg + kColCacheOff + 128 * cc + 4 * lane) : "memory");
-        do {
-          const int src = __ffs(hits) - 1;
-          hits &= hits - 1u;
-          __syncwarp();
-          if (lane == src) {
-#pragma unroll
-            for (int j = 0; j < 8; ++j) sts128(stg + 16 * j, v[4 * j], v[4 * j + 1], v[4 * j + 2], v[4 * j + 3]);
-          }
-          __syncwarp();
-          float sc;
-          asm volatile("ld.shared.f32 %0, [%1];" : "=f"(sc) : "r"(stg + 4 * lane) : "memory");
-          const float hi_s = __shfl_sync(0xffffffffu, s_hi, src), lo_s = __shfl_sync(0xffffffffu, s_lo, src);
-          const float dp_s = __shfl_sync(0xffffffffu, dpi, src), bd_s = __shfl_sync(0xffffffffu, bd, src);
-          const int ga_s = __shfl_sync(0xffffffffu, ga, src), gp_s = __shfl_sync(0xffffffffu, gp, src);
-          const float d = fmaxf(fmaf(-2.f, sc, 2.f), 0.f);
-          const bool pass = sc < hi_s && sc >= lo_s && d > dp_s && d < bd_s && g_lane != ga_s && g_lane != gp_s && g_lane >= 0;
-          const uint32_t kmin = __reduce_min_sync(0xffffffffu, pass ? __float_as_uint(d) : 0xffffffffu);
-          if (kmin != 0xffffffffu) {
-            const int col = __ffs(__ballot_sync(0xffffffffu, pass && __float_as_uint(d) == kmin)) - 1;
-            if (lane == src) {
-              bd = __uint_as_float(kmin), br = 3 * (nb + col) + cand;
-              const float s_new = 1.f - 0.5f * bd;
-              if (s_new > s_lo || (s_new == s_lo && static_cast<uint32_t>(br) < brow)) brow = static_cast<uint32_t>(br);
-              s_lo = fmaxf(s_lo, s_new);
-            }
-          }
-        } while (hits != 0u);
-      }
+      }
+    }
+  } else if (warp >= 4) {
+    const int q = warp & 3;
+    const int half = (warp - 4) >> 2;
+    const uint32_t stg = base + L::kEpiOff + (warp - 4) * kWarpSliceBytes;
+    uint32_t gnext[4];
+    auto fetch_guids = [&](int p) {
+      const int32_t* src = s.cguid + static_cast<int64_t>(p) * kBN2 + half * 128 + lane;
+#pragma unroll
+      for (int i = 0; i < 4; ++i) gnext[i] = static_cast<uint32_t>(__ldg(src + 32 * i));
     };
-    auto ok = [&](int cc) { return c0 + cc < c1 && n0 + (c0 + cc) * 32 < s.N; };
-    if constexpr ((kVariant & 2) == 0) {
-      tmem_ld_32x32(taddr + c0 * 32, va);
+    int g = static_cast<int>(t0 / per_group), p = static_cast<int>(t0 % per_group);
+    if (t0 < t1) fetch_guids(p);
+    MineRow r;
+    r.key = kNoCand;
+    r.rescans = 0;
+    int row = 0;
+    int it = 0;
+    for (long long t = t0; t < t1; ++t, ++it, p = (p + 1 == per_group) ? (++g, 0) : p + 1) {
+      if (t == t0 || p == 0) {
+        if (r.key != kNoCand) atomicMin(s.best + row, r.key);
+        mine_flush_rescans(r, s.stats);
+        row = g * (2 * kBM) + static_cast<int>(rank) * kBM + q * 32 + lane;
+        mine_row_seed(r, row, s.B, s.dp, s.guid, s.best);
+      }
+      __syncwarp();
+#pragma unroll
+      for (int i = 0; i < 4; ++i)
+        asm volatile("st.shared.b32 [%0], %1;" ::"r"(stg + kColCacheOff + 4 * (32 * i + lane)), "r"(gnext[i]) : "memory");
+      __syncwarp();
+      if (t + 1 < t1) fetch_guids(p + 1 == per_group ? 0 : p + 1);
+      const int cand = p < s.panels ? 1 : 2;
+      const int nb0 = (p < s.panels ? p : p - s.panels) * kBN2 + half * 128;
+      const int as = it & 1;
+      const uint32_t ap = (it >> 1) & 1;
+      mbar_wait(tfull_bar(as), ap, 400 + as);
+      tc_fence_after();
+      const uint32_t taddr = tmem_base + (static_cast<uint32_t>(q * 32) << 16) + as * kBN2 + half * 128;
+      auto ok = [&](int cc) { return nb0 + cc * 32 < s.B; };
+      auto chunk = [&](const uint32_t (&v)[32], int cc) {
+        mine_chunk(v, nb0 + cc * 32, cand, stg + kColCacheOff + 128 * cc, stg, r);
+      };
+      uint32_t va[32], vb[32];
+      tmem_ld_32x32(taddr, va);
 #pragma unroll
       for (int cc = 0; cc < 4; cc += 2) {
         tmem_ld_wait();
-        if (ok(cc + 1)) tmem_ld_32x32(taddr + (c0 + cc + 1) * 32, vb);
+        tmem_ld_32x32(taddr + (cc + 1) * 32, vb);
         if (ok(cc)) chunk(va, cc);
         tmem_ld_wait();
-        if (cc + 2 < 4 && ok(cc + 2)) tmem_ld_32x32(taddr + (c0 + cc + 2) * 32, va);
-        if (cc + 2 >= 4 && st.release_bar != 0u) {
+        if (cc + 2 < 4) {
+          tmem_ld_32x32(taddr + (cc + 2) * 32, va);
+        } else {
           tc_fence_before();
           __syncwarp();
-          if (lane == 0) mbar_arrive(st.release_bar);
+          if (lane == 0) mbar_arrive_cluster(tempty_bar(as) & kPeerBitMask);
         }
         if (ok(cc + 1)) chunk(vb, cc + 1);
       }
-    } else {
-#pragma unroll
-      for (int cc = 0; cc < 4; ++cc) {
-        if (ok(cc)) {
-          tmem_ld_32x32(taddr + (c0 + cc) * 32, va);
-          tmem_ld_wait();
-          chunk(va, cc);
-        }
-      }
-      if (st.release_bar != 0u) {
-        tc_fence_before();
-        __syncwarp();
-        if (lane == 0) mbar_arrive(st.release_bar);
-      }
-    }
-    if (br >= 0)
-      atomicMin(best + row, (static_cast<unsigned long long>(__float_as_uint(bd)) << 32) | static_cast<uint32_t>(br));
-  }
-};
+    }
+    if (r.key != kNoCand) atomicMin(s.best + row, r.key);
+    mine_flush_rescans(r, s.stats);
+  }
+
+  tc_fence_before();
+  cluster_sync_all();
+  if (warp == 2) {
+    tc_fence_after();
+    tmem_dealloc2(tmem_base, kTmemCols);
+  }
+}
+
+static int launch_mine_pair(cdml_ctx* ctx, const uint16_t* e16, int64_t ld16, int dtype16, int64_t B, int D,
+                            const MineScan& scan_args, cudaStream_t st) {
+  CUtensorMap ta, tc1, tc2;
+  int rc = make_tmap_2d(ctx, &ta, e16, dtype16, D, B, 3 * ld16, kBK, kBM);
+  if (rc == 0) rc = make_tmap_2d(ctx, &tc1, e16 + ld16, dtype16, D, B, 3 * ld16, kBK, kBN2 / 2);
+  if (rc == 0) rc = make_tmap_2d(ctx, &tc2, e16 + 2 * ld16, dtype16, D, B, 3 * ld16, kBK, kBN2 / 2);
+  if (rc) return rc;
+  MineScan s = scan_args;
+  s.B = static_cast<int>(B);
+  s.panels = static_cast<int>((B + kBN2 - 1) / kBN2);
+  s.num_kb = (D + kBK - 1) / kBK;
+  s.tiles = static_cast<long long>(s.panels) * 2 * s.panels;
+  s.idesc = make_idesc_f16(dtype16 == CDML_BF16 ? 1 : 0, 0, 0, 2 * kBM, kBN2);
+  cudaLaunchConfig_t cfg = {};
+  cfg.blockDim = dim3(kGemmThreads);
+  cfg.dynamicSmemBytes = MineSmem::kTotal;
+  cfg.stream = st;
+  cudaLaunchAttribute attr[1];
+  attr[0].id = cudaLaunchAttributeClusterDimension;
+  attr[0].val.clusterDim.x = 2, attr[0].val.clusterDim.y = 1, attr[0].val.clusterDim.z = 1;
+  cfg.attrs = attr;
+  cfg.numAttrs = 1;
+  static int max_pairs = 0;
+  if (max_pairs == 0) {
+    CDML_CHECK_CUDA(cudaFuncSetAttribute(mine_pair_kernel, cudaFuncAttributeMaxDynamicSharedMemorySize, MineSmem::kTotal));
+    cfg.gridDim = dim3(ctx->num_sms);
+    CDML_CHECK_CUDA(cudaOccupancyMaxActiveClusters(&max_pairs, mine_pair_kernel, &cfg));
+    CDML_REQUIRE(max_pairs > 0, "mining scan: no CTA pair fits on the device");
+  }
+  const int pairs = static_cast<int>(std::min<long long>(std::min(max_pairs, ctx->num_sms / 2), s.tiles));
+  cfg.gridDim = dim3(2 * pairs);
+  CDML_CHECK_CUDA(cudaLaunchKernelEx(&cfg, mine_pair_kernel, ta, tc1, tc2, s));
+  if (trace_sync("mine_pair", B, 2 * B, D, 2 * pairs, st)) return -2;
+  return 0;
+}
 
 __global__ void mine_prepare_kernel(const float* __restrict__ E, int64_t ld, int D, const int64_t* __restrict__ guid64,
-                                    int64_t B, float* __restrict__ dp, int32_t* __restrict__ guid32,
-                                    unsigned long long* __restrict__ best, unsigned long long* __restrict__ stats) {
+                                    int64_t B, int64_t Bp, float* __restrict__ dp, int32_t* __restrict__ guid32,
+                                    int32_t* __restrict__ cguid, unsigned long long* __restrict__ best,
+                                    unsigned long long* __restrict__ stats) {
   const int warp = threadIdx.x >> 5, lane = threadIdx.x & 31;
   if (blockIdx.x == 0 && threadIdx.x < 2) stats[threadIdx.x] = 0ull;
-  for (int64_t i = static_cast<int64_t>(blockIdx.x) * 8 + warp; i < B; i += static_cast<int64_t>(gridDim.x) * 8) {
+  for (int64_t i = static_cast<int64_t>(blockIdx.x) * 8 + warp; i < Bp; i += static_cast<int64_t>(gridDim.x) * 8) {
+    if (i >= B) {
+      if (lane < 2) cguid[lane * Bp + i] = -1;
+      continue;
+    }
     const float* a = E + 3 * i * ld;
     const float* p = a + ld;
     float s = 0.f;
@@ -203,6 +407,7 @@
     for (int o = 16; o > 0; o >>= 1) s += __shfl_xor_sync(0xffffffffu, s, o);
     if (lane == 0) dp[i] = s, best[i] = kNoCand;
     if (lane < 3) guid32[3 * i + lane] = static_cast<int32_t>(guid64[3 * i + lane]);
+    if (lane < 2) cguid[lane * Bp + i] = static_cast<int32_t>(guid64[3 * i + 1 + lane]);
   }
 }
 
@@ -244,7 +449,9 @@
   CDML_REQUIRE(B > 0 && 3 * B < (1ll << 31) && D > 0 && D % 8 == 0 && ld16 >= D && ld32 >= D,
                "cdml_mine_semihard: bad geometry B=%lld D=%d", (long long)B, D);
   cudaStream_t st = static_cast<cudaStream_t>(stream);
-  const size_t bytes = static_cast<size_t>(B) * (8 + 4 + 12) + 64;
+  const int64_t Bp = (B + kBN2 - 1) / kBN2 * kBN2;
+  const size_t cguid_off = (static_cast<size_t>(B) * (8 + 4 + 12) + 127) / 128 * 128;
+  const size_t bytes = cguid_off + static_cast<size_t>(Bp) * 8 + 64;
   uint8_t* ws = static_cast<uint8_t*>(ctx_scratch(ctx, bytes));
   if (ws == nullptr) return -2;
   if (ctx->mine_stats == nullptr) CDML_CHECK_CUDA(cudaMalloc(&ctx->mine_stats, 2 * sizeof(unsigned long long)));
@@ -252,23 +459,20 @@
   unsigned long long* best = reinterpret_cast<unsigned long long*>(ws);
   float* dp = reinterpret_cast<float*>(best + B);
   int32_t* guid32 = reinterpret_cast<int32_t*>(dp + B);
-  const int grid = static_cast<int>(std::min<int64_t>((B + 7) / 8, ctx->num_sms * 8));
-  mine_prepare_kernel<<<grid, 256, 0, st>>>(E32, ld32, D, guid, B, dp, guid32, best, stats);
+  int32_t* cguid = reinterpret_cast<int32_t*>(ws + cguid_off);
+  const int grid = static_cast<int>(std::min<int64_t>((Bp + 7) / 8, ctx->num_sms * 8));
+  mine_prepare_kernel<<<grid, 256, 0, st>>>(E32, ld32, D, guid, B, Bp, dp, guid32, cguid, best, stats);
   int rc = 0;
   const uint16_t* e16 = static_cast<const uint16_t*>(E16);
-  for (int cand = 1; cand <= 2 && rc >= 0; ++cand) {
-    EpiMine<kBN, 1> epi{dp, guid32, best, cand, stats};
-    static int rowc = -1;
-    if (rowc < 0) rowc = getenv("CDML_MINE_ROWCONSTS") != nullptr ? 1 : 0;
-    if (resb_applicable(D) && B >= 8 * kBM && rowc) {
-      EpiMine<kBN, 5> epi5{dp, guid32, best, cand, stats};
-      rc = launch_gemm_resb(ctx, e16, 3 * ld16, e16 + cand * ld16, 3 * ld16, B, B, D, dtype16, epi5, st);
-    } else if (resb_applicable(D) && B >= 8 * kBM && epi_warps() == 16)
-      rc = launch_gemm_resb<EpiMine<kBN, 1>, 16>(ctx, e16, 3 * ld16, e16 + cand * ld16, 3 * ld16, B, B, D, dtype16, epi, st);
-    else if (resb_applicable(D) && B >= 8 * kBM)
-      rc = launch_gemm_resb(ctx, e16, 3 * ld16, e16 + cand * ld16, 3 * ld16, B, B, D, dtype16, epi, st);
-    else
+  if (D <= 4 * kBK) {
+    MineScan s = {};
+    s.dp = dp, s.guid = guid32, s.cguid = cguid, s.best = best, s.stats = stats;
+    rc = launch_mine_pair(ctx, e16, ld16, dtype16, B, D, s, st);
+  } else {
+    for (int cand = 1; cand <= 2 && rc >= 0; ++cand) {
+      EpiMine<kBN> epi{dp, guid32, best, cand, stats};
       rc = launch_gemm<0, 0>(ctx, e16, 3 * ld16, e16 + cand * ld16, 3 * ld16, B, B, D, dtype16, 1, epi, st);
+    }
   }
   if (rc >= 0) {
     mine_finalize_kernel<<<grid, 256, 0, st>>>(E32, ld32, D, best, B, neg_row, d_an, stats);
diff --git a/collaborative-deep-metric-learning_b200/ops.py b/collaborative-deep-metric-learning_b200/ops.py
--- a/collaborative-deep-metric-learning_b200/ops.py
+++ b/collaborative-deep-metric-learning_b200/ops.py
@@ -281,7 +281,7 @@
   neg_row = torch.empty((B,), dtype=torch.int32, device=E32.device)
   d_an = torch.empty((B,), dtype=torch.float32, device=E32.device) if want_dist else None
   guid = guid.to(torch.int64).contiguous()
-  _count(4)
+  _count(3)
   check(_lib.load().cdml_mine_semihard(_ctx(E32), ptr(E16), E16.stride(0), dtype16_of(E16), ptr(E32), E32.stride(0),
                                        ptr(guid), B, D, float(margin), ptr(neg_row), ptr(d_an), stream_ptr()))
   return neg_row, d_an
```

Result: no change. 5.789 million (median of 6 runs) (-0.0%).
